# tgialoimtr/cnn_lstm_ctc_ocr

Hardware: AMD Instinct MI355X
Metric: line-crops/sec (train step) at 32x256 bs=256; CER vs ref (higher is better)
Workload: dtype bf16

## Files before the change

cnn_lstm_ctc_ocr_amd/_lib.py:

```python
import ctypes
import os

import torch

_HERE = os.path.dirname(os.path.abspath(__file__))
LIB_PATH = os.environ.get("OCRK_LIB") or os.path.join(_HERE, "libocrk.so")

OCRK_OK = 0
OCRK_ERR_INVALID_ARG = 1
OCRK_ERR_HIP = 2
OCRK_ERR_INFEASIBLE = 3

F32 = 0
BF16 = 1

_p = ctypes.c_void_p
_i32 = ctypes.c_int
_u32 = ctypes.c_uint
_i64 = ctypes.c_int64
_f32 = ctypes.c_float
_sz = ctypes.c_size_t

SIGNATURES = {
    "ocrk_version": [],
    "ocrk_last_error": [],
    "ocrk_set_option": [ctypes.c_char_p, _i64, _p],
    "ocrk_get_option": [ctypes.c_char_p, _p],
    "ocrk_preprocess": [_p, _i64, _p, _i32, _p],
    "ocrk_status_clear": [_p, ctypes.c_uint32, _p],
    "ocrk_set_f32_gemm_mode": [_i32],
    "ocrk_f32_gemm_exact": [],
    "ocrk_ctc_workspace_size": [_i32, _i32, _i32],
    "ocrk_ctc_loss": [_p, _p, _p, _p, _i32, _i32, _i32, _i32, _f32, _p, _p, _p, _p, _p, _sz, _p],
    "ocrk_ctc_align_workspace_size": [_i32, _i32, _i32],
    "ocrk_ctc_align": [_p, _p, _p, _p, _i32, _i32, _i32, _i32, _p, _p, _p, _p, _p, _p, _p, _sz, _p],
    "ocrk_ctc_lexicon_workspace_size": [_i32, _i32, _i32, _i32, _i32],
    "ocrk_ctc_lexicon_score": [_p, _p, _i32, _i32, _i32, _p, _p, _i32, _i32, _i32, _p, _p, _p, _p, _p, _p, _p, _sz,
                               _p],
    "ocrk_ctc_spot_workspace_size": [_i32, _i32, _i32, _i32, _i32],
    "ocrk_ctc_spot": [_p, _p, _i32, _i32, _i32, _p, _p, _p, _i32, _i32, _p, _p, _p, _p, _p, _sz, _p],
    "ocrk_ctc_greedy_decode": [_p, _p, _i32, _i32, _i32, _i32, _p, _p, _p, _p],
    "ocrk_ctc_beam_workspace_size": [_i32, _i32, _i32],
    "ocrk_gru_fwd_step": [_p, _p, _p, _p, _p, _p, _i32, _i32, _i32, _i32, _p, _p, _p, _p, _i32, _p],
    "ocrk_gru_fwd": [_p, _p, _p, _p, _p, _p, _i32, _i32, _i32, _p, _p, _p, _p, _i32, _p],
    "ocrk_gru_bwd": [_p, _p, _p, _p, _p, _p, _p, _i32, _i32, _i32, _p, _p, _p, _p, _i32, _p],
    "ocrk_ctc_beam_decode": [_p, _p, _i32, _i32, _i32, _i32, _i32, _i32, _p, _p, _p, _p, _sz, _p],
    "ocrk_crc32c": [_p, _sz, ctypes.c_uint32],
    "ocrk_edit_distance": [_p, _p, _i32, _p, _p, _i32, _i32, _p, _p, _p],
    "ocrk_conv1_fwd": [_p, _i32, _i32, _i32, _i32, _p, _p, _i32, _p, _i32, _p],
    "ocrk_conv1_wgrad_workspace_size": [_i32, _i32, _i32, _i32],
    "ocrk_conv1_bwd_weight": [_p, _i32, _p, _i32, _i32, _i32, _i32, _p, _p, _i32, _p, _sz, _i32, _p],
    "ocrk_conv2_bwd_data_conv1_wgrad_supported": [_i32, _i32, _i32, _i32, _i32, _i32],
    "ocrk_conv2_bwd_data_conv1_wgrad_workspace_size": [_i32, _i32, _i32],
    "ocrk_conv2_bwd_data_conv1_wgrad": [_p, _i32, _i32, _i32, _p, _p, _p, _p, _i32, _p, _p, _i32, _p, _sz, _i32,
                                        _p],
    "ocrk_conv12_bwd_supported": [_i32, _i32, _i32, _i32],
    "ocrk_conv12_bwd_workspace_size": [_i32, _i32, _i32],
    "ocrk_conv12_bwd": [_p, _i32, _i32, _i32, _p, _p, _p, _p, _i32, _p, _p, _p, _p, _p, _i32, _p, _sz, _i32, _p],
    "ocrk_conv12_fwd_supported": [_i32, _i32, _i32, _i32],
    "ocrk_conv12_fwd": [_p, _i32, _i32, _i32, _i32, _p, _p, _p, _p, _p, _p, _p, _p, _i32, _p],
    "ocrk_conv1_fwd_relu_bits": [_p, _i32, _i32, _i32, _i32, _p, _p, _i32, _p, _p, _i32, _p],
    "ocrk_conv_stats_tiles": [_i64],
    "ocrk_conv3x3_fwd": [_p, _i32, _i32, _i32, _i32, _p, _p, _i32, _p, _i32, _i32, _p, _i32, _p],
    "ocrk_conv3x3_bwd_data_workspace_size": [_i32, _i32, _i32, _i32],
    "ocrk_conv3x3_bwd_data": [_p, _i32, _i32, _i32, _i32, _p, _i32, _p, _p, _p, _i32, _p, _sz, _i32, _p],
    "ocrk_conv3x3_fwd_relu_bits_supported": [_i32, _i32, _i32, _i32, _i32, _i32],
    "ocrk_conv3x3_fwd_relu_bits": [_p, _i32, _i32, _i32, _i32, _p, _p, _i32, _p, _p, _i32, _p],
    "ocrk_conv3x3_bwd_data_bits_supported": [_i32, _i32, _i32, _i32, _i32, _i32],
    "ocrk_conv3x3_bwd_data_bits": [_p, _i32, _i32, _i32, _i32, _p, _i32, _p, _p, _p, _i32, _p, _sz, _i32, _p],
    "ocrk_conv3x3_bwd_data_bits_slab": [_p, _i32, _i32, _i32, _i32, _p, _i32, _p, _p, _p, _i32, _p],
    "ocrk_conv3x3_bwd_data_slab": [_p, _i32, _i32, _i32, _i32, _p, _i32, _p, _p, _p, _i32, _p],
    "ocrk_conv3x3_wgrad_workspace_size": [_i32, _i32, _i32, _i32, _i32],
    "ocrk_conv3x3_bwd_weight": [_p, _p, _i32, _i32, _i32, _i32, _i32, _p, _i32, _p, _sz, _i32, _p],
    "ocrk_bn_finalize_workspace_size": [_i32, _i32],
    "ocrk_bn_finalize": [_p, _i32, _i64, _i32, _f32, _f32, _p, _p, _p, _p, _p, _sz, _p],
    "ocrk_bn_finalize_tiles": [_p, _i32, _i32, _i64, _i32, _f32, _f32, _p, _p, _p, _p, _p, _sz, _p],
    "ocrk_conv3x3_fwd_rowstats_supported": [_i32, _i32, _i32, _i32, _i32],
    "ocrk_conv3x3_fwd_rowstats": [_p, _i32, _i32, _i32, _i32, _p, _p, _i32, _p, _i32, _p, _p],
    "ocrk_bn_infer_params": [_p, _p, _i32, _f32, _p, _p, _p],
    "ocrk_bn_relu_pool_fwd": [_p, _i32, _i32, _i32, _i32, _p, _p, _p, _p, _i32, _i32, _i32, _i32,
                              _p, _i32, _i32, _p],
    "ocrk_bn_bwd_workspace_size": [_i32, _i32, _i32, _i32],
    "ocrk_bn_relu_pool_bwd": [_p, _p, _i32, _i32, _i32, _i32, _p, _p, _p, _p, _i32, _i32, _i32, _i32,
                              _i32, _p, _p, _p, _p, _i32, _p, _sz, _i32, _p],
    "ocrk_bn_moments": [_p, _i32, _i32, _i64, _i32, _p, _p, _sz, _p],
    "ocrk_bn_finalize_moments": [_p, _i32, _f32, _f32, _p, _p, _p, _p, _p],
    "ocrk_bn_bwd_pooled_bias_slab_rows": [_i32, _i32, _i32, _i32, _i32, _i32, _i32, _i32],
    "ocrk_bn_relu_pool_bwd_pooled": [_p, _p, _p, _i32, _i32, _i32, _i32, _p, _p, _p, _p, _i32, _i32, _i32, _i32,
                                     _i32, _p, _p, _p, _p, _i32, _p, _p, _sz, _i32, _p],
    "ocrk_bn_relu_pool_bwd_reduce": [_p, _p, _i32, _i32, _i32, _i32, _p, _p, _p, _p, _i32, _i32, _i32, _i32,
                                     _i32, _p, _p, _i32, _p, _p, _sz, _i32, _p],
    "ocrk_bn_relu_pool_bwd_apply": [_p, _p, _i32, _i32, _i32, _i32, _p, _p, _p, _p, _i32, _i32, _i32, _i32,
                                    _i32, _p, _p, _p, _p, _i32, _p, _p, _sz, _i32, _p],
    "ocrk_bn_bwd_bias_slab_rows": [_i32, _i32, _i32, _i32, _i32, _i32, _i32, _i32],
    "ocrk_bn_relu_pool_bwd_slab": [_p, _p, _i32, _i32, _i32, _i32, _p, _p, _p, _p, _i32, _i32, _i32, _i32,
                                   _i32, _p, _p, _p, _i32, _p, _p, _sz, _i32, _p],
    "ocrk_lstm_fwd_step": [_p, _p, _p, _p, _p, _p, _i32, _i32, _i32, _i32, _p, _p, _p, _p, _i32, _p],
    "ocrk_lstm_bwd_step": [_p, _p, _p, _p, _p, _i32, _i32, _i32, _i32, _p, _p, _p, _p, _i32, _p],
    "ocrk_copy_batch": [_p, _i32, _i64, _p],
    "ocrk_gru_fwd_persistent_supported": [_i32, _i32],
    "ocrk_gru_fwd_persistent_workspace_size": [_i32, _i32],
    "ocrk_gru_fwd_persistent": [_p, _p, _p, _p, _i32, _i32, _i32, _p, _p, _p, _p, _p, _p, _p, _sz, _p],
    "ocrk_gru_bwd_persistent_supported": [_i32, _i32],
    "ocrk_gru_bwd_persistent_workspace_size": [_i32, _i32],
    "ocrk_gru_bwd_persistent": [_p, _p, _p, _i32, _i32, _i32, _p, _p, _p, _p, _p, _p, _p, _p, _sz, _p],
    "ocrk_persistent_flags_size": [_i32, _i32],
    "ocrk_lstm_fwd_persistent_supported": [_i32, _i32],
    "ocrk_lstm_fwd_persistent_workspace_size": [_i32, _i32],
    "ocrk_lstm_fwd_persistent": [_p, _p, _p, _i32, _i32, _i32, _p, _p, _p, _p, _p, _p, _p, _sz, _p],
    "ocrk_lstm_fwd_persistent_f32_supported": [_i32, _i32],
    "ocrk_lstm_fwd_persistent_f32_workspace_size": [_i32, _i32],
    "ocrk_lstm_fwd_persistent_f32_flags_size": [_i32, _i32],
    "ocrk_lstm_fwd_persistent_f32": [_p, _p, _p, _i32, _i32, _i32, _p, _p, _p, _p, _p, _p, _p, _sz, _p],
    "ocrk_lstm_bwd_persistent_f32_supported": [_i32, _i32],
    "ocrk_lstm_bwd_persistent_f32_workspace_size": [_i32, _i32],
    "ocrk_lstm_bwd_persistent_f32": [_p, _p, _i32, _i32, _i32, _p, _p, _p, _p, _p, _p, _p, _p, _sz, _p],
    "ocrk_lstm_bwd_persistent_supported": [_i32, _i32],
    "ocrk_lstm_bwd_persistent_workspace_size": [_i32, _i32],
    "ocrk_lstm_bwd_persistent_slices": [_i32, _i32],
    "ocrk_lstm_bwd_persistent": [_p, _p, _i32, _i32, _i32, _p, _p, _p, _p, _p, _p, _p, _p, _sz, _p],
    "ocrk_lstm_fwd": [_p, _p, _p, _p, _p, _i32, _i32, _i32, _p, _p, _p, _p, _i32, _p],
    "ocrk_lstm_bwd": [_p, _p, _p, _p, _i32, _i32, _i32, _p, _p, _p, _p, _i32, _p],
    "ocrk_gemm_workspace_size": [_i32, _i32, _i32, _i32],
    "ocrk_gemm": [_i32, _i32, _i32, _i32, _i32, _f32, _p, _i64, _i64, _p, _i64, _i64, _p, _i64, _i64,
                  _i32, _p, _i32, _i32, _i32, _i32, _i32, _p, _sz, _p],
    "ocrk_adam": [_p, _p, _p, _p, _i64, _f32, _f32, _f32, _f32, _f32, _p],
    "ocrk_adam_ex": [_p, _p, _p, _p, _i64, _f32, _f32, _f32, _f32, _f32, _u32, _p],
    "ocrk_cast": [_p, _i32, _p, _i32, _i64, _p],
    "ocrk_split_bf16": [_p, _i64, _p, _p, _p],
    "ocrk_permute3": [_p, _i32, _i32, _i32, _i32, _p, _i32, _p],
    "ocrk_strided_copy": [_p, _i64, _i64, _i64, _i64, _p, _i32, _i64, _i64, _p],
    "ocrk_colsum_workspace_size": [_i64, _i32],
    "ocrk_colsum": [_p, _i64, _i32, _i32, _p, _i32, _p, _sz, _p],
    "ocrk_slab_sum_workspace_size": [_i32],
    "ocrk_slab_sum": [_p, _i32, _i32, _i32, _p, _i32, _p, _sz, _p],
    "ocrk_relu_mask": [_p, _p, _i64, _f32, _p, _i32, _p],
    "ocrk_mul_scalar": [_p, _i64, _p, _p],
    "ocrk_mean": [_p, _i32, _p, _p],
    "ocrk_seq_len": [_p, _i32, _p, _p],
    "ocrk_timer_create": [_p],
    "ocrk_timer_record": [_p, _p],
    "ocrk_timer_elapsed": [_p, _p, _p],
    "ocrk_timer_destroy": [_p],
}
_RESTYPE = {"ocrk_last_error": ctypes.c_char_p}
_RESTYPE.update({n: ctypes.c_size_t for n in SIGNATURES if n.endswith("_workspace_size")})
_RESTYPE["ocrk_conv_stats_tiles"] = ctypes.c_size_t
_RESTYPE["ocrk_persistent_flags_size"] = ctypes.c_size_t
_RESTYPE["ocrk_bn_bwd_bias_slab_rows"] = ctypes.c_size_t
_RESTYPE["ocrk_bn_bwd_pooled_bias_slab_rows"] = ctypes.c_size_t
_RESTYPE["ocrk_crc32c"] = ctypes.c_uint32


class OcrkError(RuntimeError):

    def __init__(self, status, message):
        super().__init__(message)
        self.status = status


class InvalidArgumentError(OcrkError):
    """Mirrors tf.errors.InvalidArgumentError (e.g. infeasible CTC labels)."""


class DeviceError(OcrkError):
    """A device-side wait gave up (persistent recurrent kernels): its outputs are invalid."""


STATUS_CTC_INFEASIBLE = 1 << 1
STATUS_CTC_BAD_LENGTH = 1 << 2
STATUS_CTC_BAD_LABEL = 1 << 3
STATUS_LSTM_FWD_TIMEOUT = 1 << 4
STATUS_LSTM_BWD_TIMEOUT = 1 << 5
STATUS_LSTM_CENSUS = 1 << 6
STATUS_CTC = STATUS_CTC_INFEASIBLE | STATUS_CTC_BAD_LENGTH | STATUS_CTC_BAD_LABEL
STATUS_LSTM = STATUS_LSTM_FWD_TIMEOUT | STATUS_LSTM_BWD_TIMEOUT | STATUS_LSTM_CENSUS

_STATUS_TEXT = {
    STATUS_CTC_INFEASIBLE: "ctc_loss: not enough time for the target transition sequence "
                           "(label + repeats > sequence_length)",
    STATUS_CTC_BAD_LENGTH: "ctc_loss: a label length is negative or exceeds the labels' width",
    STATUS_CTC_BAD_LABEL: "ctc_loss: a label value is outside [0, num_classes - 1)",
    STATUS_LSTM_FWD_TIMEOUT: "persistent recurrent forward: a hand-off wait gave up (co-residency lost)",
    STATUS_LSTM_BWD_TIMEOUT: "persistent recurrent backward: a hand-off wait gave up (co-residency lost)",
    STATUS_LSTM_CENSUS: "persistent recurrent launch: the placement census gave up",
}


ON_DEVICE_ERROR = []


def raise_for_status(word):
    word = int(word)
    if not word:
        return
    text = "; ".join(t for b, t in _STATUS_TEXT.items() if word & b)
    if word & STATUS_LSTM:
        for fn in ON_DEVICE_ERROR:
            fn()
        raise DeviceError(OCRK_ERR_HIP, f"device status 0x{word:x}: {text}")
    raise InvalidArgumentError(OCRK_ERR_INFEASIBLE, f"device status 0x{word:x}: {text}")


DEBUG_SIGNATURES = {
    "ocrk_lstm_debug_stamps": [_p],
    "ocrk_conv2_bwd_weight_c1x_supported": [_i32, _i32, _i32, _i32],
    "ocrk_conv2_bwd_weight_c1x": [_p, _i32, _i32, _i32, _i32, _p, _p, _p, _p, _i32, _p, _sz, _i32, _p],
    "ocrk_stream_wait": [_p, _p, _i32],
    "ocrk_stream_create_cu_limited": [_i32, _p],
    "ocrk_stream_destroy": [_p],
    "ocrk_lstm_fwd_persistent_x_supported": [_i32, _i32, _i32],
    "ocrk_lstm_fwd_persistent_x": [_p, _i32, _p, _p, _p, _p, _i32, _i32, _i32, _p, _p, _p, _p, _p, _p, _p, _sz, _p],
}

_lib = None


def lib():
    global _lib
    if _lib is None:
        if not os.path.exists(LIB_PATH):
            raise ImportError(
                f"{LIB_PATH} is missing: build it with `make` in the repo root "
                "(or __graft_entry__.build()); there is no CPU fallback")
        handle = ctypes.CDLL(LIB_PATH)
        for name, argtypes in SIGNATURES.items():
            fn = getattr(handle, name)
            fn.argtypes = argtypes
            fn.restype = _RESTYPE.get(name, ctypes.c_int)
        for name, argtypes in DEBUG_SIGNATURES.items():
            if hasattr(handle, name):
                getattr(handle, name).argtypes = argtypes
        _lib = handle
    return _lib


class Timer:

    def __init__(self):
        h = ctypes.c_void_p()
        call("ocrk_timer_create", ctypes.byref(h))
        self.h = h

    def record(self):
        call("ocrk_timer_record", self.h, stream_ptr())

    def elapsed_ms(self, end):
        ms = ctypes.c_float()
        call("ocrk_timer_elapsed", self.h, end.h, ctypes.byref(ms))
        return ms.value

    def __del__(self):
        if _lib is not None and self.h:
            _lib.ocrk_timer_destroy(self.h)


PROBES = {}


def call(name, *args):
    probe = PROBES.get(name)
    if probe is not None and probe[0] is not None and probe[0](args) is None:
        probe = None
    if probe is not None:
        work_fn, records = probe
        ev0, ev1 = Timer(), Timer()
        ev0.record()
        status = getattr(lib(), name)(*args)
        ev1.record()
        records.append((ev0, ev1, work_fn(args) if work_fn else 0.0))
    else:
        status = getattr(lib(), name)(*args)
    if status != OCRK_OK:
        msg = lib().ocrk_last_error().decode(errors="replace")
        if status in (OCRK_ERR_INFEASIBLE, OCRK_ERR_INVALID_ARG):
            raise InvalidArgumentError(status, msg)
        raise OcrkError(status, msg)
    return status


def ptr(t):
    return None if t is None else ctypes.c_void_p(t.data_ptr())


def stream_ptr(device=None):
    return ctypes.c_void_p(torch.cuda.current_stream(device).cuda_stream)
```

cnn_lstm_ctc_ocr_amd/csrc/conv.hip:

```cpp
#include "common.h"
#include "gemm.h"
#include "reduce.h"
#include "mfma_util.h"

constexpr int C1_PX = 256;
constexpr int C1_WR = 8;

template <typename TIn>
__device__ __forceinline__ float conv1_in(TIn v) {
    if constexpr (sizeof(TIn) == 1) {
#pragma clang fp contract(off)
        return (float)v * (1.0f / 255.0f) - 0.5f;
    } else {
        return to_f32(v);
    }
}

template <typename TIn, int ROWS>
__device__ __forceinline__ void conv1_stage(const TIn* __restrict__ x, int H, int W, int b, int h0, int wo0,
                                            float (*sx)[C1_PX + 2]) {
    constexpr int N = ROWS * (C1_PX + 2), IT = (N + 255) / 256;
    TIn v[IT];
    bool ok[IT];
#pragma unroll
// ... 201 lines not shown
    OCRK_REQUIRE(relu_bits, "ocrk_conv1_fwd_relu_bits: null mask");
    return conv1_fwd_run(x, x_is_u8, B, H, W, w, bias, cout, y, (uint8_t*)relu_bits, dtype, stream);
}

static int64_t conv1_blocks(int B, int H, int W) {
    return std::max<int64_t>(1, (int64_t)B * ocrk::cdiv(H - 2, C1_GR) * ocrk::cdiv(W - 2, C1_PX));
}

extern "C" size_t ocrk_conv1_wgrad_workspace_size(int B, int H, int W, int cout) {
    return ((size_t)conv1_blocks(B, H, W) * 10 * cout * sizeof(float) + 15) / 16 * 16 +
           (size_t)ocrk::SLAB_P * 10 * cout * sizeof(double);
}

extern "C" int ocrk_conv1_bwd_weight(const void* x, int x_is_u8, const void* dz, int B, int H, int W,
                                     int cout, float* dw, float* db, int accumulate, void* ws,
                                     size_t ws_bytes, int dtype, void* stream) {
    OCRK_REQUIRE(cout == 32, "ocrk_conv1_bwd_weight: Cout=%d unsupported", cout);
    OCRK_REQUIRE(ws_bytes >= ocrk_conv1_wgrad_workspace_size(B, H, W, cout), "ocrk_conv1_bwd_weight: workspace too small");
    OCRK_REQUIRE(B >= 1 && H >= 3 && W >= 3, "ocrk_conv1_bwd_weight: bad shape B=%d H=%d W=%d", B, H, W);
    const int64_t nb = conv1_blocks(B, H, W);
    OCRK_REQUIRE(nb < (1ll << 31), "ocrk_conv1_bwd_weight: too many rows");
    hipStream_t s = ocrk::as_stream(stream);
    float* slab = (float*)ws;
    if (x_is_u8) {
        if (dtype == OCRK_BF16) conv1_wgrad_partial<uint8_t, bf16, 32><<<nb, 256, 0, s>>>((const uint8_t*)x, (const bf16*)dz, B, H, W, slab);
        else conv1_wgrad_partial<uint8_t, float, 32><<<nb, 256, 0, s>>>((const uint8_t*)x, (const float*)dz, B, H, W, slab);
    } else {
        if (dtype == OCRK_BF16) conv1_wgrad_partial<bf16, bf16, 32><<<nb, 256, 0, s>>>((const bf16*)x, (const bf16*)dz, B, H, W, slab);
        else conv1_wgrad_partial<float, float, 32><<<nb, 256, 0, s>>>((const float*)x, (const float*)dz, B, H, W, slab);
    }
    int st = ocrk::launch_status("ocrk_conv1_bwd_weight");
    if (st) return st;
    double* part = (double*)((char*)ws + ((size_t)nb * 10 * cout * sizeof(float) + 15) / 16 * 16);
    return ocrk::slab_sum(slab, (int)nb, 10 * cout, part, nullptr, dw, db, 9 * cout, accumulate, s);
}

extern "C" size_t ocrk_conv_stats_tiles(int64_t M) { return (size_t)ocrk::cdiv(M, 128); }

namespace ocrk {
int conv_direct_fwd(const void* x, int B, int H, int W, int cin, const void* w_nk, const float* bias, int cout,
                    void* y, int relu, float* stats, hipStream_t s);
int conv_direct_bwd_data(const void* dy, int B, int H, int W, int cout, const void* w_bwd, int cin, void* dx,
                         const void* relu_mask, float* stats, hipStream_t s);
size_t conv_direct_wgrad_ws_bytes(int B, int H, int W, int cin, int cout);
int conv_direct_wgrad(const void* x, const void* dy, int B, int H, int W, int cin, int cout, float* dw,
                      int accumulate, void* ws, size_t ws_bytes, hipStream_t s);
size_t conv_rows_wgrad_ws_bytes(int B, int cin, int cout);
bool conv_rows_fwd_covers(int B, int H, int W, int cin, int cout);
int conv_rows_fwd(const void* x, int B, int H, int W, int cin, const void* w_nk, const float* bias, int cout, void* y,
                  int relu, float* stats, hipStream_t s);
int conv_rows_dgrad(const void* dy, int B, int H, int W, int cout, const void* w_bwd, int cin, void* dx,
                    const void* relu_mask, float* stats, hipStream_t s);
int conv_rows_wgrad(const void* x, const void* dy, int B, int H, int W, int cin, int cout, float* dw, int accumulate,
                    void* ws, size_t ws_bytes, hipStream_t s);
bool conv_rows_dgrad_c1_covers(int B, int H, int W, int cin, int cout);
bool conv_rows_fwd_bits_covers(int B, int H, int W, int cin, int cout);
bool conv12_fwd_covers(int B, int H, int W);
int conv12_fwd(const void* img, int x_is_u8, int B, int H, int W, const float* w1, const float* b1,
               const void* w_nk2, const float* b2, void* y1, void* bits, void* z, float* stats, hipStream_t s);
int conv_rows_wgrad_c1x(const void* img, int x_is_u8, const float* w1, const float* b1, const void* dy, int B, int H,
                        int W, float* dw, int accumulate, void* ws, size_t ws_bytes, hipStream_t s);
int conv_rows_fwd_bits(const void* x, int B, int H, int W, int cin, const void* w_nk, const float* bias, int cout,
                       void* y, void* bits, hipStream_t s);
bool conv_rows_dgrad_bits_covers(int B, int H, int W, int cin, int cout);
int conv_rows_dgrad_bits(const void* dy, int B, int H, int W, int cout, const void* w_bwd, int cin, void* dx,
                         const void* bits, float* stats, hipStream_t s);
bool gemm_nt_enabled();
bool nt_staged_enabled();
int64_t conv_rows_dgrad_c1_parts(int B);
int conv_rows_dgrad_c1(const void* dy, int B, int H, int W, const void* w_bwd, const void* relu_mask,
                       const void* relu_bits, const void* x, int x_is_u8, float* part, hipStream_t s);
int64_t conv_rows_bwd_w2_parts(int B);
int conv_rows_bwd_w2(const void* dy, int B, int H, int W, const void* w_bwd, const void* relu_mask,
                     const void* relu_bits, const void* x, int x_is_u8, const float* w1, const float* b1,
                     float* c1part, float* w2part, float* dw2, int accumulate, hipStream_t s);
}

extern "C" int ocrk_conv12_fwd_supported(int B, int IH, int IW, int dtype) {
    return dtype == OCRK_BF16 && IH >= 3 && IW >= 3 && ocrk::conv12_fwd_covers(B, IH - 2, IW - 2) ? 1 : 0;
}

extern "C" int ocrk_conv12_fwd(const void* x, int x_is_u8, int B, int IH, int IW, const float* w1, const float* b1,
                               const void* w_nk2, const float* b2, void* y1, void* relu_bits, void* z, float* stats,
                               int dtype, void* stream) {
    OCRK_REQUIRE(ocrk_conv12_fwd_supported(B, IH, IW, dtype), "ocrk_conv12_fwd: B=%d IH=%d IW=%d dtype=%d not covered",
                 B, IH, IW, dtype);
    OCRK_REQUIRE(x && w1 && b1 && w_nk2 && relu_bits && z && stats, "ocrk_conv12_fwd: null pointer");
    return ocrk::conv12_fwd(x, x_is_u8, B, IH - 2, IW - 2, w1, b1, w_nk2, b2, y1, relu_bits, z, stats,
                            ocrk::as_stream(stream));
}

#ifdef OCRK_EXPERIMENTS
extern "C" int ocrk_conv2_bwd_weight_c1x_supported(int B, int IH, int IW, int dtype) {
    return ocrk_conv12_fwd_supported(B, IH, IW, dtype);
}

extern "C" int ocrk_conv2_bwd_weight_c1x(const void* x, int x_is_u8, int B, int IH, int IW, const float* w1,
                                         const float* b1, const void* dz, float* dw, int accumulate, void* ws,
                                         size_t ws_bytes, int dtype, void* stream) {
    OCRK_REQUIRE(ocrk_conv2_bwd_weight_c1x_supported(B, IH, IW, dtype),
                 "ocrk_conv2_bwd_weight_c1x: B=%d IH=%d IW=%d dtype=%d not covered", B, IH, IW, dtype);
    OCRK_REQUIRE(x && w1 && b1 && dz && dw && ws, "ocrk_conv2_bwd_weight_c1x: null pointer");
    int st = ocrk::conv_rows_wgrad_c1x(x, x_is_u8, w1, b1, dz, B, IH - 2, IW - 2, dw, accumulate, ws, ws_bytes,
                                       ocrk::as_stream(stream));
    OCRK_REQUIRE(st >= 0, "ocrk_conv2_bwd_weight_c1x: workspace too small or path disabled");
    return st;
}
#endif

extern "C" int ocrk_conv2_bwd_data_conv1_wgrad_supported(int B, int H, int W, int cin, int cout, int dtype) {
    return dtype == OCRK_BF16 && ocrk::conv_rows_dgrad_c1_covers(B, H, W, cin, cout) ? 1 : 0;
}

extern "C" size_t ocrk_conv2_bwd_data_conv1_wgrad_workspace_size(int B, int H, int W) {
    (void)H; (void)W;
    return ((size_t)ocrk::conv_rows_dgrad_c1_parts(std::max(B, 1)) * 10 * 32 * sizeof(float) + 15) / 16 * 16 +
           (size_t)ocrk::SLAB_P * 10 * 32 * sizeof(double);
}

extern "C" int ocrk_conv2_bwd_data_conv1_wgrad(const void* dz, int B, int H, int W, const void* w_bwd,
                                               const void* relu_mask, const void* relu_bits, const void* x,
                                               int x_is_u8, float* dw, float* db, int accumulate, void* ws,
                                               size_t ws_bytes, int dtype, void* stream) {
    OCRK_REQUIRE(ocrk_conv2_bwd_data_conv1_wgrad_supported(B, H, W, 32, 32, dtype),
                 "ocrk_conv2_bwd_data_conv1_wgrad: B=%d H=%d W=%d dtype=%d not covered", B, H, W, dtype);
    OCRK_REQUIRE(dz && w_bwd && x && dw && db && ws, "ocrk_conv2_bwd_data_conv1_wgrad: null pointer");
    OCRK_REQUIRE(!relu_mask != !relu_bits, "ocrk_conv2_bwd_data_conv1_wgrad: give exactly one of relu_mask / relu_bits");
    OCRK_REQUIRE(ws_bytes >= ocrk_conv2_bwd_data_conv1_wgrad_workspace_size(B, H, W) && (uintptr_t)ws % 16 == 0,
                 "ocrk_conv2_bwd_data_conv1_wgrad: workspace too small or misaligned");
    const int64_t nb = ocrk::conv_rows_dgrad_c1_parts(B);
    OCRK_REQUIRE(nb < (1ll << 31), "ocrk_conv2_bwd_data_conv1_wgrad: too many rows");
    hipStream_t s = ocrk::as_stream(stream);
    float* part = (float*)ws;
    int st = ocrk::conv_rows_dgrad_c1(dz, B, H, W, w_bwd, relu_mask, relu_bits, x, x_is_u8, part, s);
    if (st) return st;
    double* part2 = (double*)((char*)ws + ((size_t)nb * 10 * 32 * sizeof(float) + 15) / 16 * 16);
    return ocrk::slab_sum(part, (int)nb, 10 * 32, part2, nullptr, dw, db, 9 * 32, accumulate, s);
}

static size_t conv12_bwd_c1_bytes(int B) {
    return ((size_t)ocrk::conv_rows_bwd_w2_parts(std::max(B, 1)) * 10 * 32 * sizeof(float) + 15) / 16 * 16;
}

extern "C" int ocrk_conv12_bwd_supported(int B, int H, int W, int dtype) {
    return dtype == OCRK_BF16 && ocrk::conv_rows_dgrad_c1_covers(B, H, W, 32, 32) ? 1 : 0;
}

extern "C" size_t ocrk_conv12_bwd_workspace_size(int B, int H, int W) {
    (void)H; (void)W;
    return conv12_bwd_c1_bytes(B) + (size_t)ocrk::SLAB_P * 10 * 32 * sizeof(double) +
           (size_t)std::max<int64_t>(2, ocrk::conv_rows_bwd_w2_parts(std::max(B, 1))) * 9 * 32 * 32 * sizeof(float);
}

extern "C" int ocrk_conv12_bwd(const void* dz, int B, int H, int W, const void* w_bwd, const void* relu_mask,
                               const void* relu_bits, const void* x, int x_is_u8, const float* w1, const float* b1,
                               float* dw2, float* dw1, float* db1, int accumulate, void* ws, size_t ws_bytes,
                               int dtype, void* stream) {
    OCRK_REQUIRE(ocrk_conv12_bwd_supported(B, H, W, dtype), "ocrk_conv12_bwd: B=%d H=%d W=%d dtype=%d not covered",
                 B, H, W, dtype);
    OCRK_REQUIRE(dz && w_bwd && x && w1 && b1 && dw2 && dw1 && db1 && ws, "ocrk_conv12_bwd: null pointer");
    OCRK_REQUIRE(!relu_mask != !relu_bits, "ocrk_conv12_bwd: give exactly one of relu_mask / relu_bits");
    OCRK_REQUIRE(ws_bytes >= ocrk_conv12_bwd_workspace_size(B, H, W) && (uintptr_t)ws % 16 == 0,
                 "ocrk_conv12_bwd: workspace too small or misaligned");
    const int64_t nb = ocrk::conv_rows_bwd_w2_parts(B);
    OCRK_REQUIRE(nb < (1ll << 31), "ocrk_conv12_bwd: too many rows");
    hipStream_t s = ocrk::as_stream(stream);
    float* c1part = (float*)ws;
    double* c1sum = (double*)((char*)ws + conv12_bwd_c1_bytes(B));
    float* w2part = (float*)((char*)c1sum + (size_t)ocrk::SLAB_P * 10 * 32 * sizeof(double));
    int st = ocrk::conv_rows_bwd_w2(dz, B, H, W, w_bwd, relu_mask, relu_bits, x, x_is_u8, w1, b1, c1part, w2part, dw2,
                                    accumulate, s);
    if (st) return st;
    return ocrk::slab_sum(c1part, (int)nb, 10 * 32, c1sum, nullptr, dw1, db1, 9 * 32, accumulate, s);
}

extern "C" int ocrk_conv3x3_fwd(const void* x, int B, int H, int W, int cin, const void* w_nk,
                                const float* bias, int cout, void* y, int y_dtype, int relu,
                                float* stats, int dtype, void* stream) {
    ocrk::GemmParams p = {};
    p.M = B * H * W; p.N = cout; p.K = 9 * cin; p.batch = 1;
    p.A = x; p.B = w_nk; p.ldb = 9 * cin;
    p.C = y; p.ldc = cout; p.c_bf16 = y_dtype == OCRK_BF16;
    p.bias = bias; p.relu = relu; p.alpha = 1.f; p.stats = stats;
    p.splits = 1; p.k_chunk = (int)ocrk::cdiv(p.K, 32) * 32;
    p.convH = H; p.convW = W; p.convC = cin;
    if (dtype == OCRK_BF16 && y_dtype == OCRK_BF16) {
        int st = stats ? -1 : ocrk::conv_rows_fwd(x, B, H, W, cin, w_nk, bias, cout, y, relu, nullptr, ocrk::as_stream(stream));
        if (st >= 0) return st;
        st = ocrk::conv_direct_fwd(x, B, H, W, cin, w_nk, bias, cout, y, relu, stats, ocrk::as_stream(stream));
        if (st >= 0) return st;
    }
    return ocrk::gemm(p, ocrk::A_IM2COL, ocrk::B_NK, dtype, ocrk::as_stream(stream));
}

extern "C" int ocrk_conv3x3_fwd_rowstats_supported(int B, int H, int W, int cin, int cout) {
    return ocrk::conv_rows_fwd_covers(B, H, W, cin, cout) ? 1 : 0;
}

extern "C" int ocrk_conv3x3_fwd_rowstats(const void* x, int B, int H, int W, int cin, const void* w_nk,
                                         const float* bias, int cout, void* y, int relu, float* stats, void* stream) {
    OCRK_REQUIRE(stats && ocrk::conv_rows_fwd_covers(B, H, W, cin, cout),
                 "ocrk_conv3x3_fwd_rowstats: shape B=%d H=%d W=%d %d->%d not covered", B, H, W, cin, cout);
    return ocrk::conv_rows_fwd(x, B, H, W, cin, w_nk, bias, cout, y, relu, stats, ocrk::as_stream(stream));
}

static int64_t bwd_data_tiles(int B, int H, int W) { return ocrk::cdiv((int64_t)B * H * W, 128); }

static int bwd_data_run(const void* dy, int B, int H, int W, int cout, const void* w_bwd, int cin, void* dx,
                        const void* relu_mask, float* stats, int dtype, hipStream_t s, const void* relu_bits = nullptr) {
    ocrk::GemmParams p = {};
    p.M = B * H * W; p.N = cin; p.K = 9 * cout; p.batch = 1;
    p.A = dy; p.B = w_bwd; p.ldb = 9 * cout;
    p.C = dx; p.ldc = cin; p.c_bf16 = dtype == OCRK_BF16;
    p.mask = relu_mask; p.ldmask = cin; p.alpha = 1.f;
    p.splits = 1; p.k_chunk = (int)ocrk::cdiv(p.K, 32) * 32;
    p.convH = H; p.convW = W; p.convC = cout;
    p.stats = stats;
    if (relu_bits) {
        const int sb = ocrk::conv_rows_dgrad_bits(dy, B, H, W, cout, w_bwd, cin, dx, relu_bits, stats, s);
        if (sb >= 0) return sb;
        p.mask = nullptr;
        p.mask_bits = relu_bits;
        return ocrk::gemm(p, ocrk::A_IM2COL_FLIP, ocrk::B_NK, dtype, s);
    }
    int st = dtype == OCRK_BF16 ? ocrk::conv_rows_dgrad(dy, B, H, W, cout, w_bwd, cin, dx, relu_mask, stats, s) : -1;
    if (st < 0 && dtype == OCRK_BF16) st = ocrk::conv_direct_bwd_data(dy, B, H, W, cout, w_bwd, cin, dx, relu_mask, stats, s);
    if (st < 0) st = ocrk::gemm(p, ocrk::A_IM2COL_FLIP, ocrk::B_NK, dtype, s);
    return st;
}

static bool nt_bits_ok(int cin, int cout) {
    return ocrk::gemm_nt_enabled() && ocrk::nt_staged_enabled() && cin % 8 == 0 && cout % 8 == 0 &&
           (9 * cin >= 512 || cout <= 64);
}

extern "C" int ocrk_conv3x3_fwd_relu_bits_supported(int B, int H, int W, int cin, int cout, int dtype) {
    if (dtype != OCRK_BF16 || B < 1 || H < 1 || W < 1 || (int64_t)B * H * W >= (1ll << 31)) return 0;
    return ocrk::conv_rows_fwd_bits_covers(B, H, W, cin, cout) || nt_bits_ok(cin, cout) ? 1 : 0;
}

extern "C" int ocrk_conv3x3_fwd_relu_bits(const void* x, int B, int H, int W, int cin, const void* w_nk,
                                          const float* bias, int cout, void* y, void* relu_bits, int dtype,
                                          void* stream) {
    OCRK_REQUIRE(relu_bits && ocrk_conv3x3_fwd_relu_bits_supported(B, H, W, cin, cout, dtype),
                 "ocrk_conv3x3_fwd_relu_bits: B=%d H=%d W=%d %d->%d dtype=%d not covered", B, H, W, cin, cout, dtype);
    hipStream_t s = ocrk::as_stream(stream);
    const int st = ocrk::conv_rows_fwd_bits(x, B, H, W, cin, w_nk, bias, cout, y, relu_bits, s);
    if (st >= 0) return st;
    ocrk::GemmParams p = {};
    p.M = B * H * W; p.N = cout; p.K = 9 * cin; p.batch = 1;
    p.A = x; p.B = w_nk; p.ldb = 9 * cin;
    p.C = y; p.ldc = cout; p.c_bf16 = 1;
    p.bias = bias; p.relu = 1; p.alpha = 1.f;
    p.splits = 1; p.k_chunk = (int)ocrk::cdiv(p.K, 32) * 32;
    p.convH = H; p.convW = W; p.convC = cin;
    p.relu_bits = relu_bits;
    return ocrk::gemm(p, ocrk::A_IM2COL, ocrk::B_NK, dtype, s);
}

extern "C" int ocrk_conv3x3_bwd_data_bits_supported(int B, int H, int W, int cout, int cin, int dtype) {
    if (dtype != OCRK_BF16 || B < 1 || H < 1 || W < 1 || (int64_t)B * H * W >= (1ll << 31)) return 0;
    return ocrk::conv_rows_dgrad_bits_covers(B, H, W, cin, cout) || nt_bits_ok(cout, cin) ? 1 : 0;
}

extern "C" size_t ocrk_conv3x3_bwd_data_workspace_size(int B, int H, int W, int cin) {
    return ((size_t)bwd_data_tiles(B, H, W) * 2 * cin * sizeof(float) + 7) / 8 * 8 +
           (size_t)ocrk::SLAB_P * cin * sizeof(double);
}

extern "C" int ocrk_conv3x3_bwd_data_bits(const void* dy, int B, int H, int W, int cout, const void* w_bwd, int cin,
                                          void* dx, const void* relu_bits, float* dbias, int accumulate, void* ws,
                                          size_t ws_bytes, int dtype, void* stream) {
    OCRK_REQUIRE(relu_bits && ocrk_conv3x3_bwd_data_bits_supported(B, H, W, cout, cin, dtype),
                 "ocrk_conv3x3_bwd_data_bits: B=%d H=%d W=%d %d<-%d dtype=%d not covered", B, H, W, cin, cout, dtype);
    hipStream_t s = ocrk::as_stream(stream);
    if (!dbias) return bwd_data_run(dy, B, H, W, cout, w_bwd, cin, dx, nullptr, nullptr, dtype, s, relu_bits);
    OCRK_REQUIRE(ws && ws_bytes >= ocrk_conv3x3_bwd_data_workspace_size(B, H, W, cin),
                 "ocrk_conv3x3_bwd_data_bits: workspace too small for the bias gradient");
    int st = bwd_data_run(dy, B, H, W, cout, w_bwd, cin, dx, nullptr, (float*)ws, dtype, s, relu_bits);
    if (st) return st;
    const int tiles = (int)bwd_data_tiles(B, H, W);
    double* part = (double*)((char*)ws + ((size_t)tiles * 2 * cin * sizeof(float) + 7) / 8 * 8);
    return ocrk::slab_sum((const float*)ws, tiles, cin, part, nullptr, dbias, nullptr, cin, accumulate, s, 2 * cin);
}

extern "C" int ocrk_conv3x3_bwd_data(const void* dy, int B, int H, int W, int cout, const void* w_bwd,
                                     int cin, void* dx, const void* relu_mask, float* dbias, int accumulate,
                                     void* ws, size_t ws_bytes, int dtype, void* stream) {
    hipStream_t s = ocrk::as_stream(stream);
    if (!dbias) return bwd_data_run(dy, B, H, W, cout, w_bwd, cin, dx, relu_mask, nullptr, dtype, s);
    OCRK_REQUIRE(ws && ws_bytes >= ocrk_conv3x3_bwd_data_workspace_size(B, H, W, cin),
                 "ocrk_conv3x3_bwd_data: workspace too small for the bias gradient");
    int st = bwd_data_run(dy, B, H, W, cout, w_bwd, cin, dx, relu_mask, (float*)ws, dtype, s);
    if (st) return st;
    const int tiles = (int)bwd_data_tiles(B, H, W);
    double* part = (double*)((char*)ws + ((size_t)tiles * 2 * cin * sizeof(float) + 7) / 8 * 8);
    return ocrk::slab_sum((const float*)ws, tiles, cin, part, nullptr, dbias, nullptr, cin, accumulate, s, 2 * cin);
}

extern "C" int ocrk_conv3x3_bwd_data_bits_slab(const void* dy, int B, int H, int W, int cout, const void* w_bwd,
                                               int cin, void* dx, const void* relu_bits, float* slab, int dtype,
                                               void* stream) {
    OCRK_REQUIRE(slab && relu_bits && ocrk_conv3x3_bwd_data_bits_supported(B, H, W, cout, cin, dtype),
                 "ocrk_conv3x3_bwd_data_bits_slab: B=%d H=%d W=%d %d<-%d dtype=%d not covered (or no slab)", B, H, W,
                 cin, cout, dtype);
    return bwd_data_run(dy, B, H, W, cout, w_bwd, cin, dx, nullptr, slab, dtype, ocrk::as_stream(stream), relu_bits);
}

extern "C" int ocrk_conv3x3_bwd_data_slab(const void* dy, int B, int H, int W, int cout, const void* w_bwd,
                                          int cin, void* dx, const void* relu_mask, float* slab, int dtype,
                                          void* stream) {
    OCRK_REQUIRE(slab, "ocrk_conv3x3_bwd_data_slab: slab is required");
    return bwd_data_run(dy, B, H, W, cout, w_bwd, cin, dx, relu_mask, slab, dtype, ocrk::as_stream(stream));
}

static int conv_tn_items() {
    const int64_t v = ocrk::opt(ocrk::OPT_CONV_TN_ITEMS);
    return v >= 16 ? (int)v : 192;
}

static int wgrad_splits(int64_t M, int cin, int cout) {
    if (ocrk::gemm_pptn_covers(ocrk::A_IM2COL_T, 9 * cin, cout, cin)) {
        const int64_t tiles = ocrk::cdiv(9 * cin, 256) * ocrk::cdiv(cout, 256);
        return (int)std::max<int64_t>(1, std::min<int64_t>(conv_tn_items() / tiles, M / 2048));
    }
    int64_t tiles = ocrk::cdiv(9 * cin, 128) * ocrk::cdiv(cout, cout <= 32 ? 32 : (cout <= 64 ? 64 : 128));
// ... 41 lines not shown
```

cnn_lstm_ctc_ocr_amd/csrc/tensor_ops.hip:

```cpp
#include "common.h"
#include "reduce.h"
#include "mfma_util.h"

template <typename TI, typename TO>
__global__ void __launch_bounds__(256) cast_kernel(const TI* __restrict__ in, TO* __restrict__ out, int64_t n) {
    for (int64_t i = (int64_t)blockIdx.x * 256 + threadIdx.x; i < n; i += (int64_t)gridDim.x * 256)
        out[i] = from_f32<TO>(to_f32(in[i]));
}

template <typename TI, typename TO>
__global__ void __launch_bounds__(256) permute3_kernel(const TI* __restrict__ in, int d0, int d1, int d2,
                                                       TO* __restrict__ out) {
    const int64_t n = (int64_t)d0 * d1 * d2;
    for (int64_t o = (int64_t)blockIdx.x * 256 + threadIdx.x; o < n; o += (int64_t)gridDim.x * 256) {
        int i2 = (int)(o % d2);
        int64_t t = o / d2;
        int i0 = (int)(t % d0);
        int i1 = (int)(t / d0);
        out[o] = from_f32<TO>(to_f32(in[((int64_t)i0 * d1 + i1) * d2 + i2]));
    }
}

namespace ocrk {
namespace {

__global__ void __launch_bounds__(256)
slab_sum_fused(const float* __restrict__ slab, int nslab, int NC, int ld, float* __restrict__ res,
               float* __restrict__ dst_lo, float* __restrict__ dst_hi, int split, int accumulate) {
    constexpr int RG = 64, CQ = 4, U = 16;
    __shared__ double red[RG][4 * CQ + 1];
    const int cq = threadIdx.x % CQ, rg = threadIdx.x / CQ;
    const int c0 = blockIdx.x * 4 * CQ + 4 * cq;
    double s[4] = {0.0, 0.0, 0.0, 0.0};
    if (c0 < NC) {
        const float* col = slab + c0;
        int i = rg;
        for (; i + (U - 1) * RG < nslab; i += U * RG) {
            f32x4 v[U];
#pragma unroll
            for (int u = 0; u < U; ++u) v[u] = *reinterpret_cast<const f32x4*>(col + (int64_t)(i + u * RG) * ld);
#pragma unroll
            for (int u = 0; u < U; ++u)
#pragma unroll
                for (int e = 0; e < 4; ++e) s[e] += v[u][e];
        }
        for (; i < nslab; i += RG) {
            const f32x4 v = *reinterpret_cast<const f32x4*>(col + (int64_t)i * ld);
#pragma unroll
            for (int e = 0; e < 4; ++e) s[e] += v[e];
        }
    }
#pragma unroll
    for (int e = 0; e < 4; ++e) red[rg][4 * cq + e] = s[e];
    __syncthreads();
    if (threadIdx.x < 4 * CQ) {
        const int c = blockIdx.x * 4 * CQ + threadIdx.x;
        if (c >= NC) return;
        double t = 0.0;
        for (int y = 0; y < RG; ++y) t += red[y][threadIdx.x];
        const float v = (float)t;
        if (res) res[c] = v;
        float* d = c < split ? (dst_lo ? dst_lo + c : nullptr) : (dst_hi ? dst_hi + (c - split) : nullptr);
        if (d) *d = accumulate ? *d + v : v;
    }
}

__global__ void __launch_bounds__(256)
slab_sum_stage1(const float* __restrict__ slab, int nslab, int NC, int ld, double* __restrict__ part) {
    __shared__ double red[4][64];
    const int cl = threadIdx.x & 63, q = threadIdx.x >> 6;
    const int c = blockIdx.x * 64 + cl;
    const int rows = (nslab + SLAB_P - 1) / SLAB_P;
    const int r0 = blockIdx.y * rows, r1 = min(nslab, r0 + rows);
    double s = 0.0;
    if (c < NC)
        for (int i = r0 + q; i < r1; i += 4) s += slab[(int64_t)i * ld + c];
    red[q][cl] = s;
    __syncthreads();
    if (q == 0 && c < NC) part[(int64_t)blockIdx.y * NC + c] = red[0][cl] + red[1][cl] + red[2][cl] + red[3][cl];
}

__global__ void __launch_bounds__(64)
slab_sum_stage2(const double* __restrict__ part, int NC, float* __restrict__ res, float* __restrict__ dst_lo,
                float* __restrict__ dst_hi, int split, int accumulate) {
    const int c = blockIdx.x * 64 + threadIdx.x;
    if (c >= NC) return;
    double t = 0.0;
    for (int y = 0; y < SLAB_P; ++y) t += part[(int64_t)y * NC + c];
    const float v = (float)t;
    if (res) res[c] = v;
    float* d = c < split ? (dst_lo ? dst_lo + c : nullptr) : (dst_hi ? dst_hi + (c - split) : nullptr);
    if (d) *d = accumulate ? *d + v : v;
}

}

int slab_sum(const float* slab, int nslab, int NC, double* part, float* res, float* dst_lo, float* dst_hi,
             int split, int accumulate, hipStream_t s, int ld) {
    const int l = ld > 0 ? ld : NC;
    if (NC % 4 == 0 && l % 4 == 0 && ((uintptr_t)slab & 15) == 0) {
        slab_sum_fused<<<(NC + 15) / 16, 256, 0, s>>>(slab, nslab, NC, l, res, dst_lo, dst_hi, split, accumulate);
        return ocrk::launch_status("slab sum");
    }
    slab_sum_stage1<<<dim3((NC + 63) / 64, SLAB_P), 256, 0, s>>>(slab, nslab, NC, ld > 0 ? ld : NC, part);
    int st = ocrk::launch_status("slab sum 1");
    if (st) return st;
    slab_sum_stage2<<<(NC + 63) / 64, 64, 0, s>>>(part, NC, res, dst_lo, dst_hi, split, accumulate);
    return ocrk::launch_status("slab sum 2");
}

}

template <typename T>
__global__ void __launch_bounds__(256) colsum_partial_kernel(const T* __restrict__ in, int64_t M, int N,
                                                             int64_t rows_per_block, float* __restrict__ slab) {
    __shared__ float red[256 * 9];
    const int G = N / 8;
    const int TPR = G < 64 ? G : 64;
    const int RPP = 256 / TPR;
    const int tg = threadIdx.x % TPR, tr = threadIdx.x / TPR;
    const int g = blockIdx.x * TPR + tg;
    const int64_t r0 = (int64_t)blockIdx.y * rows_per_block;
    const int64_t r1 = min(M, r0 + rows_per_block);
    float acc[8] = {0.f, 0.f, 0.f, 0.f, 0.f, 0.f, 0.f, 0.f};
    if (tr < RPP && g < G) {
#pragma unroll 4
        for (int64_t r = r0 + tr; r < r1; r += RPP) {
            const F8 v = load8(in + r * N + g * 8);
#pragma unroll
            for (int i = 0; i < 8; ++i) acc[i] += v.v[i];
        }
    }
#pragma unroll
    for (int i = 0; i < 8; ++i) red[threadIdx.x * 9 + i] = acc[i];
    __syncthreads();
    for (int o = threadIdx.x; o < TPR * 8; o += 256) {
        int gg = o / 8, i = o % 8;
        float sum = 0.f;
        for (int q = 0; q < RPP; ++q) sum += red[(q * TPR + gg) * 9 + i];
        if (blockIdx.x * TPR + gg < G) slab[(int64_t)blockIdx.y * N + (blockIdx.x * TPR + gg) * 8 + i] = sum;
    }
}

template <typename TO>
__global__ void __launch_bounds__(256) relu_mask_kernel(const float* __restrict__ dy, const float* __restrict__ y,
                                                        int64_t n, float scale, TO* __restrict__ out) {
    for (int64_t i = (int64_t)blockIdx.x * 256 + threadIdx.x; i < n; i += (int64_t)gridDim.x * 256)
        out[i] = from_f32<TO>(y[i] > 0.f ? dy[i] * scale : 0.f);
}

static unsigned grid1d(int64_t n) { return (unsigned)std::max<int64_t>(1, std::min<int64_t>(ocrk::cdiv(n, 256), 16384)); }

extern "C" int ocrk_cast(const void* in, int in_dtype, void* out, int out_dtype, int64_t n, void* stream) {
    if (n == 0) return OCRK_OK;
    hipStream_t s = ocrk::as_stream(stream);
    if (in_dtype == OCRK_F32 && out_dtype == OCRK_BF16) cast_kernel<float, bf16><<<grid1d(n), 256, 0, s>>>((const float*)in, (bf16*)out, n);
    else if (in_dtype == OCRK_BF16 && out_dtype == OCRK_F32) cast_kernel<bf16, float><<<grid1d(n), 256, 0, s>>>((const bf16*)in, (float*)out, n);
    else if (in_dtype == OCRK_F32 && out_dtype == OCRK_F32) cast_kernel<float, float><<<grid1d(n), 256, 0, s>>>((const float*)in, (float*)out, n);
    else cast_kernel<bf16, bf16><<<grid1d(n), 256, 0, s>>>((const bf16*)in, (bf16*)out, n);
    return ocrk::launch_status("ocrk_cast");
}

__global__ void split_bf16_kernel(const float* __restrict__ x, unsigned* __restrict__ hi, unsigned* __restrict__ lo,
                                  int64_t n8) {
    for (int64_t i = blockIdx.x * (int64_t)blockDim.x + threadIdx.x; i < n8; i += (int64_t)gridDim.x * blockDim.x) {
        const float4 a = reinterpret_cast<const float4*>(x)[2 * i], b = reinterpret_cast<const float4*>(x)[2 * i + 1];
        unsigned h[4], l[4];
        ocrk::split2_bf16(a.x, a.y, h[0], l[0]);
        ocrk::split2_bf16(a.z, a.w, h[1], l[1]);
        ocrk::split2_bf16(b.x, b.y, h[2], l[2]);
        ocrk::split2_bf16(b.z, b.w, h[3], l[3]);
        reinterpret_cast<uint4*>(hi)[i] = make_uint4(h[0], h[1], h[2], h[3]);
        reinterpret_cast<uint4*>(lo)[i] = make_uint4(l[0], l[1], l[2], l[3]);
    }
}

extern "C" int ocrk_split_bf16(const float* x, int64_t n, void* hi, void* lo, void* stream) {
    OCRK_REQUIRE(n % 8 == 0 && ((uintptr_t)x | (uintptr_t)hi | (uintptr_t)lo) % 16 == 0,
                 "ocrk_split_bf16: n=%lld must be a multiple of 8 and the buffers 16-B aligned", (long long)n);
    if (n == 0) return OCRK_OK;
    split_bf16_kernel<<<grid1d(n / 8), 256, 0, ocrk::as_stream(stream)>>>(x, (unsigned*)hi, (unsigned*)lo, n / 8);
    return ocrk::launch_status("ocrk_split_bf16");
}

extern "C" int ocrk_permute3(const void* in, int in_dtype, int d0, int d1, int d2, void* out, int out_dtype,
                             void* stream) {
    int64_t n = (int64_t)d0 * d1 * d2;
    if (n == 0) return OCRK_OK;
    hipStream_t s = ocrk::as_stream(stream);
    OCRK_REQUIRE(in_dtype == OCRK_F32, "ocrk_permute3: f32 input only");
    if (out_dtype == OCRK_BF16) permute3_kernel<float, bf16><<<grid1d(n), 256, 0, s>>>((const float*)in, d0, d1, d2, (bf16*)out);
    else permute3_kernel<float, float><<<grid1d(n), 256, 0, s>>>((const float*)in, d0, d1, d2, (float*)out);
    return ocrk::launch_status("ocrk_permute3");
}

static int colsum_col_blocks(int N) { return (int)ocrk::cdiv(N / 8, 64); }
static int64_t colsum_blocks(int64_t M, int N) {
    const int64_t want = std::max<int64_t>(1, 2048 / colsum_col_blocks(std::max(N, 8)));
    return std::max<int64_t>(1, std::min<int64_t>(want, ocrk::cdiv(M, 64)));
}

extern "C" size_t ocrk_colsum_workspace_size(int64_t M, int N) {
    return ((size_t)colsum_blocks(M, N) * N * sizeof(float) + 7) / 8 * 8 + (size_t)ocrk::SLAB_P * N * sizeof(double);
}

extern "C" int ocrk_colsum(const void* in, int64_t M, int N, int dtype, float* out, int accumulate, void* ws,
                           size_t ws_bytes, void* stream) {
    OCRK_REQUIRE(ws_bytes >= ocrk_colsum_workspace_size(M, N), "ocrk_colsum: workspace too small");
    OCRK_REQUIRE(N % 8 == 0, "ocrk_colsum: N=%d must be a multiple of 8", N);
    if (N == 0) return OCRK_OK;
    int64_t nb = colsum_blocks(M, N);
    int64_t rpb = ocrk::cdiv(M, nb);
    nb = std::max<int64_t>(1, ocrk::cdiv(M, rpb));
    hipStream_t s = ocrk::as_stream(stream);
    dim3 grid(colsum_col_blocks(N), (unsigned)nb);
    if (dtype == OCRK_BF16) colsum_partial_kernel<bf16><<<grid, 256, 0, s>>>((const bf16*)in, M, N, rpb, (float*)ws);
    else colsum_partial_kernel<float><<<grid, 256, 0, s>>>((const float*)in, M, N, rpb, (float*)ws);
    int st = ocrk::launch_status("ocrk_colsum");
    if (st) return st;
    double* part = (double*)((char*)ws + ((size_t)nb * N * sizeof(float) + 7) / 8 * 8);
    return ocrk::slab_sum((const float*)ws, (int)nb, N, part, nullptr, out, nullptr, N, accumulate, s);
}

extern "C" size_t ocrk_slab_sum_workspace_size(int nc) { return (size_t)ocrk::SLAB_P * std::max(nc, 1) * sizeof(double); }

extern "C" int ocrk_slab_sum(const float* slab, int nslab, int nc, int ld, float* out, int accumulate, void* ws,
                             size_t ws_bytes, void* stream) {
    OCRK_REQUIRE(nslab >= 0 && nc >= 0 && ld >= nc, "ocrk_slab_sum: bad sizes");
    OCRK_REQUIRE(ws_bytes >= ocrk_slab_sum_workspace_size(nc), "ocrk_slab_sum: workspace too small");
    if (nc == 0) return OCRK_OK;
    return ocrk::slab_sum(slab, nslab, nc, (double*)ws, nullptr, out, nullptr, nc, accumulate, ocrk::as_stream(stream),
                          ld);
}

extern "C" int ocrk_relu_mask(const float* dy, const float* y, int64_t n, float scale, void* out, int out_dtype,
                              void* stream) {
    if (n == 0) return OCRK_OK;
    hipStream_t s = ocrk::as_stream(stream);
    if (out_dtype == OCRK_BF16) relu_mask_kernel<bf16><<<grid1d(n), 256, 0, s>>>(dy, y, n, scale, (bf16*)out);
    else relu_mask_kernel<float><<<grid1d(n), 256, 0, s>>>(dy, y, n, scale, (float*)out);
    return ocrk::launch_status("ocrk_relu_mask");
}

template <typename TO>
__global__ void __launch_bounds__(256) strided_copy_kernel(const float* __restrict__ in, int64_t rows, int64_t cols,
                                                           int64_t in_rs, int64_t in_cs, TO* __restrict__ out,
                                                           int64_t out_rs, int64_t out_cs) {
    const int64_t n = rows * cols;
    for (int64_t i = (int64_t)blockIdx.x * 256 + threadIdx.x; i < n; i += (int64_t)gridDim.x * 256) {
        int64_t r = i / cols, c = i - r * cols;
        out[r * out_rs + c * out_cs] = from_f32<TO>(in[r * in_rs + c * in_cs]);
    }
}

extern "C" int ocrk_strided_copy(const float* in, int64_t rows, int64_t cols, int64_t in_rs, int64_t in_cs,
                                 void* out, int out_dtype, int64_t out_rs, int64_t out_cs, void* stream) {
    int64_t n = rows * cols;
    if (n == 0) return OCRK_OK;
    hipStream_t s = ocrk::as_stream(stream);
    if (out_dtype == OCRK_BF16)
        strided_copy_kernel<bf16><<<grid1d(n), 256, 0, s>>>(in, rows, cols, in_rs, in_cs, (bf16*)out, out_rs, out_cs);
    else
        strided_copy_kernel<float><<<grid1d(n), 256, 0, s>>>(in, rows, cols, in_rs, in_cs, (float*)out, out_rs, out_cs);
    return ocrk::launch_status("ocrk_strided_copy");
}

struct CopyJob {
    const float* src;
    void* dst;
    int64_t rows, cols, in_rs, out_rs, tile0;
    int transpose, dtype;
};
static_assert(sizeof(CopyJob) == 8 * 8, "job layout (include/ocrk.h)");

constexpr int COPY_JOBS_LDS = 256;
__global__ void __launch_bounds__(256) copy_batch_kernel(const CopyJob* __restrict__ jobs, int njobs) {
    __shared__ float tile[32][33];
    __shared__ int64_t first[COPY_JOBS_LDS];
    const int64_t t = blockIdx.x;
    int lo = 0, hi = njobs - 1;
    if (njobs <= COPY_JOBS_LDS) {
        if ((int)threadIdx.x < njobs) first[threadIdx.x] = jobs[threadIdx.x].tile0;
        __syncthreads();
        while (lo < hi) {
            const int mid = (lo + hi + 1) >> 1;
            if (first[mid] <= t) lo = mid; else hi = mid - 1;
        }
    } else {
        while (lo < hi) {
            const int mid = (lo + hi + 1) >> 1;
            if (jobs[mid].tile0 <= t) lo = mid; else hi = mid - 1;
        }
    }
    const CopyJob j = jobs[lo];
    const int64_t lt = t - j.tile0, tc = (j.cols + 31) / 32;
    const int64_t r0 = (lt / tc) * 32, c0 = (lt % tc) * 32;
    const bool bf = j.dtype == OCRK_BF16;
    const bool vec = ((j.rows | j.cols | j.in_rs | j.out_rs) & 3) == 0 && ((uintptr_t)j.src & 15) == 0 &&
                     ((uintptr_t)j.dst & (bf ? 7 : 15)) == 0;
    if (vec) {
        const int q = threadIdx.x >> 3, c4 = (threadIdx.x & 7) * 4;
        if (r0 + q < j.rows && c0 + c4 < j.cols) {
            const float4 v = *reinterpret_cast<const float4*>(j.src + (r0 + q) * j.in_rs + c0 + c4);
            tile[q][c4] = v.x; tile[q][c4 + 1] = v.y; tile[q][c4 + 2] = v.z; tile[q][c4 + 3] = v.w;
        }
        __syncthreads();
        float o[4];
        int64_t orow, ocol;
        if (j.transpose) {
            orow = c0 + q; ocol = r0 + c4;
            if (orow >= j.cols || ocol >= j.rows) return;
#pragma unroll
            for (int e = 0; e < 4; ++e) o[e] = tile[c4 + e][q];
        } else {
            orow = r0 + q; ocol = c0 + c4;
            if (orow >= j.rows || ocol >= j.cols) return;
#pragma unroll
            for (int e = 0; e < 4; ++e) o[e] = tile[q][c4 + e];
        }
        const int64_t off = orow * j.out_rs + ocol;
        if (bf) {
            typedef unsigned int u32x2_t __attribute__((ext_vector_type(2)));
            u32x2_t w;
            w[0] = (unsigned)__builtin_bit_cast(unsigned short, (bf16)o[0]) |
                   ((unsigned)__builtin_bit_cast(unsigned short, (bf16)o[1]) << 16);
            w[1] = (unsigned)__builtin_bit_cast(unsigned short, (bf16)o[2]) |
                   ((unsigned)__builtin_bit_cast(unsigned short, (bf16)o[3]) << 16);
            *reinterpret_cast<u32x2_t*>(reinterpret_cast<bf16*>(j.dst) + off) = w;
        } else {
            *reinterpret_cast<float4*>(reinterpret_cast<float*>(j.dst) + off) = make_float4(o[0], o[1], o[2], o[3]);
        }
        return;
    }
    const int tx = threadIdx.x & 31, ty = threadIdx.x >> 5;
#pragma unroll
    for (int k = 0; k < 4; ++k) {
        const int64_t r = r0 + ty + 8 * k, c = c0 + tx;
        tile[ty + 8 * k][tx] = (r < j.rows && c < j.cols) ? j.src[r * j.in_rs + c] : 0.f;
    }
    __syncthreads();
#pragma unroll
    for (int k = 0; k < 4; ++k) {
        int64_t orow, ocol;
        float v;
        if (j.transpose) {
            orow = c0 + ty + 8 * k; ocol = r0 + tx;
            v = tile[tx][ty + 8 * k];
            if (orow >= j.cols || ocol >= j.rows) continue;
        } else {
            orow = r0 + ty + 8 * k; ocol = c0 + tx;
            v = tile[ty + 8 * k][tx];
            if (orow >= j.rows || ocol >= j.cols) continue;
        }
        const int64_t o = orow * j.out_rs + ocol;
        if (bf) reinterpret_cast<bf16*>(j.dst)[o] = (bf16)v;
        else reinterpret_cast<float*>(j.dst)[o] = v;
    }
}

extern "C" int ocrk_copy_batch(const void* jobs, int njobs, int64_t total_tiles, void* stream) {
    OCRK_REQUIRE(njobs >= 1 && total_tiles >= 1 && total_tiles < (1ll << 31), "ocrk_copy_batch: njobs=%d tiles=%lld",
                 njobs, (long long)total_tiles);
    copy_batch_kernel<<<(unsigned)total_tiles, 256, 0, ocrk::as_stream(stream)>>>((const CopyJob*)jobs, njobs);
    return ocrk::launch_status("ocrk_copy_batch");
}

__global__ void __launch_bounds__(256) mul_scalar_kernel(float* __restrict__ x, int64_t n, const float* __restrict__ s) {
    const float v = s[0];
    for (int64_t i = (int64_t)blockIdx.x * 256 + threadIdx.x; i < n; i += (int64_t)gridDim.x * 256) x[i] *= v;
}

extern "C" int ocrk_mul_scalar(float* x, int64_t n, const float* s, void* stream) {
    if (n == 0) return OCRK_OK;
    mul_scalar_kernel<<<grid1d(n), 256, 0, ocrk::as_stream(stream)>>>(x, n, s);
    return ocrk::launch_status("ocrk_mul_scalar");
}

__global__ void __launch_bounds__(256) mean_kernel(const float* __restrict__ x, int n, float* __restrict__ out) {
    __shared__ double s[256];
    double acc = 0.0;
    for (int i = threadIdx.x; i < n; i += 256) acc += x[i];
    s[threadIdx.x] = acc;
    __syncthreads();
    for (int k = 128; k > 0; k >>= 1) {
        if (threadIdx.x < k) s[threadIdx.x] += s[threadIdx.x + k];
        __syncthreads();
    }
// ... 34 lines not shown
```

cnn_lstm_ctc_ocr_amd/kernels.py:

```python
import ctypes

import torch

from . import _lib, options
from ._lib import ptr, call

F32, BF16 = _lib.F32, _lib.BF16
_DT = {torch.float32: F32, torch.bfloat16: BF16}


def dtype_code(dt):
    try:
        return _DT[dt]
    except KeyError:
        raise TypeError(f"unsupported dtype {dt}; libocrk computes in float32 or bfloat16")


def _stream(t):
    return _lib.stream_ptr(t.device)


def _chk(*ts):
    for t in ts:
        if t is None:
            continue
        if not t.is_cuda:
            raise ValueError("libocrk ops take device tensors (got a CPU tensor)")
        if not t.is_contiguous():
            raise ValueError("libocrk ops take contiguous tensors")


def _ws(nbytes, device):
    return torch.empty(max(int(nbytes), 16), dtype=torch.uint8, device=device)


def preprocess(img_u8, dtype=torch.float32):
    if img_u8.dtype != torch.uint8:
        raise TypeError("preprocess expects uint8 pixels")
    _chk(img_u8)
    out = torch.empty(img_u8.shape, dtype=dtype, device=img_u8.device)
    call("ocrk_preprocess", ptr(img_u8), img_u8.numel(), ptr(out), dtype_code(dtype), _stream(img_u8))
    return out


def seq_len(widths):
    _chk(widths)
    w = widths if widths.dtype == torch.int32 else widths.to(torch.int32)
    out = torch.empty_like(w)
    call("ocrk_seq_len", ptr(w), w.numel(), ptr(out), _stream(w))
    return out


def conv1_fwd(x, w, b, dtype, relu_bits=False):
    _chk(x, w, b)
    B, H, W = x.shape[0], x.shape[1], x.shape[2]
    C = w.shape[-1]
    y = torch.empty(B, H - 2, W - 2, C, dtype=dtype, device=x.device)
    is_u8 = x.dtype == torch.uint8
    if not is_u8 and x.dtype != dtype:
        raise TypeError("conv1 float input must have the compute dtype")
    if relu_bits:
        bits = torch.empty(B, H - 2, W - 2, C // 8, dtype=torch.uint8, device=x.device)
        call("ocrk_conv1_fwd_relu_bits", ptr(x), int(is_u8), B, H, W, ptr(w), ptr(b), C, ptr(y), ptr(bits),
             dtype_code(dtype), _stream(x))
        return y, bits
    call("ocrk_conv1_fwd", ptr(x), int(is_u8), B, H, W, ptr(w), ptr(b), C, ptr(y), dtype_code(dtype), _stream(x))
    return y


def conv12_fwd_ok(x, dtype):
    B, IH, IW = x.shape[:3]
    return (x.dtype in (torch.uint8, torch.bfloat16) and (x.dtype == torch.uint8 or x.dtype == dtype)
            and bool(_lib.lib().ocrk_conv12_fwd_supported(B, IH, IW, dtype_code(dtype))))


def conv12_fwd(x, w1, b1, w_nk2, b2, want_y1=True):
    _chk(x, w1, b1, w_nk2, b2)
    B, IH, IW = x.shape[:3]
    H, W = IH - 2, IW - 2
    dev = x.device
    y1 = torch.empty(B, H, W, 32, dtype=torch.bfloat16, device=dev) if want_y1 else None
    bits = torch.empty(B, H, W, 4, dtype=torch.uint8, device=dev)
    z = torch.empty(B, H, W, 32, dtype=torch.bfloat16, device=dev)
    stats = torch.empty(B * H, 2, 32, dtype=torch.float32, device=dev)
    call("ocrk_conv12_fwd", ptr(x), int(x.dtype == torch.uint8), B, IH, IW, ptr(w1), ptr(b1), ptr(w_nk2), ptr(b2),
         ptr(y1), ptr(bits), ptr(z), ptr(stats), BF16, _stream(x))
    return y1, bits, z, stats


def conv2_bwd_weight_c1x(x, w1, b1, dz, dw, accumulate=True):
    _chk(x, w1, b1, dz, dw)
    B, IH, IW = x.shape[:3]
    nb = _lib.lib().ocrk_conv3x3_wgrad_workspace_size(B, IH - 2, IW - 2, 32, 32)
    ws = _ws(nb, x.device)
    call("ocrk_conv2_bwd_weight_c1x", ptr(x), int(x.dtype == torch.uint8), B, IH, IW, ptr(w1), ptr(b1), ptr(dz),
         ptr(dw), int(accumulate), ptr(ws), nb, BF16, _stream(x))


def conv1_bwd_weight(x, dz, dw, db, accumulate=True):
    _chk(x, dz, dw, db)
    B, H, W = x.shape[0], x.shape[1], x.shape[2]
    C = dz.shape[-1]
    nb = _lib.lib().ocrk_conv1_wgrad_workspace_size(B, H, W, C)
    ws = _ws(nb, x.device)
    call("ocrk_conv1_bwd_weight", ptr(x), int(x.dtype == torch.uint8), ptr(dz), B, H, W, C, ptr(dw), ptr(db),
         int(accumulate), ptr(ws), nb, dtype_code(dz.dtype), _stream(x))


def conv2_bwd_data_conv1_wgrad_ok(dz, x):
    B, H, W, C = dz.shape
    return (x.dtype in (torch.uint8, torch.bfloat16) and tuple(x.shape) == (B, H + 2, W + 2)
            and bool(_lib.lib().ocrk_conv2_bwd_data_conv1_wgrad_supported(B, H, W, C, C, dtype_code(dz.dtype))))


def conv2_bwd_data_conv1_wgrad(dz, w_bwd, relu_mask, x, dw, db, accumulate=True, relu_bits=None):
    _chk(dz, w_bwd, relu_mask, relu_bits, x, dw, db)
    if (relu_mask is None) == (relu_bits is None):
        raise ValueError("give exactly one of relu_mask / relu_bits")
    B, H, W, _ = dz.shape
    if relu_bits is not None and (relu_bits.dtype != torch.uint8 or tuple(relu_bits.shape) != (B, H, W, 4)):
        raise ValueError("relu_bits must be uint8 [B, H, W, 4]")
    nb = _lib.lib().ocrk_conv2_bwd_data_conv1_wgrad_workspace_size(B, H, W)
    ws = _ws(nb, dz.device)
    call("ocrk_conv2_bwd_data_conv1_wgrad", ptr(dz), B, H, W, ptr(w_bwd), ptr(relu_mask), ptr(relu_bits), ptr(x),
         int(x.dtype == torch.uint8), ptr(dw), ptr(db), int(accumulate), ptr(ws), nb, dtype_code(dz.dtype),
         _stream(dz))


def conv12_bwd_ok(x, dtype):
    B, IH, IW = x.shape[:3]
    return (x.dim() == 3 and dtype == torch.bfloat16 and x.dtype in (torch.uint8, torch.bfloat16)
            and IH >= 3 and IW >= 3 and bool(_lib.lib().ocrk_conv12_bwd_supported(B, IH - 2, IW - 2, BF16)))


def conv12_bwd(dz, w_bwd, x, w1, b1, dw2, dw1, db1, relu_mask=None, relu_bits=None, accumulate=True):
    _chk(dz, w_bwd, relu_mask, relu_bits, x, w1, b1, dw2, dw1, db1)
    if (relu_mask is None) == (relu_bits is None):
        raise ValueError("give exactly one of relu_mask / relu_bits")
    B, H, W, _ = dz.shape
    if relu_bits is not None and (relu_bits.dtype != torch.uint8 or tuple(relu_bits.shape) != (B, H, W, 4)):
        raise ValueError("relu_bits must be uint8 [B, H, W, 4]")
    nb = _lib.lib().ocrk_conv12_bwd_workspace_size(B, H, W)
    ws = _ws(nb, dz.device)
    call("ocrk_conv12_bwd", ptr(dz), B, H, W, ptr(w_bwd), ptr(relu_mask), ptr(relu_bits), ptr(x),
         int(x.dtype == torch.uint8), ptr(w1), ptr(b1), ptr(dw2), ptr(dw1), ptr(db1), int(accumulate), ptr(ws), nb,
         BF16, _stream(dz))


def conv_stats_tiles(M):
    return _lib.lib().ocrk_conv_stats_tiles(M)


def relu_bits_ok(x_shape, cin, cout, cout_next, dtype):
    B, H, W = x_shape[:3]
    lib = _lib.lib()
    code = dtype_code(dtype)
    return (bool(lib.ocrk_conv3x3_fwd_relu_bits_supported(B, H, W, cin, cout, code))
            and bool(lib.ocrk_conv3x3_bwd_data_bits_supported(B, H, W, cout_next, cout, code)))


def conv3x3_fwd_relu_bits(x, w_nk, bias):
    _chk(x, w_nk, bias)
    B, H, W, Cin = x.shape
    Cout = w_nk.shape[0]
    y = torch.empty(B, H, W, Cout, dtype=x.dtype, device=x.device)
    bits = torch.empty(B, H, W, Cout // 8, dtype=torch.uint8, device=x.device)
    call("ocrk_conv3x3_fwd_relu_bits", ptr(x), B, H, W, Cin, ptr(w_nk), ptr(bias), Cout, ptr(y), ptr(bits),
         dtype_code(x.dtype), _stream(x))
    return y, bits


def conv3x3_fwd(x, w_nk, bias, relu, stats=None, y_dtype=None):
    _chk(x, w_nk, bias, stats)
    B, H, W, Cin = x.shape
    Cout = w_nk.shape[0]
    y_dtype = y_dtype or x.dtype
    y = torch.empty(B, H, W, Cout, dtype=y_dtype, device=x.device)
    call("ocrk_conv3x3_fwd", ptr(x), B, H, W, Cin, ptr(w_nk), ptr(bias), Cout, ptr(y), dtype_code(y_dtype),
         int(relu), ptr(stats), dtype_code(x.dtype), _stream(x))
    return y


def conv3x3_bwd_data(dy, w_bwd, relu_mask=None, dbias=None, accumulate=True, defer=None, relu_bits=None):
    _chk(dy, w_bwd, relu_mask, dbias, relu_bits)
    B, H, W, Cout = dy.shape
    Cin = w_bwd.shape[0]
    dx = torch.empty(B, H, W, Cin, dtype=dy.dtype, device=dy.device)
    if relu_bits is not None:
        if relu_mask is not None:
            raise ValueError("relu_bits replaces relu_mask")
        if dbias is not None and defer is not None:
            tiles = conv_stats_tiles(B * H * W)
            slab = torch.empty(tiles, 2 * Cin, dtype=torch.float32, device=dy.device)
            call("ocrk_conv3x3_bwd_data_bits_slab", ptr(dy), B, H, W, Cout, ptr(w_bwd), Cin, ptr(dx), ptr(relu_bits),
                 ptr(slab), dtype_code(dy.dtype), _stream(dy))
            defer.append((lambda: slab_sum(slab, tiles, Cin, 2 * Cin, dbias, accumulate), (slab,)))
            return dx
        nb, ws = 0, None
        if dbias is not None:
            nb = _lib.lib().ocrk_conv3x3_bwd_data_workspace_size(B, H, W, Cin)
            ws = _ws(nb, dy.device)
        call("ocrk_conv3x3_bwd_data_bits", ptr(dy), B, H, W, Cout, ptr(w_bwd), Cin, ptr(dx), ptr(relu_bits),
             ptr(dbias), int(accumulate), ptr(ws), nb, dtype_code(dy.dtype), _stream(dy))
        return dx
    if dbias is not None and defer is not None:
        tiles = conv_stats_tiles(B * H * W)
        slab = torch.empty(tiles, 2 * Cin, dtype=torch.float32, device=dy.device)
        call("ocrk_conv3x3_bwd_data_slab", ptr(dy), B, H, W, Cout, ptr(w_bwd), Cin, ptr(dx), ptr(relu_mask),
             ptr(slab), dtype_code(dy.dtype), _stream(dy))
        defer.append((lambda: slab_sum(slab, tiles, Cin, 2 * Cin, dbias, accumulate), (slab,)))
        return dx
    nb, ws = 0, None
    if dbias is not None:
        nb = _lib.lib().ocrk_conv3x3_bwd_data_workspace_size(B, H, W, Cin)
        ws = _ws(nb, dy.device)
    call("ocrk_conv3x3_bwd_data", ptr(dy), B, H, W, Cout, ptr(w_bwd), Cin, ptr(dx), ptr(relu_mask), ptr(dbias),
         int(accumulate), ptr(ws), nb, dtype_code(dy.dtype), _stream(dy))
    return dx


def conv3x3_bwd_weight(x, dy, dw, accumulate=True):
    _chk(x, dy, dw)
    B, H, W, Cin = x.shape
    Cout = dy.shape[-1]
    nb = _lib.lib().ocrk_conv3x3_wgrad_workspace_size(B, H, W, Cin, Cout)
    ws = _ws(nb, x.device)
    call("ocrk_conv3x3_bwd_weight", ptr(x), ptr(dy), B, H, W, Cin, Cout, ptr(dw), int(accumulate), ptr(ws), nb,
         dtype_code(x.dtype), _stream(x))


def bn_finalize(stats, M, C, eps, momentum, moving_mean=None, moving_var=None, tile_rows=128):
    _chk(stats, moving_mean, moving_var)
    tiles = stats.shape[0]
    mean = torch.empty(C, dtype=torch.float32, device=stats.device)
    invstd = torch.empty_like(mean)
    nb = _lib.lib().ocrk_bn_finalize_workspace_size(tiles, C)
    ws = _ws(nb, stats.device)
    call("ocrk_bn_finalize_tiles", ptr(stats), tiles, int(tile_rows), M, C, float(eps), float(momentum), ptr(mean),
         ptr(invstd), ptr(moving_mean), ptr(moving_var), ptr(ws), nb, _stream(stats))
    return mean, invstd


def bn_finalize_sync(stats, M, C, eps, momentum, moving_mean, moving_var, tile_rows, group):
    import torch.distributed as dist
    _chk(stats, moving_mean, moving_var)
    tiles = stats.shape[0]
    moments = torch.empty(3 * C + 1, dtype=torch.float64, device=stats.device)
    nb = _lib.lib().ocrk_bn_finalize_workspace_size(tiles, C)
    ws = _ws(nb, stats.device)
    call("ocrk_bn_moments", ptr(stats), tiles, int(tile_rows), M, C, ptr(moments), ptr(ws), nb, _stream(stats))
    dist.all_reduce(moments, op=dist.ReduceOp.SUM, group=group)
    mean = torch.empty(C, dtype=torch.float32, device=stats.device)
    invstd = torch.empty_like(mean)
    call("ocrk_bn_finalize_moments", ptr(moments), C, float(eps), float(momentum), ptr(mean), ptr(invstd),
         ptr(moving_mean), ptr(moving_var), _stream(stats))
    return mean, invstd, moments[3 * C:]


def conv3x3_fwd_rowstats_ok(x, cout):
    if x.dtype != torch.bfloat16 or not x.is_cuda:
        return False
    B, H, W, cin = x.shape
    return bool(_lib.lib().ocrk_conv3x3_fwd_rowstats_supported(B, H, W, cin, cout))


def conv3x3_fwd_rowstats(x, w_nk, bias, relu=False):
    _chk(x, w_nk, bias)
    B, H, W, cin = x.shape
    cout = w_nk.shape[0]
    y = torch.empty(B, H, W, cout, dtype=x.dtype, device=x.device)
    stats = torch.empty(B * H, 2, cout, dtype=torch.float32, device=x.device)
    call("ocrk_conv3x3_fwd_rowstats", ptr(x), B, H, W, cin, ptr(w_nk), ptr(bias), cout, ptr(y), int(relu),
         ptr(stats), _stream(x))
    return y, stats


def bn_infer_params(moving_mean, moving_var, eps):
    _chk(moving_mean, moving_var)
    C = moving_mean.numel()
    mean = torch.empty(C, dtype=torch.float32, device=moving_mean.device)
    invstd = torch.empty_like(mean)
    call("ocrk_bn_infer_params", ptr(moving_mean), ptr(moving_var), C, float(eps), ptr(mean), ptr(invstd),
         _stream(moving_mean))
    return mean, invstd


def bn_relu_pool_fwd(z, mean, invstd, gamma, beta, pool, time_major=False):
    _chk(z, mean, invstd, gamma, beta)
    B, H, W, C = z.shape
    kh, kw, sh, sw = pool
    Ho, Wo = (H - kh) // sh + 1, (W - kw) // sw + 1
    shape = (Wo, B, C) if time_major else (B, Ho, Wo, C)
    out = torch.empty(shape, dtype=z.dtype, device=z.device)
    call("ocrk_bn_relu_pool_fwd", ptr(z), B, H, W, C, ptr(mean), ptr(invstd), ptr(gamma), ptr(beta), kh, kw, sh, sw,
         ptr(out), int(time_major), dtype_code(z.dtype), _stream(z))
    return out


def bn_relu_pool_bwd(z, dp, mean, invstd, gamma, beta, pool, dp_time_major, dgamma, dbeta, accumulate=True,
                     dbias=None, defer=None, sync=None, pooled=None):
    _chk(z, dp, mean, invstd, gamma, beta, dgamma, dbeta, dbias, pooled)
    B, H, W, C = z.shape
    kh, kw, sh, sw = pool
    nb = _lib.lib().ocrk_bn_bwd_workspace_size(B, H, W, C)
    ws = _ws(nb, z.device)
    dz = torch.empty_like(z)
    if sync is not None:
        return _bn_bwd_sync(z, dp, mean, invstd, gamma, beta, pool, dp_time_major, dgamma, dbeta, accumulate, dbias,
                            defer, sync, dz, ws, nb)
    if pooled is not None:
        if pooled.shape != dp.shape or pooled.dtype != dp.dtype:
            raise ValueError("pooled must have dp's shape and dtype")
        rows = _lib.lib().ocrk_bn_bwd_pooled_bias_slab_rows(B, H, W, C, kh, kw, sh, sw)
        if rows == 0:
            pooled = None
    if pooled is not None:
        slab = None
        if dbias is not None and defer is not None:
            slab = torch.empty(rows, 2 * C, dtype=torch.float32, device=z.device)
        call("ocrk_bn_relu_pool_bwd_pooled", ptr(z), ptr(pooled), ptr(dp), B, H, W, C, ptr(mean), ptr(invstd),
             ptr(gamma), ptr(beta), kh, kw, sh, sw, int(dp_time_major), ptr(dz), ptr(dgamma), ptr(dbeta),
             ptr(dbias), int(accumulate), ptr(slab), ptr(ws), nb, dtype_code(z.dtype), _stream(z))
        if slab is not None:
            def _late():
                slab_sum(slab, rows, C, 2 * C, dbias, accumulate)
                slab_sum(slab.view(-1)[C:], rows, C, 2 * C, dgamma, accumulate)
            defer.append((_late, (slab,)))
        return dz
    if dbias is not None and defer is not None:
        rows = _lib.lib().ocrk_bn_bwd_bias_slab_rows(B, H, W, C, kh, kw, sh, sw)
        slab = torch.empty(rows, C, dtype=torch.float32, device=z.device)
        call("ocrk_bn_relu_pool_bwd_slab", ptr(z), ptr(dp), B, H, W, C, ptr(mean), ptr(invstd), ptr(gamma),
             ptr(beta), kh, kw, sh, sw, int(dp_time_major), ptr(dz), ptr(dgamma), ptr(dbeta), int(accumulate),
             ptr(slab), ptr(ws), nb, dtype_code(z.dtype), _stream(z))
        defer.append((lambda: slab_sum(slab, rows, C, C, dbias, accumulate), (slab,)))
        return dz
    call("ocrk_bn_relu_pool_bwd", ptr(z), ptr(dp), B, H, W, C, ptr(mean), ptr(invstd), ptr(gamma), ptr(beta),
         kh, kw, sh, sw, int(dp_time_major), ptr(dz), ptr(dgamma), ptr(dbeta), ptr(dbias), int(accumulate),
         ptr(ws), nb,
         dtype_code(z.dtype), _stream(z))
    return dz


def _bn_bwd_sync(z, dp, mean, invstd, gamma, beta, pool, dp_time_major, dgamma, dbeta, accumulate, dbias, defer,
                 sync, dz, ws, nb):
    import torch.distributed as dist
    group, count = sync
    B, H, W, C = z.shape
    kh, kw, sh, sw = pool
    dsum = torch.empty(2 * C, dtype=torch.float32, device=z.device)
    args = (ptr(z), ptr(dp), B, H, W, C, ptr(mean), ptr(invstd), ptr(gamma), ptr(beta), kh, kw, sh, sw,
            int(dp_time_major))
    call("ocrk_bn_relu_pool_bwd_reduce", *args, ptr(dgamma), ptr(dbeta), int(accumulate), ptr(dsum), ptr(ws), nb,
         dtype_code(z.dtype), _stream(z))
    dist.all_reduce(dsum, op=dist.ReduceOp.SUM, group=group)
    slab = None
    if dbias is not None and defer is not None:
        rows = _lib.lib().ocrk_bn_bwd_bias_slab_rows(B, H, W, C, kh, kw, sh, sw)
        slab = torch.empty(rows, C, dtype=torch.float32, device=z.device)
    call("ocrk_bn_relu_pool_bwd_apply", *args, ptr(dsum), ptr(count), ptr(dz),
         ptr(dbias if slab is None else None), int(accumulate), ptr(slab), ptr(ws), nb, dtype_code(z.dtype), _stream(z))
    if slab is not None:
        defer.append((lambda: slab_sum(slab, rows, C, C, dbias, accumulate), (slab,)))
    return dz


def gemm(a, b, trans_a=False, trans_b=False, bias=None, relu=False, out=None, out_dtype=torch.float32,
         accumulate=False, alpha=1.0, M=None, N=None, K=None, lda=None, ldb=None, ldc=None,
         batch=1, stride_a=0, stride_b=0, stride_c=0, splits=1):
    for t in (a, b, bias, out):
        if t is not None and not t.is_cuda:
            raise ValueError("libocrk ops take device tensors (got a CPU tensor)")
    if M is None:
        _chk(a, b)
        M, K = (a.shape[1], a.shape[0]) if trans_a else (a.shape[0], a.shape[1])
        N = b.shape[0] if trans_b else b.shape[1]
        lda, ldb = a.shape[1], b.shape[1]
    if out is None:
        out = torch.empty(M, N, dtype=out_dtype, device=a.device)
        ldc = N
    ldc = ldc if ldc is not None else N
    if a.dtype != b.dtype:
        raise TypeError("gemm operands must share a dtype")
    kc = -(-(-(-K // splits)) // 32) * 32 if splits > 1 else K
    splits = -(-K // kc) if splits > 1 else 1
    nb = _lib.lib().ocrk_gemm_workspace_size(M, N, batch, splits) if splits > 1 else 0
    ws = _ws(nb, a.device) if nb else None
    call("ocrk_gemm", int(trans_a), int(trans_b), M, N, K, float(alpha), ptr(a), lda, stride_a, ptr(b), ldb,
         stride_b, ptr(out), ldc, stride_c, dtype_code(out.dtype), ptr(bias), int(relu), int(accumulate),
         batch, dtype_code(a.dtype), splits, ptr(ws), nb, _stream(a))
    return out


_PERSISTENT = {}


def lstm_persistent_ok(B, H, dtype):
    if dtype != torch.bfloat16 or not options.get("LSTM_PERSISTENT"):
        return False
    key = (B, H)
    if key not in _PERSISTENT:
        lib = _lib.lib()
        _PERSISTENT[key] = bool(lib.ocrk_lstm_fwd_persistent_supported(B, H)) and \
            bool(lib.ocrk_lstm_bwd_persistent_supported(B, H))
    return _PERSISTENT[key]


_STATUS = {}
_FLAGS = {}


def persistent_flags(kind, B, H, device, size_fn="ocrk_persistent_flags_size"):
    device = torch.device(device)
    key = (kind, B, H, device, torch.cuda.current_stream(device).cuda_stream)
    t = _FLAGS.get(key)
    if t is None:
        nb = getattr(_lib.lib(), size_fn)(B, H)
        t = _FLAGS[key] = torch.zeros(max(int(nb), 16) // 4, dtype=torch.int32, device=device)
    return t


def reset_persistent_flags():
    for t in _FLAGS.values():
        t.zero_()
    for d in {t.device for t in _FLAGS.values()}:
        torch.cuda.synchronize(d)


_lib.ON_DEVICE_ERROR.append(reset_persistent_flags)


def status_word(device):
    device = torch.device(device)
    if device not in _STATUS:
        _STATUS[device] = torch.zeros(1, dtype=torch.int32, device=device)
    return _STATUS[device]


lstm_error_word = status_word


def clear_status(device, bits):
    w = status_word(device)
    if bits:
        call("ocrk_status_clear", ptr(w), int(bits) & 0xFFFFFFFF, _stream(w))


def read_status(device, reset=True):
    w = status_word(device)
    v = int(w.item())
    if v and reset:
        clear_status(device, v)
    return v


def check_status(device, reset=True):
    _lib.raise_for_status(read_status(device, reset))


class f32_exact:

    def __init__(self, on=True):
        self.on = on
        self.prev = None

    def __enter__(self):
        self.prev = _lib.lib().ocrk_set_f32_gemm_mode(1 if self.on else 0)
        return self

    def __exit__(self, *exc):
        _lib.lib().ocrk_set_f32_gemm_mode(self.prev)
        return False


def f32_mode_exact():
    return bool(_lib.lib().ocrk_f32_gemm_exact())


def lstm_f32_persistent_ok(B, H):
    if not options.get("LSTM_PERSISTENT") or f32_mode_exact():
        return False
    key = ("f32", B, H)
    if key not in _PERSISTENT:
        _PERSISTENT[key] = bool(_lib.lib().ocrk_lstm_fwd_persistent_f32_supported(B, H))
    return _PERSISTENT[key]


def lstm_f32_bwd_persistent_ok(B, H):
    if not options.get("LSTM_PERSISTENT") or f32_mode_exact():
        return False
    key = ("f32bwd", B, H)
    if key not in _PERSISTENT:
        _PERSISTENT[key] = bool(_lib.lib().ocrk_lstm_bwd_persistent_f32_supported(B, H))
    return _PERSISTENT[key]


def lstm_fwd(gx, whT, seq_len, T, B, H, dtype, save=True):
    _chk(gx, whT, seq_len)
    if gx.dtype != dtype or whT.dtype != dtype:
        raise TypeError(f"lstm_fwd: gx and whT must be {dtype} (got {gx.dtype}, {whT.dtype})")
    dev = gx.device
    if dtype == torch.float32 and lstm_f32_persistent_ok(B, H):
        out = torch.empty(T, B, 2 * H, dtype=dtype, device=dev)
        hprev = cprev = acts = None
        if save:
            hprev = torch.empty(T, B, 2, H, dtype=dtype, device=dev)
            cprev = torch.empty(T, B, 2, H, dtype=torch.float32, device=dev)
            acts = torch.empty(T, B, 2, 4 * H, dtype=dtype, device=dev)
        nb = _lib.lib().ocrk_lstm_fwd_persistent_f32_workspace_size(B, H)
        ws = _ws(nb, dev)
        call("ocrk_lstm_fwd_persistent_f32", ptr(gx), ptr(whT), ptr(seq_len), T, B, H, ptr(out), ptr(hprev),
             ptr(cprev), ptr(acts), ptr(lstm_error_word(dev)),
             ptr(persistent_flags("lstm_fwd_f32", B, H, dev, "ocrk_lstm_fwd_persistent_f32_flags_size")),
             ptr(ws), nb, _stream(gx))
        return out, hprev, cprev, acts
    if lstm_persistent_ok(B, H, dtype):
# ... 70 lines not shown
    dc_state = torch.zeros(2, B, H, dtype=torch.float32, device=dev)
    call("ocrk_lstm_bwd", ptr(wh), ptr(dg_state), ptr(dc_state), ptr(seq_len), T, B, H, ptr(dout), ptr(cprev),
         ptr(acts), ptr(dG), dtype_code(dtype), _stream(dout))
    if dbias is not None:
        colsum(dG, T * B, 2 * 4 * H, dbias)
    return dG


_GRU_PERSISTENT = {}


def gru_persistent_ok(B, H, dtype):
    if dtype != torch.bfloat16 or not options.get("LSTM_PERSISTENT"):
        return False
    key = (B, H)
    if key not in _GRU_PERSISTENT:
        lib = _lib.lib()
        _GRU_PERSISTENT[key] = bool(lib.ocrk_gru_fwd_persistent_supported(B, H)) and \
            bool(lib.ocrk_gru_bwd_persistent_supported(B, H))
    return _GRU_PERSISTENT[key]


def gru_fwd(gx, whgT, whcT, seq_len, T, B, H, dtype):
    _chk(gx, whgT, whcT, seq_len)
    if gx.dtype != dtype or whgT.dtype != dtype:
        raise TypeError(f"gru_fwd: gx and weights must be {dtype} (got {gx.dtype}, {whgT.dtype})")
    dev = gx.device
    if gru_persistent_ok(B, H, dtype):
        out = torch.empty(T, B, 2 * H, dtype=dtype, device=dev)
        hprev = torch.empty(T, B, 2, H, dtype=dtype, device=dev)
        rh_t = torch.empty(T, B, 2, H, dtype=dtype, device=dev)
        acts = torch.empty(T, B, 2, 3 * H, dtype=dtype, device=dev)
        nb = _lib.lib().ocrk_gru_fwd_persistent_workspace_size(B, H)
        ws = _ws(nb, dev)
        call("ocrk_gru_fwd_persistent", ptr(gx), ptr(whgT), ptr(whcT), ptr(seq_len), T, B, H, ptr(out), ptr(hprev),
             ptr(rh_t), ptr(acts), ptr(status_word(dev)), ptr(persistent_flags("gru_fwd", B, H, dev)), ptr(ws), nb,
             _stream(gx))
        return out, hprev, rh_t, acts
    h = torch.zeros(2, B, H, dtype=dtype, device=dev)
    rh = torch.empty(2, B, H, dtype=dtype, device=dev)
    out = torch.zeros(T, B, 2 * H, dtype=dtype, device=dev)
    hprev = torch.empty(T, B, 2, H, dtype=dtype, device=dev)
    rh_t = torch.empty(T, B, 2, H, dtype=dtype, device=dev)
    acts = torch.empty(T, B, 2, 3 * H, dtype=dtype, device=dev)
    call("ocrk_gru_fwd", ptr(gx), ptr(whgT), ptr(whcT), ptr(h), ptr(rh), ptr(seq_len), T, B, H, ptr(out),
         ptr(hprev), ptr(rh_t), ptr(acts), dtype_code(dtype), _stream(gx))
    return out, hprev, rh_t, acts


def gru_bwd(whg, whc, seq_len, dout, hprev, acts, T, B, H, dbias=None, defer=None):
    _chk(whg, whc, seq_len, dout, hprev, acts, dbias)
    dtype = dout.dtype
    dev = dout.device
    if gru_persistent_ok(B, H, dtype):
        dG = torch.empty(T, B, 2, 3 * H, dtype=dtype, device=dev)
        nb = _lib.lib().ocrk_gru_bwd_persistent_workspace_size(B, H)
        ws = _ws(nb, dev)
        part = torch.empty(B // 32, 2 * 3 * H, dtype=torch.float32, device=dev) if dbias is not None else None
        call("ocrk_gru_bwd_persistent", ptr(whg), ptr(whc), ptr(seq_len), T, B, H, ptr(dout), ptr(hprev), ptr(acts),
             ptr(dG), ptr(status_word(dev)), ptr(persistent_flags("gru_bwd", B, H, dev)), ptr(part), ptr(ws), nb,
             _stream(dout))
        if dbias is not None:
            _bias_parts(part, B // 32, 2 * 3 * H, dbias, defer)
        return dG
    dzg = torch.empty(2, B, 2 * H, dtype=dtype, device=dev)
    dzc = torch.empty(2, B, H, dtype=dtype, device=dev)
    dh_tot = torch.empty(2, B, H, dtype=torch.float32, device=dev)
    direct = torch.empty(2, B, H, dtype=torch.float32, device=dev)
    dG = torch.empty(T, B, 2, 3 * H, dtype=dtype, device=dev)
    call("ocrk_gru_bwd", ptr(whg), ptr(whc), ptr(dzg), ptr(dzc), ptr(dh_tot), ptr(direct), ptr(seq_len), T, B, H,
         ptr(dout), ptr(hprev), ptr(acts), ptr(dG), dtype_code(dtype), _stream(dout))
    if dbias is not None:
        colsum(dG, T * B, 2 * 3 * H, dbias)
    return dG


def split_bf16(x):
    _chk(x)
    if x.dtype != torch.float32 or not x.is_contiguous():
        raise TypeError("split_bf16 takes a contiguous float32 tensor")
    hi = torch.empty(x.shape, dtype=torch.bfloat16, device=x.device)
    lo = torch.empty_like(hi)
    call("ocrk_split_bf16", ptr(x), x.numel(), ptr(hi), ptr(lo), _stream(x))
    return hi, lo


def split_products(*tensors):
    a, b = (split_bf16(t) for t in tensors)
    return [(a[0], b[0]), (a[0], b[1]), (a[1], b[0])]


def cast(x, dtype, out=None):
    _chk(x)
    out = out if out is not None else torch.empty(x.shape, dtype=dtype, device=x.device)
    call("ocrk_cast", ptr(x), dtype_code(x.dtype), ptr(out), dtype_code(out.dtype), x.numel(), _stream(x))
    return out


def permute3(x, d0, d1, d2, dtype, out=None):
    _chk(x)
    out = out if out is not None else torch.empty(d1, d0, d2, dtype=dtype, device=x.device)
    call("ocrk_permute3", ptr(x), dtype_code(x.dtype), d0, d1, d2, ptr(out), dtype_code(out.dtype), _stream(x))
    return out


def stream_wait(waiter, signaller, mode=1):
    call("ocrk_stream_wait", ctypes.c_void_p(waiter.cuda_stream), ctypes.c_void_p(signaller.cuda_stream), int(mode))


_CU_STREAMS = []


def cu_limited_stream(device, n_cus):
    with torch.cuda.device(device):
        h = ctypes.c_void_p()
        call("ocrk_stream_create_cu_limited", int(n_cus), ctypes.byref(h))
        st = torch.cuda.ExternalStream(h.value, device=device)
    _CU_STREAMS.append((h, st))
    return st


def fork(waiter, signaller):
    waiter.wait_stream(signaller)


def wait_mark(waiter, mark):
    waiter.wait_event(mark)


def copy_batch(table, njobs, total_tiles, stream_of):
    _chk(table, stream_of)
    call("ocrk_copy_batch", ptr(table), int(njobs), int(total_tiles), _stream(stream_of))


def strided_copy(src, rows, cols, in_rs, in_cs, out, out_rs, out_cs, out_offset=0, in_offset=0):
    _chk(src, out)
    sp = ctypes_offset(src, in_offset)
    op = ctypes_offset(out, out_offset)
    call("ocrk_strided_copy", sp, rows, cols, in_rs, in_cs, op, dtype_code(out.dtype), out_rs, out_cs, _stream(src))


def ctypes_offset(t, elems):
    return ctypes.c_void_p(t.data_ptr() + elems * t.element_size())


def slab_sum(slab, nslab, nc, ld, out, accumulate=True):
    _chk(slab, out)
    nb = _lib.lib().ocrk_slab_sum_workspace_size(nc)
    ws = _ws(nb, slab.device)
    call("ocrk_slab_sum", ptr(slab), int(nslab), int(nc), int(ld), ptr(out), int(accumulate), ptr(ws), nb,
         _stream(slab))


def _bias_parts(part, rows, nc, dbias, defer):
    if defer is None:
        slab_sum(part, rows, nc, nc, dbias)
    else:
        defer.append((lambda: slab_sum(part, rows, nc, nc, dbias), (part,)))


def colsum(x, M, N, out, accumulate=True):
    _chk(x, out)
    nb = _lib.lib().ocrk_colsum_workspace_size(M, N)
    ws = _ws(nb, x.device)
    call("ocrk_colsum", ptr(x), M, N, dtype_code(x.dtype), ptr(out), int(accumulate), ptr(ws), nb, _stream(x))


def relu_mask(dy, y, out_dtype, scale=1.0):
    _chk(dy, y)
    out = torch.empty(dy.shape, dtype=out_dtype, device=dy.device)
    call("ocrk_relu_mask", ptr(dy), ptr(y), dy.numel(), float(scale), ptr(out), dtype_code(out_dtype), _stream(dy))
    return out


def mul_scalar_(x, s):
    _chk(x, s)
    call("ocrk_mul_scalar", ptr(x), x.numel(), ptr(s), _stream(x))
    return x


def mean(x):
    _chk(x)
    out = torch.empty((), dtype=torch.float32, device=x.device)
    call("ocrk_mean", ptr(x), x.numel(), ptr(out), _stream(x))
    return out


def adam_(p, g, m, v, lr_t, beta1=0.9, beta2=0.999, eps=1e-8, grad_scale=1.0, zero_grad=False):
    _chk(p, g, m, v)
    call("ocrk_adam_ex", ptr(p), ptr(g), ptr(m), ptr(v), p.numel(), float(lr_t), float(beta1), float(beta2),
         float(eps), float(grad_scale), 1 if zero_grad else 0, _stream(p))


def ctc_loss(logits, labels, label_len, seq_len, grad_scale=1.0, need_grad=True, status=None):
    if logits.dtype != torch.float32:
        raise TypeError("ctc_loss takes float32 logits")
    _chk(logits, labels, label_len, seq_len)
    T, B, C = logits.shape
    Lmax = labels.shape[1] if labels.dim() == 2 else 0
    labels = labels.reshape(B, Lmax)
    if labels.numel() == 0:
        labels = torch.zeros(B, 1, dtype=torch.int32, device=logits.device)
        Lmax = 1
    nb = _lib.lib().ocrk_ctc_workspace_size(T, B, Lmax)
    ws = _ws(nb, logits.device)
    loss = torch.empty(B, dtype=torch.float32, device=logits.device)
    grad = torch.empty_like(logits) if need_grad else None
    if status is None:
        status = torch.empty(B, dtype=torch.int32, device=logits.device)
    call("ocrk_ctc_loss", ptr(logits), ptr(labels), ptr(label_len), ptr(seq_len), T, B, C, Lmax,
         float(grad_scale), ptr(loss), ptr(grad), ptr(status), ptr(status_word(logits.device)), ptr(ws), nb,
         _stream(logits))
    return loss, grad, status


def ctc_align(logits, labels, label_len, seq_len, status=None):
    if logits.dtype != torch.float32:
        raise TypeError("ctc_align takes float32 logits")
    _chk(logits, labels, label_len, seq_len)
    T, B, C = logits.shape
    Lmax = Lout = labels.shape[1] if labels.dim() == 2 else 0
    labels = labels.reshape(B, Lmax)
    if labels.numel() == 0:
        labels = torch.zeros(B, 1, dtype=torch.int32, device=logits.device)
        Lmax = 1
    nb = _lib.lib().ocrk_ctc_align_workspace_size(T, B, Lmax)
    ws = _ws(nb, logits.device)
    dev = logits.device
    frame_state = torch.empty(B, T, dtype=torch.int32, device=dev)
    span = torch.empty(B, Lmax, 2, dtype=torch.int32, device=dev)
    char_conf = torch.empty(B, Lmax, dtype=torch.float32, device=dev)
    path_logp = torch.empty(B, dtype=torch.float32, device=dev)
    if status is None:
        status = torch.empty(B, dtype=torch.int32, device=dev)
    call("ocrk_ctc_align", ptr(logits), ptr(labels), ptr(label_len), ptr(seq_len), T, B, C, Lmax,
         ptr(frame_state), ptr(span), ptr(char_conf), ptr(path_logp), ptr(status), ptr(status_word(dev)),
         ptr(ws), nb, _stream(logits))
    return frame_state, span[:, :Lout], char_conf[:, :Lout], path_logp, status


def ctc_lexicon_score(logits, seq_len, words, word_len, top_k=1, need_scores=True):
    if logits.dtype != torch.float32:
        raise TypeError("ctc_lexicon_score takes float32 logits")
    if words.dim() != 2 or word_len.dim() != 1 or words.shape[0] != word_len.shape[0]:
        raise ValueError("ctc_lexicon_score takes words [K, Wmax] and word_len [K]")
    if words.dtype != torch.int32 or word_len.dtype != torch.int32 or seq_len.dtype != torch.int32:
        raise TypeError("ctc_lexicon_score takes int32 words, word_len and seq_len")
    _chk(logits, seq_len, words, word_len)
    T, B, C = logits.shape
    n_words, Wmax = words.shape
    top_k = int(top_k)
    dev = logits.device
    nb = _lib.lib().ocrk_ctc_lexicon_workspace_size(T, B, C, n_words, Wmax)
    ws = _ws(nb, dev)
    logp = torch.empty(B, n_words, dtype=torch.float32, device=dev) if need_scores else None
    top_idx = torch.empty(B, max(top_k, 0), dtype=torch.int32, device=dev)
    top_logp = torch.empty(B, max(top_k, 0), dtype=torch.float32, device=dev)
    log_norm = torch.empty(B, dtype=torch.float32, device=dev)
    word_status = torch.empty(n_words, dtype=torch.int32, device=dev)
    call("ocrk_ctc_lexicon_score", ptr(logits), ptr(seq_len), T, B, C, ptr(words), ptr(word_len), n_words, Wmax,
         top_k, ptr(logp), ptr(top_idx), ptr(top_logp), ptr(log_norm), ptr(word_status), ptr(status_word(dev)),
         ptr(ws), nb, _stream(logits))
    return logp, top_idx, top_logp, log_norm, word_status


def ctc_spot(logits, seq_len, kw, kw_alt, kw_len):
    if logits.dtype != torch.float32:
        raise TypeError("ctc_spot takes float32 logits")
    if kw.dim() != 2 or kw_len.dim() != 1 or kw.shape[0] != kw_len.shape[0]:
        raise ValueError("ctc_spot takes kw [K, Wmax] and kw_len [K]")
    if kw_alt is not None and kw_alt.shape != kw.shape:
        raise ValueError("ctc_spot takes kw_alt of kw's shape")
    if any(t.dtype != torch.int32 for t in (kw, kw_len, seq_len) + (() if kw_alt is None else (kw_alt,))):
        raise TypeError("ctc_spot takes int32 kw, kw_alt, kw_len and seq_len")
    _chk(logits, seq_len, kw, kw_alt, kw_len)
    T, B, C = logits.shape
    n_kw, Wmax = kw.shape
    dev = logits.device
    nb = _lib.lib().ocrk_ctc_spot_workspace_size(T, B, C, n_kw, Wmax)
    ws = _ws(nb, dev)
    score = torch.empty(B, n_kw, dtype=torch.float32, device=dev)
    span = torch.empty(B, n_kw, 2, dtype=torch.int32, device=dev)
    kw_status = torch.empty(n_kw, dtype=torch.int32, device=dev)
    call("ocrk_ctc_spot", ptr(logits), ptr(seq_len), T, B, C, ptr(kw), ptr(kw_alt), ptr(kw_len), n_kw, Wmax,
         ptr(score), ptr(span), ptr(kw_status), ptr(status_word(dev)), ptr(ws), nb, _stream(logits))
    return score, span, kw_status


def ctc_greedy_decode(logits, seq_len, merge_repeated=True):
    if logits.dtype != torch.float32:
        raise TypeError("ctc_greedy_decode takes float32 logits")
    _chk(logits, seq_len)
    T, B, C = logits.shape
    out = torch.empty(B, T, dtype=torch.int64, device=logits.device)
    out_len = torch.empty(B, dtype=torch.int32, device=logits.device)
    neg = torch.empty(B, dtype=torch.float32, device=logits.device)
    call("ocrk_ctc_greedy_decode", ptr(logits), ptr(seq_len), T, B, C, int(bool(merge_repeated)),
         ptr(out), ptr(out_len), ptr(neg), _stream(logits))
    return out, out_len, neg


def ctc_beam_decode(logits, seq_len, beam_width=100, top_paths=1, merge_repeated=True):
    if logits.dtype != torch.float32:
        raise TypeError("ctc_beam_decode takes float32 logits")
    _chk(logits, seq_len)
    T, B, C = logits.shape
    dev = logits.device
    out = torch.empty(top_paths, B, T, dtype=torch.int64, device=dev)
    out_len = torch.empty(top_paths, B, dtype=torch.int32, device=dev)
    logp = torch.empty(B, top_paths, dtype=torch.float32, device=dev)
    nb = _lib.lib().ocrk_ctc_beam_workspace_size(T, B, int(beam_width))
# ... 20 lines not shown
```

cnn_lstm_ctc_ocr_amd/model.py:

```python
import contextlib

import numpy as np
import torch
import torch.distributed as dist

from . import kernels as K
from . import options
from .config import BN_EPS, BN_MOMENTUM, INFER, LAYER_PARAMS, POOLS, TRAIN, ModelConfig, rnn_size
from .params import ParamStore

layer_params = LAYER_PARAMS

_DEFAULT = []


@contextlib.contextmanager
def use_store(store):
    _DEFAULT.append(store)
    try:
        yield store
    finally:
        _DEFAULT.pop()


def default_store():
    if not _DEFAULT:
        raise RuntimeError("no ParamStore: pass store= or wrap the calls in model.use_store(store)")
    return _DEFAULT[-1]


def _grad_enabled(*ts):
    return torch.is_grad_enabled() and any(t is not None and t.requires_grad for t in ts)


def _conv_precision(exact):
    return K.f32_exact() if exact else contextlib.nullcontext()


def _conv_wgrad(split, x, dy, dw):
    if split:
        for xa, da in K.split_products(x, dy):
            K.conv3x3_bwd_weight(xa, da, dw)
    else:
        K.conv3x3_bwd_weight(x, dy, dw)


class _ConvBlock(torch.autograd.Function):

    @staticmethod
    def forward(ctx, x, store, k, training, *variables):
        ctx.exact = store.cfg.dtype == torch.float32 and store.f32_conv_exact
        with _conv_precision(ctx.exact):
            return _ConvBlock._forward(ctx, x, store, k, training)

    @staticmethod
    def _forward(ctx, x, store, k, training):
        dt = store.cfg.dtype
        odd, even = f"conv{2 * k - 1}", f"conv{2 * k}"
        P = store.params
        pe = f"convnet/{even}"
        ctx.bn_sync = None
        ctx.relu_bits = None
        ctx.c1_fused = bool(k == 1 and not ctx.exact and options.get("CONV1_FUSED"))
        ctx.pooled_bn = bool(options.get("POOLED_BN"))
        ctx.conv12_bwd = False
        zs = None
        if (k == 1 and training and dt == torch.bfloat16 and not ctx.exact and options.get("CONV1_FUSED")
                and options.get("CONV12_FUSED") and K.conv12_fwd_ok(x, dt)):
            ctx.conv12_bwd = bool(options.get("CONV12_BWD") and K.conv12_bwd_ok(x, dt))
            w_nk2, _ = store.conv_images(even, dt)
            y_odd, bits, z12, st12 = K.conv12_fwd(x, P["convnet/conv1/kernel"], P["convnet/conv1/bias"], w_nk2,
                                                  P[pe + "/bias"], want_y1=not ctx.conv12_bwd)
            ctx.relu_bits = bits if ctx.conv12_bwd or K.conv2_bwd_data_conv1_wgrad_ok(z12, x) else None
            zs = (z12, st12)
        elif k == 1 and training and dt == torch.bfloat16 and not ctx.exact and options.get("CONV1_FUSED"):
            y_odd, bits = K.conv1_fwd(x, P["convnet/conv1/kernel"], P["convnet/conv1/bias"], dt, relu_bits=True)
            ctx.relu_bits = bits if K.conv2_bwd_data_conv1_wgrad_ok(y_odd, x) else None
        elif k == 1:
            y_odd = K.conv1_fwd(x, P["convnet/conv1/kernel"], P["convnet/conv1/bias"], dt)
        else:
            w_nk, _ = store.conv_images(odd, dt)
            if (training and dt == torch.bfloat16 and not ctx.exact and options.get("RELU_BITS")
                    and K.relu_bits_ok(x.shape, x.shape[3], w_nk.shape[0], store.conv_images(even, dt)[0].shape[0],
                                       dt)):
                y_odd, ctx.relu_bits = K.conv3x3_fwd_relu_bits(x, w_nk, P[f"convnet/{odd}/bias"])
            else:
                y_odd = K.conv3x3_fwd(x, w_nk, P[f"convnet/{odd}/bias"], relu=True)
        B, H, W, _ = (y_odd if zs is None else zs[0]).shape
        M = B * H * W
        w_nk, _ = store.conv_images(even, dt)
        C = w_nk.shape[0]
        if training:
            if zs is not None:
                z, stats = zs
                trows = W
            elif K.conv3x3_fwd_rowstats_ok(y_odd, C):
                z, stats = K.conv3x3_fwd_rowstats(y_odd, w_nk, P[pe + "/bias"])
                trows = W
            else:
                stats = torch.empty(K.conv_stats_tiles(M), 2, C, dtype=torch.float32, device=x.device)
                z = K.conv3x3_fwd(y_odd, w_nk, P[pe + "/bias"], relu=False, stats=stats)
                trows = 128
            group = _bn_group(store)
            if group is not None:
                mean, invstd, count = K.bn_finalize_sync(stats, M, C, BN_EPS, BN_MOMENTUM,
                                                         store.stats[pe + "/batch_norm/moving_mean"],
                                                         store.stats[pe + "/batch_norm/moving_variance"], trows,
                                                         group)
                ctx.bn_sync = (group, count)
            else:
                mean, invstd = K.bn_finalize(stats, M, C, BN_EPS, BN_MOMENTUM,
                                             store.stats[pe + "/batch_norm/moving_mean"],
                                             store.stats[pe + "/batch_norm/moving_variance"], tile_rows=trows)
        else:
            z = K.conv3x3_fwd(y_odd, w_nk, P[pe + "/bias"], relu=False)
            mean, invstd = K.bn_infer_params(store.stats[pe + "/batch_norm/moving_mean"],
                                             store.stats[pe + "/batch_norm/moving_variance"], BN_EPS)
        p = K.bn_relu_pool_fwd(z, mean, invstd, P[pe + "/batch_norm/gamma"], P[pe + "/batch_norm/beta"],
                               POOLS[even], time_major=(k == 4))
        ctx.store, ctx.k = store, k
        ctx.save_for_backward(x, y_odd, z, mean, invstd, p)
        return p

    @staticmethod
    def backward(ctx, dp):
        with _conv_precision(ctx.exact):
            return _ConvBlock._backward(ctx, dp)

    @staticmethod
    def _backward(ctx, dp):
        store, k = ctx.store, ctx.k
        x, y_odd, z, mean, invstd, pooled = ctx.saved_tensors
        dt = store.cfg.dtype
        P, G = store.params, store.grads
        odd, even = f"conv{2 * k - 1}", f"conv{2 * k}"
        pe, po = f"convnet/{even}", f"convnet/{odd}"
        dp = dp.contiguous()
        if dp.dtype != dt:
            dp = K.cast(dp, dt)
        dz = K.bn_relu_pool_bwd(z, dp, mean, invstd, P[pe + "/batch_norm/gamma"], P[pe + "/batch_norm/beta"],
                                POOLS[even], dp_time_major=(k == 4),
                                dgamma=G[pe + "/batch_norm/gamma"], dbeta=G[pe + "/batch_norm/beta"],
                                dbias=G[pe + "/bias"],
                                sync=ctx.bn_sync,
                                pooled=pooled if ctx.bn_sync is None and ctx.pooled_bn else None)
        B, H, W, C = dz.shape
        if k > 1:
            with _conv_side(store, y_odd, dz, *_conv_late_tensors(store)):
                _conv_late_run(store)
                _conv_wgrad(ctx.exact, y_odd, dz, G[pe + "/kernel"])
        _, w_bwd = store.conv_images(even, dt)
        if ctx.conv12_bwd:
            if store.conv_late:
                with _conv_side(store, *_conv_late_tensors(store)):
                    _conv_late_run(store)
            K.conv12_bwd(dz, w_bwd, x, P["convnet/conv1/kernel"], P["convnet/conv1/bias"], G[pe + "/kernel"],
                         G[po + "/kernel"], G[po + "/bias"], relu_bits=ctx.relu_bits)
            store.join()
            return (None, None, None, None) + (None,) * (len(ctx.needs_input_grad) - 4)
        if ctx.c1_fused and K.conv2_bwd_data_conv1_wgrad_ok(dz, x):
            with _conv_side(store, y_odd, dz, *_conv_late_tensors(store)):
                _conv_late_run(store)
                _conv_wgrad(ctx.exact, y_odd, dz, G[pe + "/kernel"])
            bits = ctx.relu_bits
            K.conv2_bwd_data_conv1_wgrad(dz, w_bwd, None if bits is not None else y_odd, x, G[po + "/kernel"],
                                         G[po + "/bias"], relu_bits=bits)
            store.join()
            return (None, None, None, None) + (None,) * (len(ctx.needs_input_grad) - 4)
        if k > 1 and ctx.relu_bits is not None:
            dy_odd = K.conv3x3_bwd_data(dz, w_bwd, dbias=G[po + "/bias"], relu_bits=ctx.relu_bits)
        else:
            dy_odd = K.conv3x3_bwd_data(dz, w_bwd, relu_mask=y_odd, dbias=G[po + "/bias"] if k > 1 else None)
        dx = None
        if k == 1:
            with _conv_side(store, x, dy_odd, *_conv_late_tensors(store)):
                _conv_late_run(store)
                K.conv1_bwd_weight(x, dy_odd, G[po + "/kernel"], G[po + "/bias"])
            _conv_wgrad(ctx.exact, y_odd, dz, G[pe + "/kernel"])
            store.join()
        else:
            if k > 2 and options.get("CONV_SIDE") and options.get("SIDE_STREAM"):
                store.conv_late.append((lambda x=x, d=dy_odd, dw=G[po + "/kernel"], ex=ctx.exact:
                                        _conv_wgrad(ex, x, d, dw), (x, dy_odd)))
            else:
                with _conv_side(store, x, dy_odd):
                    _conv_wgrad(ctx.exact, x, dy_odd, G[po + "/kernel"])
            if ctx.needs_input_grad[0]:
                _, w_bwd_odd = store.conv_images(odd, dt)
                dx = K.conv3x3_bwd_data(dy_odd, w_bwd_odd)
        return (dx, None, None, None) + (None,) * (len(ctx.needs_input_grad) - 4)


def _bn_group(store):
    g = store.bn_group
    if g is None or not (dist.is_available() and dist.is_initialized()):
        return None
    return g if dist.get_world_size(g) > 1 else None


def _block_variables(store, k):
    names = [f"convnet/conv{2 * k - 1}/kernel", f"convnet/conv{2 * k - 1}/bias",
             f"convnet/conv{2 * k}/kernel", f"convnet/conv{2 * k}/bias",
             f"convnet/conv{2 * k}/batch_norm/gamma", f"convnet/conv{2 * k}/batch_norm/beta"]
    return [store.params[n] for n in names]


def convnet_layers(inputs, widths, mode, store=None):
    store = store or default_store()
    training = mode == TRAIN
    x = inputs
    if x.dim() == 4:
        if x.shape[-1] != 1:
            raise ValueError("inputs must be [batch, 32, width, 1]")
        x = x[..., 0]
    x = x.contiguous()
    if x.dtype not in (torch.uint8, store.cfg.dtype):
        x = K.cast(x, store.cfg.dtype)
    track = torch.is_grad_enabled() and training
    h = x
    for k in (1, 2, 3, 4):
        variables = _block_variables(store, k) if track else []
        if track:
            for v in variables:
                v.requires_grad_(True)
        h = _ConvBlock.apply(h, store, k, training, *variables)
    if not isinstance(widths, torch.Tensor):
        widths = torch.as_tensor(np.asarray(widths), dtype=torch.int32)
    widths = widths.to(device=h.device, dtype=torch.int32)
    sequence_length = K.seq_len(widths)
    return h.transpose(0, 1), sequence_length


_SIDE_STREAMS = {}


def _new_side_stream(dev, lane):
    return torch.cuda.Stream(device=dev)


class side_work:

    def __init__(self, store, *tensors, lane="side"):
        self.store, self.tensors, self.lane = store, tensors, lane

    def __enter__(self):
        dev = self.store.device
        if not options.get("SIDE_STREAM"):
            self.side = None
            return self
        side = _SIDE_STREAMS.get((dev, self.lane))
        if side is None:
            side = _SIDE_STREAMS[(dev, self.lane)] = _new_side_stream(dev, self.lane)
        self.side = side
        K.fork(side, torch.cuda.current_stream(dev))
        self.ctx = torch.cuda.stream(side)
        self.ctx.__enter__()
        return self

    def __exit__(self, *exc):
        if self.side is None:
            return False
        done = torch.cuda.Event()
        done.record(self.side)
        self.ctx.__exit__(*exc)
        for t in self.tensors:
            t.record_stream(self.side)
        self.store.pending.append(done)
        return False


def _conv_late_tensors(store):
    return tuple(t for _, ts in store.conv_late for t in ts)


def _conv_late_run(store):
    late, store.conv_late = store.conv_late, []
    for fn, _ in late:
        fn()


def _conv_side(store, *tensors):
    if not options.get("CONV_SIDE"):
        return contextlib.nullcontext()
    return side_work(store, *tensors)


class _BiLSTM(torch.autograd.Function):

    @staticmethod
    def forward(ctx, x, seq_len, store, layer, *variables):
        dt = store.cfg.dtype
        T, B, n_in = x.shape
        H = store.cfg.rnn_sizes[layer - 1]
        wxT, _wx, whT, _wh, bias = store.lstm_images(layer, dt)
        gx = K.gemm(x.view(T * B, n_in), wxT, trans_b=True, bias=bias, out_dtype=dt)
        out, hprev, cprev, acts = K.lstm_fwd(gx, whT, seq_len, T, B, H, dt, save=any(ctx.needs_input_grad))
        ctx.store, ctx.layer, ctx.H = store, layer, H
        ctx.save_for_backward(x, seq_len, hprev, cprev, acts)
        return out

    @staticmethod
    def backward(ctx, dout):
        store, layer, H = ctx.store, ctx.layer, ctx.H
        x, seq_len, hprev, cprev, acts = ctx.saved_tensors
        dt = store.cfg.dtype
        T, B, n_in = x.shape
        G4 = 4 * H
        dout = dout.contiguous()
        if dout.dtype != dt:
            dout = K.cast(dout, dt)
        _wxT, wx, _whT, wh, _bias = store.lstm_images(layer, dt)
        dG = K.lstm_bwd(wh, seq_len, dout, cprev, acts, T, B, H, dbias=store.flat_bias_pair_grad(layer))
        R = T * B
        dx = None
        pre = f"rnn/bdrnn{layer}"
        with side_work(store, x, hprev, dG):
            gf, gb = store.grads[f"{pre}/fw/lstm_cell/kernel"], store.grads[f"{pre}/bw/lstm_cell/kernel"]
            sk = gf.numel()
            if dt == torch.float32 and not K.f32_mode_exact():
                (xh, xl), (hh, hl), (gh, gl) = K.split_bf16(x), K.split_bf16(hprev), K.split_bf16(dG)
                passes = [(xh, hh, gh), (xh, hh, gl), (xl, hl, gh)]
            else:
                passes = [(x, hprev, dG)]
            if gb.data_ptr() == gf.data_ptr() + 4 * sk:
                for _xa, ha, ga in passes:
                    K.gemm(ha.view(R, 2 * H), ga.view(R, 2 * G4), trans_a=True, out=gf[n_in:], accumulate=True,
                           M=H, N=G4, K=R, lda=2 * H, ldb=2 * G4, ldc=G4, batch=2, stride_a=H, stride_b=G4,
                           stride_c=sk, splits=_splits(H, G4, R, batch=2, items=_tn_items(layer)))
                for xa, _ha, ga in passes:
                    K.gemm(xa, ga.view(R, 2 * G4), trans_a=True, out=gf, accumulate=True, M=n_in, N=G4, K=R,
                           lda=n_in, ldb=2 * G4, ldc=G4, batch=2, stride_a=0, stride_b=G4, stride_c=sk,
                           splits=_splits(n_in, G4, R, batch=2, items=_tn_items(layer)))
            else:
                for xa, ha, ga in passes:
                    dg = ga.view(R, 2 * G4)
                    for d, gk in enumerate((gf, gb)):
                        dgd = dg[:, d * G4:]
                        K.gemm(xa, dgd, trans_a=True, out=gk, accumulate=True, M=n_in, N=G4, K=R, lda=n_in,
                               ldb=2 * G4, ldc=G4, splits=_splits(n_in, G4, R, items=_tn_items(layer)))
                        K.gemm(ha.view(R, 2 * H)[:, d * H:], dgd, trans_a=True, out=gk[n_in:], accumulate=True,
                               M=H, N=G4, K=R, lda=2 * H, ldb=2 * G4, ldc=G4,
                               splits=_splits(H, G4, R, items=_tn_items(layer)))
        if ctx.needs_input_grad[0]:
            dx = K.gemm(dG.view(R, 2 * G4), wx, trans_b=True, out_dtype=dt).view(T, B, n_in)
        return (dx,) + (None,) * (len(ctx.needs_input_grad) - 1)


class _BiGRU(torch.autograd.Function):

    @staticmethod
    def forward(ctx, x, seq_len, store, layer, *variables):
        dt = store.cfg.dtype
        T, B, n_in = x.shape
        H = store.cfg.rnn_sizes[layer - 1]
        wxT, _wx, whgT, whcT, _whg, _whc, bias = store.gru_images(layer, dt)
        gx = K.gemm(x.view(T * B, n_in), wxT, trans_b=True, bias=bias, out_dtype=dt)
        out, hprev, rh, acts = K.gru_fwd(gx, whgT, whcT, seq_len, T, B, H, dt)
        ctx.store, ctx.layer, ctx.H = store, layer, H
        ctx.save_for_backward(x, seq_len, hprev, rh, acts)
        return out

    @staticmethod
    def backward(ctx, dout):
        store, layer, H = ctx.store, ctx.layer, ctx.H
        x, seq_len, hprev, rh, acts = ctx.saved_tensors
        dt = store.cfg.dtype
        T, B, n_in = x.shape
        G2, G3 = 2 * H, 3 * H
        dout = dout.contiguous()
        if dout.dtype != dt:
            dout = K.cast(dout, dt)
        _wxT, wx, _whgT, _whcT, whg, whc, _bias = store.gru_images(layer, dt)
        dG = K.gru_bwd(whg, whc, seq_len, dout, hprev, acts, T, B, H, dbias=store.gru_bias_cat_grad(layer))
        pre = f"rnn/bdrnn{layer}"
        R = T * B
        side = side_work(store, x, hprev, rh, dG)
        side.__enter__()
        gf, gb = store.grads[f"{pre}/fw/gru_cell/gates/kernel"], store.grads[f"{pre}/bw/gru_cell/gates/kernel"]
        cf, cb = store.grads[f"{pre}/fw/gru_cell/candidate/kernel"], store.grads[f"{pre}/bw/gru_cell/candidate/kernel"]
        sk = (gb.data_ptr() - gf.data_ptr()) // 4
        batched = sk > 0 and cb.data_ptr() - cf.data_ptr() == 4 * sk
        if batched:
            dg = dG.view(R, 2 * G3)
            hp, rhv = hprev.view(R, 2 * H), rh.view(R, 2 * H)
            K.gemm(x, dg, trans_a=True, out=gf, accumulate=True, M=n_in, N=G2, K=R, lda=n_in, ldb=2 * G3,
                   ldc=G2, batch=2, stride_a=0, stride_b=G3, stride_c=sk, splits=_splits(n_in, G2, R, batch=2, items=_tn_items(layer)))
            K.gemm(hp, dg, trans_a=True, out=gf[n_in:], accumulate=True, M=H, N=G2, K=R, lda=2 * H, ldb=2 * G3,
                   ldc=G2, batch=2, stride_a=H, stride_b=G3, stride_c=sk, splits=_splits(H, G2, R, batch=2, items=_tn_items(layer)))
            K.gemm(x, dg[:, G2:], trans_a=True, out=cf, accumulate=True, M=n_in, N=H, K=R, lda=n_in,
                   ldb=2 * G3, ldc=H, batch=2, stride_a=0, stride_b=G3, stride_c=sk,
                   splits=_splits(n_in, H, R, batch=2, items=_tn_items(layer)))
            K.gemm(rhv, dg[:, G2:], trans_a=True, out=cf[n_in:], accumulate=True, M=H, N=H, K=R, lda=2 * H,
                   ldb=2 * G3, ldc=H, batch=2, stride_a=H, stride_b=G3, stride_c=sk, splits=_splits(H, H, R, batch=2, items=_tn_items(layer)))
        for d, dn in enumerate(() if batched else ("fw", "bw")):
            gk = store.grads[f"{pre}/{dn}/gru_cell/gates/kernel"]
            ck = store.grads[f"{pre}/{dn}/gru_cell/candidate/kernel"]
            dgg = dG.view(R, 2 * G3)[:, d * G3:]
            dgc = dG.view(R, 2 * G3)[:, d * G3 + G2:]
            hp = hprev.view(R, 2 * H)[:, d * H:]
            rhd = rh.view(R, 2 * H)[:, d * H:]
            K.gemm(x, dgg, trans_a=True, out=gk, accumulate=True, M=n_in, N=G2, K=R, lda=n_in,
                   ldb=2 * G3, ldc=G2, splits=_splits(n_in, G2, R, items=_tn_items(layer)))
            K.gemm(hp, dgg, trans_a=True, out=gk[n_in:], accumulate=True, M=H, N=G2, K=R, lda=2 * H,
                   ldb=2 * G3, ldc=G2, splits=_splits(H, G2, R, items=_tn_items(layer)))
            K.gemm(x, dgc, trans_a=True, out=ck, accumulate=True, M=n_in, N=H, K=R, lda=n_in,
                   ldb=2 * G3, ldc=H, splits=_splits(n_in, H, R, items=_tn_items(layer)))
            K.gemm(rhd, dgc, trans_a=True, out=ck[n_in:], accumulate=True, M=H, N=H, K=R, lda=2 * H,
                   ldb=2 * G3, ldc=H, splits=_splits(H, H, R, items=_tn_items(layer)))
        side.__exit__(None, None, None)
        dx = None
        if ctx.needs_input_grad[0]:
            dx = K.gemm(dG.view(R, 2 * G3), wx, trans_b=True, out_dtype=dt).view(T, B, n_in)
        return (dx,) + (None,) * (len(ctx.needs_input_grad) - 1)




def _tn_items(layer):
    if layer == 1:
        return options.get("TN_ITEMS_L1")
    return options.get("TN_ITEMS")


def _splits(M, N, Kdim, batch=1, items=None):
    if M >= 256 and N >= 256:
        tiles = -(-M // 256) * -(-N // 256) * batch
        return int(max(1, min((items or options.get("TN_ITEMS")) // tiles, Kdim // 1024)))
    tiles = -(-M // 128) * -(-N // 128) * batch
    return int(max(1, min(-(-512 // tiles), Kdim // 2048)))


class _Logits(torch.autograd.Function):

    @staticmethod
    def forward(ctx, x, store, *variables):
        dt = store.cfg.dtype
        T, B, D = x.shape
        wT = store.logits_image_t(dt)
        logits = K.gemm(x.view(T * B, D), wT, trans_b=True, bias=store.params["rnn/logits/bias"], relu=True)
        logits = logits.view(T, B, -1)
        ctx.store = store
        ctx.save_for_backward(x, logits)
        return logits

    @staticmethod
    def backward(ctx, dlogits):
        store = ctx.store
        x, logits = ctx.saved_tensors
        dt = store.cfg.dtype
        T, B, D = x.shape
        C = logits.shape[-1]
        R = T * B
        dpre = K.relu_mask(dlogits.contiguous(), logits, dt)
        with side_work(store, x, dpre):
            split = dt == torch.float32 and not K.f32_mode_exact() and x.numel() % 8 == 0 and dpre.numel() % 8 == 0
            for xa, pa in (K.split_products(x, dpre) if split else [(x, dpre)]):
                K.gemm(xa, pa, trans_a=True, out=store.grads["rnn/logits/kernel"], accumulate=True,
                       M=D, N=C, K=R, lda=D, ldb=C, ldc=C, splits=_splits(D, C, R))
            K.colsum(dpre, R, C, store.grads["rnn/logits/bias"])
        dx = None
        if ctx.needs_input_grad[0]:
            dx = K.gemm(dpre.view(R, C), store.logits_image(dt), trans_b=True, out_dtype=dt).view(T, B, D)
        return (dx,) + (None,) * (len(ctx.needs_input_grad) - 1)


def rnn_layers(features, sequence_length, num_classes, store=None):
    store = store or default_store()
    cfg = store.cfg
    if num_classes != cfg.num_classes:
        raise ValueError(f"store was built for {cfg.num_classes} classes, got {num_classes}")
    x = features.transpose(0, 1)
    if not x.is_contiguous():
        x = x.contiguous()
    if x.dtype != cfg.dtype:
        x = K.cast(x, cfg.dtype)
    sequence_length = sequence_length.to(device=x.device, dtype=torch.int32).contiguous()
    B = x.shape[1]
    mult = 64 if cfg.dtype == torch.bfloat16 else 32
    Bp = -(-B // mult) * mult
    if Bp != B:
        x = torch.cat([x, x.new_zeros(x.shape[0], Bp - B, x.shape[2])], dim=1)
        sequence_length = torch.cat([sequence_length, sequence_length.new_zeros(Bp - B)])
    track = torch.is_grad_enabled() and x.requires_grad
    for layer in range(1, len(cfg.rnn_sizes) + 1):
        variables = []
        if track:
            pre = f"rnn/bdrnn{layer}"
            leaves = ("lstm_cell/kernel", "lstm_cell/bias") if cfg.cell == "lstm" else \
                ("gru_cell/gates/kernel", "gru_cell/gates/bias", "gru_cell/candidate/kernel", "gru_cell/candidate/bias")
            variables = [store.params[f"{pre}/{d}/{v}"] for d in ("fw", "bw") for v in leaves]
        op = _BiLSTM if cfg.cell == "lstm" else _BiGRU
        x = op.apply(x, sequence_length, store, layer, *variables)
    variables = [store.params["rnn/logits/kernel"], store.params["rnn/logits/bias"]] if track else []
    logits = _Logits.apply(x, store, *variables)
    return logits if Bp == B else logits[:, :B]


class _CTCLoss(torch.autograd.Function):
    @staticmethod
    def forward(ctx, logits, labels, label_len, seq_len):
        B = logits.shape[1]
        loss_b, grad, status = K.ctc_loss(logits.contiguous(), labels, label_len, seq_len,
                                          grad_scale=1.0 / max(B, 1), need_grad=logits.requires_grad)
        ctx.save_for_backward(grad if grad is not None else loss_b)
        ctx.status = status
        return K.mean(loss_b)

    @staticmethod
    def backward(ctx, g):
        (grad,) = ctx.saved_tensors
        if _UNIT_ARMED[0] and g.data_ptr() in _UNIT_SEEDS and g.dtype == torch.float32:
            return grad, None, None, None
        return K.mul_scalar_(grad, g.to(torch.float32).contiguous()), None, None, None


_UNIT_SEEDS = {}
_UNIT_BY_DEVICE = {}
_UNIT_ARMED = [False]


def _unit_seed(device):
    t = _UNIT_BY_DEVICE.get(device)
    if t is None:
        t = _UNIT_BY_DEVICE[device] = torch.ones((), dtype=torch.float32, device=device)
        _UNIT_SEEDS[t.data_ptr()] = t
    return t
# ... 87 lines not shown
```

cnn_lstm_ctc_ocr_amd/options.py:

```python
import contextlib
import os

_HOST_DEFAULTS = {
    "LSTM_PERSISTENT": 1,
    "F32_TRAIN_EXACT": 0,
    "SIDE_STREAM": 1,
    "CONV_SIDE": 1,
    "CONV12_FUSED": 1,
    "RELU_BITS": 1,
    "POOLED_BN": 1,
    "CONV1_FUSED": 1,
    "CONV12_BWD": 1,
    "TN_ITEMS": 256,
    "TN_ITEMS_L1": 160,
}
KERNEL_OPTIONS = ("CONV_DIRECT", "CONV_ROWS", "CONV_ROWS_WIDE", "CONV_WGRAD_BLOCKS", "LSTM_SPIN_LIMIT",
                  "PERSIST_LATE", "LSTM_BWD_R16", "CTC_LDS",
                  "PP_PERSIST_NK", "NT_F32_EXACT", "NT_F32_MASK",
                  "NT_F32_X6", "BEAM_WAVE", "BN_BWD_BLOCKS", "BN_ROUTE", "BN_ROUTE_SEG", "BN_ROUTE_NCH", "CONV_TN_ITEMS", "CONV_TN4_ITEMS",
                  "CONV_WGRAD_CUS", "F32_MFMA", "GEMM_NT", "GEMM_NT_STAGED", "GEMM_PP", "GEMM_PPTN", "PP_MIN_N", "GEMM_TN",
                  "LSTM_DMA", "LSTM_BWD_DMA", "LSTM_FWD_R16", "NT_TAP_UNIFORM")


def _env_int(name, default):
    v = os.environ.get("OCRK_" + name)
    if v is None or v == "":
        return default
    try:
        return int(v)
    except ValueError:
        raise ValueError(f"OCRK_{name}={v!r}: an integer is expected") from None


_HOST = {k: _env_int(k, d) for k, d in _HOST_DEFAULTS.items()}


def get(name):
    if name in _HOST:
        return _HOST[name]
    if name in KERNEL_OPTIONS:
        import ctypes

        from . import _lib
        v = ctypes.c_int64()
        _lib.call("ocrk_get_option", name.encode(), ctypes.byref(v))
        return v.value
    raise KeyError(f"unknown option {name!r}")


def set(name, value):
    value = int(value)
    if name in _HOST:
        prev, _HOST[name] = _HOST[name], value
        return prev
    if name in KERNEL_OPTIONS:
        import ctypes

        from . import _lib
        prev = ctypes.c_int64()
        _lib.call("ocrk_set_option", name.encode(), value, ctypes.byref(prev))
        return prev.value
    raise KeyError(f"unknown option {name!r}")


@contextlib.contextmanager
def override(**values):
    prev = []
    try:
        for k, v in values.items():
            prev.append((k, set(k, v)))
        yield
    finally:
        for k, v in reversed(prev):
            set(k, v)
```

cnn_lstm_ctc_ocr_amd/params.py:

```python

import numpy as np
import torch

from . import kernels as K
from .config import LAYER_PARAMS, ModelConfig

_ALIGN = 64


def param_shapes(cfg):
    out = []
    cin = 1
    for filters, k, _pad, name, bn in LAYER_PARAMS:
        out.append((f"convnet/{name}/kernel", (k, k, cin, filters), True))
        out.append((f"convnet/{name}/bias", (filters,), True))
        if bn:
            out.append((f"convnet/{name}/batch_norm/gamma", (filters,), True))
            out.append((f"convnet/{name}/batch_norm/beta", (filters,), True))
            out.append((f"convnet/{name}/batch_norm/moving_mean", (filters,), False))
            out.append((f"convnet/{name}/batch_norm/moving_variance", (filters,), False))
        cin = filters
    n_in = cin
    for li, H in enumerate(cfg.rnn_sizes, start=1):
        pre = f"rnn/bdrnn{li}"
        if cfg.cell == "lstm":
            for d in ("fw", "bw"):
                out.append((f"{pre}/{d}/lstm_cell/kernel", (n_in + H, 4 * H), True))
            for d in ("fw", "bw"):
                out.append((f"{pre}/{d}/lstm_cell/bias", (4 * H,), True))
        else:
            for d in ("fw", "bw"):
                out.append((f"{pre}/{d}/gru_cell/gates/kernel", (n_in + H, 2 * H), True))
                out.append((f"{pre}/{d}/gru_cell/candidate/kernel", (n_in + H, H), True))
            for d in ("fw", "bw"):
                out.append((f"{pre}/{d}/gru_cell/gates/bias", (2 * H,), True))
                out.append((f"{pre}/{d}/gru_cell/candidate/bias", (H,), True))
        n_in = 2 * H
    out.append(("rnn/logits/kernel", (n_in, cfg.num_classes + 1), True))
    out.append(("rnn/logits/bias", (cfg.num_classes + 1,), True))
    return out


def creation_order(cfg):
    names = [n for n, _s, _t in param_shapes(cfg)]
    out = [n for n in names if not n.startswith("rnn/bdrnn")]
    rnn = []
    for li in range(1, len(cfg.rnn_sizes) + 1):
        pre = f"rnn/bdrnn{li}"
        for d in ("fw", "bw"):
            if cfg.cell == "lstm":
                rnn += [f"{pre}/{d}/lstm_cell/kernel", f"{pre}/{d}/lstm_cell/bias"]
            else:
                rnn += [f"{pre}/{d}/gru_cell/{v}" for v in
                        ("gates/kernel", "gates/bias", "candidate/kernel", "candidate/bias")]
    i = out.index("rnn/logits/kernel")
    return out[:i] + rnn + out[i:]


def _trunc_normal(rng, shape, std):
    x = rng.standard_normal(shape)
    bad = np.abs(x) > 2
    while bad.any():
        x[bad] = rng.standard_normal(int(bad.sum()))
        bad = np.abs(x) > 2
    return x * std


def reference_init(cfg, seed=0):
    rng = np.random.default_rng(seed)
    vals = {}
    shapes = {n: sh for n, sh, _t in param_shapes(cfg)}
    for name in creation_order(cfg):
        shape = shapes[name]
        leaf = name.rsplit("/", 1)[1]
        if name.startswith("convnet") and leaf == "kernel":
            v = _trunc_normal(rng, shape, np.sqrt(2.6 / (shape[0] * shape[1] * shape[2])))
        elif name == "rnn/logits/kernel":
            v = _trunc_normal(rng, shape, np.sqrt(2.6 / shape[0]))
        elif "gru_cell" in name or ("lstm_cell" in name and leaf == "kernel"):
            v = _trunc_normal(rng, shape, 0.01)
        elif leaf in ("gamma", "moving_variance"):
            v = np.ones(shape)
        else:
            v = np.zeros(shape)
        vals[name] = v.astype(np.float32)
    return vals


class ParamStore:
    def __init__(self, cfg=None, device="cuda", seed=0, values=None):
        self.cfg = cfg or ModelConfig()
        self.device = torch.device(device)
        self.spec = param_shapes(self.cfg)
        self.offsets = {}
        sizes = {True: 0, False: 0}
        for name, shape, tr in self.spec:
            n = int(np.prod(shape))
            self.offsets[name] = (tr, sizes[tr], shape)
            sizes[tr] += (n + _ALIGN - 1) // _ALIGN * _ALIGN
        self.n_trainable = sum(int(np.prod(s)) for _, s, tr in self.spec if tr)
        self.flat = torch.zeros(sizes[True], dtype=torch.float32, device=self.device)
        self.flat_grad = torch.zeros_like(self.flat)
        self.flat_stats = torch.zeros(max(sizes[False], _ALIGN), dtype=torch.float32, device=self.device)
        self.params, self.grads, self.stats = {}, {}, {}
        for name, shape, tr in self.spec:
            _, off, _ = self.offsets[name]
            n = int(np.prod(shape))
            if tr:
                self.params[name] = self.flat[off:off + n].view(shape)
                self.grads[name] = self.flat_grad[off:off + n].view(shape)
            else:
                self.stats[name] = self.flat_stats[off:off + n].view(shape)
        self.version = 0
        self._images = {}
        self.pending = []
        self.conv_late = []
        self.bn_group = None
        self.f32_conv_exact = False
        self.load_state_dict(values if values is not None else reference_init(self.cfg, seed))

    def state_dict(self):
        out = {k: v.detach().cpu().numpy().copy() for k, v in self.params.items()}
        out.update({k: v.detach().cpu().numpy().copy() for k, v in self.stats.items()})
        return out

    def load_state_dict(self, values):
        for name, _shape, _tr in self.spec:
            if name not in values:
                raise KeyError(f"missing variable {name}")
            dst = self.params.get(name, self.stats.get(name))
            src = torch.as_tensor(np.asarray(values[name], dtype=np.float32))
            if tuple(src.shape) != tuple(dst.shape):
                raise ValueError(f"{name}: shape {tuple(src.shape)} != {tuple(dst.shape)}")
            dst.copy_(src.to(self.device))
        self.bump()

    def save(self, path):
        np.savez(path, **{k.replace("/", "__"): v for k, v in self.state_dict().items()})

    def load(self, path):
        with np.load(path, allow_pickle=False) as z:
            self.load_state_dict({k.replace("__", "/"): z[k] for k in z.files})

    def zero_grad(self):
        self.join()
        self.flat_grad.zero_()

    def join(self):
        while self.conv_late:
            fn, _tensors = self.conv_late.pop(0)
            fn()
        if self.pending:
            cur = torch.cuda.current_stream(self.device)
            for ev in self.pending:
                K.wait_mark(cur, ev)
            self.pending.clear()

    def bump(self):
        self.version += 1
        self._images.clear()
        self._plan_fresh = False

    def images(self, key, builder):
        plan = self._plan_for(key)
        if plan is not None:
            if not self._plan_fresh:
                K.copy_batch(plan["table"], plan["njobs"], plan["tiles"], self.flat)
                self._plan_fresh = True
            return plan["images"][key]
        img = self._images.get(key)
        if img is None:
            img = builder()
            self._images[key] = img
        return img

    def _plan_for(self, key):
        if self.device.type != "cuda":
            return None
        dtype = key[-1]
        if dtype != self.cfg.dtype:
            return None
        plan = getattr(self, "_plan", None)
        if plan is None:
            plan = self._plan = self._build_plan(dtype)
            self._plan_fresh = False
        return plan if key in plan["images"] else None

    def _build_plan(self, dtype):
        dev = self.device
        esz = torch.empty(0, dtype=dtype).element_size()
        code = K.dtype_code(dtype)
        jobs, images = [], {}

        def job(src, s_off, rows, cols, in_rs, dst, d_off, out_rs, transpose):
            jobs.append([src.data_ptr() + 4 * s_off, dst.data_ptr() + esz * d_off, rows, cols, in_rs, out_rs, 0,
                         int(transpose) | (code << 32)])

        for li in range(2, 9):
            w = self.params[f"convnet/conv{li}/kernel"]
            kh, kw, cin, cout = w.shape
            w_nk = torch.empty(cout, kh * kw * cin, dtype=dtype, device=dev)
            w_bwd = torch.empty(cin, kh * kw * cout, dtype=dtype, device=dev)
            job(w, 0, kh * kw * cin, cout, cout, w_nk, 0, kh * kw * cin, True)
            for t in range(kh * kw):
                job(w, t * cin * cout, cin, cout, cout, w_bwd, t * cout, kh * kw * cout, False)
            images[("conv", f"conv{li}", dtype)] = (w_nk, w_bwd)
        for layer in range(1, len(self.cfg.rnn_sizes) + 1):
            pre = f"rnn/bdrnn{layer}"
            if self.cfg.cell == "lstm":
                kf = self.params[f"{pre}/fw/lstm_cell/kernel"]
                rows, G = kf.shape
                H = G // 4
                n_in = rows - H
                wxT = torch.empty(2 * G, n_in, dtype=dtype, device=dev)
                wx = torch.empty(n_in, 2 * G, dtype=dtype, device=dev)
                whT = torch.empty(2, G, H, dtype=dtype, device=dev)
                wh = torch.empty(2, H, G, dtype=dtype, device=dev)
                for d, dn in enumerate(("fw", "bw")):
                    k = self.params[f"{pre}/{dn}/lstm_cell/kernel"]
                    job(k, 0, n_in, G, G, wxT, d * G * n_in, n_in, True)
                    job(k, 0, n_in, G, G, wx, d * G, 2 * G, False)
                    job(k, n_in * G, H, G, G, whT, d * G * H, H, True)
                    job(k, n_in * G, H, G, G, wh, d * H * G, G, False)
                images[("lstm", layer, dtype)] = (wxT, wx, whT, wh, self.flat_bias_pair(layer))
            else:
                gk = self.params[f"{pre}/fw/gru_cell/gates/kernel"]
                rows, G2 = gk.shape
                H = G2 // 2
                n_in = rows - H
                G3 = 3 * H
                wxT = torch.empty(2 * G3, n_in, dtype=dtype, device=dev)
                wx = torch.empty(n_in, 2 * G3, dtype=dtype, device=dev)
                whgT = torch.empty(2, G2, H, dtype=dtype, device=dev)
                whcT = torch.empty(2, H, H, dtype=dtype, device=dev)
                whg = torch.empty(2, H, G2, dtype=dtype, device=dev)
                whc = torch.empty(2, H, H, dtype=dtype, device=dev)
                for d, dn in enumerate(("fw", "bw")):
                    g = self.params[f"{pre}/{dn}/gru_cell/gates/kernel"]
                    c = self.params[f"{pre}/{dn}/gru_cell/candidate/kernel"]
                    job(g, 0, n_in, G2, G2, wxT, d * G3 * n_in, n_in, True)
                    job(c, 0, n_in, H, H, wxT, (d * G3 + G2) * n_in, n_in, True)
                    job(g, 0, n_in, G2, G2, wx, d * G3, 2 * G3, False)
                    job(c, 0, n_in, H, H, wx, d * G3 + G2, 2 * G3, False)
                    job(g, n_in * G2, H, G2, G2, whgT, d * G2 * H, H, True)
                    job(c, n_in * H, H, H, H, whcT, d * H * H, H, True)
                    job(g, n_in * G2, H, G2, G2, whg, d * H * G2, G2, False)
                    job(c, n_in * H, H, H, H, whc, d * H * H, H, False)
                images[("gru", layer, dtype)] = (wxT, wx, whgT, whcT, whg, whc, self.gru_bias_cat(layer))
        lk = self.params["rnn/logits/kernel"]
        limg = torch.empty(lk.shape, dtype=dtype, device=dev)
        limgT = torch.empty(lk.shape[1], lk.shape[0], dtype=dtype, device=dev)
        job(lk, 0, lk.shape[0], lk.shape[1], lk.shape[1], limg, 0, lk.shape[1], False)
        job(lk, 0, lk.shape[0], lk.shape[1], lk.shape[1], limgT, 0, lk.shape[0], True)
        images[("logits", dtype)] = limg
        images[("logitsT", dtype)] = limgT
        tiles = 0
        for j in jobs:
            j[6] = tiles
            tiles += -(-j[2] // 32) * -(-j[3] // 32)
        table = torch.tensor(jobs, dtype=torch.int64).to(dev)
        return {"table": table, "njobs": len(jobs), "tiles": tiles, "images": images}

    def conv_images(self, name, dtype):
        def build():
            w = self.params[f"convnet/{name}/kernel"]
            kh, kw, cin, cout = w.shape
            w_nk = K.permute3(w, kh * kw * cin, cout, 1, dtype).view(cout, kh * kw * cin)
            w_bwd = K.permute3(w, kh * kw, cin, cout, dtype).view(cin, kh * kw * cout)
            return w_nk, w_bwd
        return self.images(("conv", name, dtype), build)

    def lstm_images(self, layer, dtype):
        def build():
            pre = f"rnn/bdrnn{layer}"
            kf = self.params[f"{pre}/fw/lstm_cell/kernel"]
            rows, G = kf.shape
            H = G // 4
            n_in = rows - H
            dev = kf.device
            wxT = torch.empty(2 * G, n_in, dtype=dtype, device=dev)
            wx = torch.empty(n_in, 2 * G, dtype=dtype, device=dev)
            whT = torch.empty(2, G, H, dtype=dtype, device=dev)
            wh = torch.empty(2, H, G, dtype=dtype, device=dev)
            for d, dn in enumerate(("fw", "bw")):
                k = self.params[f"{pre}/{dn}/lstm_cell/kernel"]
                K.strided_copy(k, n_in, G, G, 1, wxT, 1, n_in, out_offset=d * G * n_in)
                K.strided_copy(k, n_in, G, G, 1, wx, 2 * G, 1, out_offset=d * G)
                K.strided_copy(k, H, G, G, 1, whT, 1, H, out_offset=d * G * H, in_offset=n_in * G)
                K.strided_copy(k, H, G, G, 1, wh, G, 1, out_offset=d * H * G, in_offset=n_in * G)
            bias = self.flat_bias_pair(layer)
            return wxT, wx, whT, wh, bias
        return self.images(("lstm", layer, dtype), build)

    def flat_bias_pair(self, layer):
        pre = f"rnn/bdrnn{layer}"
        bf = self.params[f"{pre}/fw/lstm_cell/bias"]
        _, off, _ = self.offsets[f"{pre}/fw/lstm_cell/bias"]
        _, off2, _ = self.offsets[f"{pre}/bw/lstm_cell/bias"]
        n = bf.numel()
        if off2 != off + n:
            raise RuntimeError("LSTM biases must be adjacent in the flat buffer")
# ... 66 lines not shown
```

cnn_lstm_ctc_ocr_amd/train.py:

```python
import collections
import math
import time

import torch
import torch.distributed as dist

from . import _lib
from . import kernels as K
from . import options
from . import model as _model
from .config import TRAIN
from .model import check_feasible_host, convnet_layers, ctc_loss_layer, dense_labels, host_labels, rnn_layers




class GradBuckets:

    def __init__(self, store, group=None, comm=None, force=False):
        self.store, self.group, self.comm, self.force = store, group, comm, bool(force)
        rnn = [off for name, (tr, off, _s) in store.offsets.items() if tr and name.startswith("rnn/")]
        self.split = min(rnn) if rnn else store.flat_grad.numel()
        self.work = None
        self._stream = None
        self._comm_world = comm.info()[0] if comm is not None else None

    def world(self):
        if self.comm is not None:
            return self._comm_world
        if not (dist.is_available() and dist.is_initialized()):
            return 1
        return dist.get_world_size(self.group)

    def active(self):
        return self.world() > 1 or (self.force and (self.comm is not None or
                                                    (dist.is_available() and dist.is_initialized())))

    def _sum_(self, t, async_op=False):
        if self.comm is not None:
            self.comm.allreduce_(t)
            return None
        return dist.all_reduce(t, op=dist.ReduceOp.SUM, group=self.group, async_op=async_op)

    def rnn_ready(self, *_):
        if not self.active() or self.work is not None:
            return
        g = self.store.flat_grad
        if g.is_cuda:
            if self._stream is None:
                self._stream = torch.cuda.Stream(g.device)
            K.fork(self._stream, torch.cuda.current_stream(g.device))
            for ev in self.store.pending:
                K.wait_mark(self._stream, ev)
            with torch.cuda.stream(self._stream):
                self.work = self._sum_(g[self.split:], async_op=True)
                if self.work is None:
                    self.work = "stream"
                g.record_stream(self._stream)
        else:
            self.work = self._sum_(g[self.split:], async_op=True)

    def finish(self):
        if not self.active():
            return 1.0
        world = self.world()
        g = self.store.flat_grad
        if self.work is None:
            self._sum_(g)
        else:
            self._sum_(g[:self.split])
            if self.work == "stream":
                torch.cuda.current_stream(g.device).wait_stream(self._stream)
            else:
                self.work.wait()
            self.work = None
        if g.is_cuda:
            or_allreduce_status(K.status_word(g.device), self.group, comm=self.comm)
        return 1.0 / world


_STATUS_BITS = {}


def or_allreduce_status(word, group=None, comm=None):
    key = word.device
    if key not in _STATUS_BITS:
        _STATUS_BITS[key] = torch.arange(31, dtype=torch.int32, device=word.device)
    bits = _STATUS_BITS[key]
    vec = torch.bitwise_and(torch.bitwise_right_shift(word, bits), 1)
    if comm is not None:
        comm.allreduce_(vec)
        vec = (vec > 0).to(torch.int32)
    else:
        dist.all_reduce(vec, op=dist.ReduceOp.MAX, group=group)
    word.bitwise_or_(torch.bitwise_left_shift(vec, bits).sum(dtype=torch.int32).view(1))
    return word


def allreduce_mean_scale(flat_grad, group=None):
    if not (dist.is_available() and dist.is_initialized()):
        return 1.0
    world = dist.get_world_size(group)
    if world > 1:
        dist.all_reduce(flat_grad, op=dist.ReduceOp.SUM, group=group)
    return 1.0 / world


class Trainer:

    def __init__(self, store, learning_rate=1e-4, momentum=0.9, decay_rate=0.9, decay_steps=2 ** 16,
                 decay_staircase=False, beta2=0.999, epsilon=1e-8, process_group=None, global_step=0,
                 summary=None, summary_every=100, sync_bn=False, comm=None, force_exchange=False):
        self.store = store
        self.sync_bn = bool(sync_bn)
        self.summary = summary
        self.summary_every = max(1, int(summary_every))
        self._summary_mark = None
        self.base_lr = learning_rate
        self.beta1 = momentum
        self.beta2 = beta2
        self.eps = epsilon
        self.decay_rate = decay_rate
        self.decay_steps = decay_steps
        self.staircase = decay_staircase
        self.group = process_group
        self.global_step = global_step
        self.m = torch.zeros_like(store.flat)
        self.v = torch.zeros_like(store.flat)
        self._grads_zeroed = False
        self._status_host = None
        self._status_ev = None
        self._status_stream = None
        self._status_ring = collections.deque()
        self.status_lag = 2
        self.buckets = GradBuckets(store, process_group, comm=comm, force=force_exchange)
        self.overlap_allreduce = True

    def learning_rate(self, step=None):
        step = self.global_step if step is None else step
        e = step / self.decay_steps
        if self.staircase:
            e = math.floor(e)
        return self.base_lr * self.decay_rate ** e

    def _bn_group(self):
        if not self.sync_bn or not (dist.is_available() and dist.is_initialized()):
            return None
        return self.group if self.group is not None else dist.group.WORLD

    def world_size(self):
        if self.buckets.comm is not None:
            return self.buckets.world()
        if dist.is_available() and dist.is_initialized():
            return dist.get_world_size(self.group)
        return 1

    def loss_and_grads(self, image, width, label):
        store = self.store
        if store.cfg.dtype != torch.float32:
            return self._loss_and_grads(image, width, label)
        if options.get("F32_TRAIN_EXACT"):
            with K.f32_exact():
                return self._loss_and_grads(image, width, label)
        prev, store.f32_conv_exact = store.f32_conv_exact, True
        try:
            return self._loss_and_grads(image, width, label)
        finally:
            store.f32_conv_exact = prev

    def _loss_and_grads(self, image, width, label):
        store = self.store
        prev_group, store.bn_group = store.bn_group, self._bn_group()
        try:
            return self._forward_backward(image, width, label)
        finally:
            store.bn_group = prev_group

    def _forward_backward(self, image, width, label):
        store = self.store
        if host_labels(label) and not (isinstance(width, torch.Tensor) and width.is_cuda):
            check_feasible_host(label, width)
        if self._grads_zeroed and not (store.device.type == "cuda" and torch.cuda.is_current_stream_capturing()):
            store.join()
        else:
            store.zero_grad()
        self._grads_zeroed = False
        features, seq_len = convnet_layers(image, width, TRAIN, store)
        if self.overlap_allreduce and features.requires_grad and self.buckets.active() and \
                not (features.is_cuda and torch.cuda.is_current_stream_capturing()):
            features.register_hook(self.buckets.rnn_ready)
        logits = rnn_layers(features, seq_len, store.cfg.num_classes, store)
        loss = ctc_loss_layer(logits, label, seq_len)
        if loss.dtype == torch.float32:
            _model.unit_backward(loss)
        else:
            loss.backward()
        return loss

    def reduce_gradients(self):
        self.store.join()
        return self.buckets.finish()

    def apply_gradients(self):
        store = self.store
        grad_scale = self.reduce_gradients()
        t = self.global_step + 1
        lr = self.learning_rate()
        lr_t = lr * math.sqrt(1 - self.beta2 ** t) / (1 - self.beta1 ** t)
        zero = store.device.type == "cuda"
        K.adam_(store.flat, store.flat_grad, self.m, self.v, lr_t, self.beta1, self.beta2, self.eps,
                grad_scale=grad_scale, zero_grad=zero)
        self._grads_zeroed = zero
        store.bump()
        self.global_step += 1

    def step(self, image, width, label):
        self.poll_status()
        lr = self.learning_rate()
        loss = self.loss_and_grads(image, width, label)
        self.apply_gradients()
        self.post_status()
        self.summarize(loss, lr, int(image.shape[0]))
        return loss

    def summarize(self, loss, lr, batch):
        if self.summary is None:
            return
        if self._summary_mark is not None and self.global_step % self.summary_every:
            return
        dev = self.store.device
        if dev.type == "cuda":
            now = torch.cuda.Event(enable_timing=True)
            now.record(torch.cuda.current_stream(dev))
        else:
            now = time.perf_counter()
        if self._summary_mark is None:
            self._summary_mark = (self.global_step, now)
        if self.global_step % self.summary_every:
            return
        s0, t0 = self._summary_mark
        crops = (self.global_step - s0) * batch * self.world_size()
        vals = {"learning_rate": lr, "loss": loss}
        if self.global_step > s0:
            if dev.type == "cuda":
                vals["crops_per_sec"] = lambda: round(crops / max(t0.elapsed_time(now) / 1e3, 1e-9), 2)
            elif now > t0:
                vals["crops_per_sec"] = round(crops / (now - t0), 2)
        self.summary.scalars(self.global_step, **vals)
        self._summary_mark = (self.global_step, now)

    def post_status(self):
        dev = self.store.device
        if dev.type == "cuda" and self.buckets.active():
            buf = torch.zeros(1, dtype=torch.int32, pin_memory=True)
            buf.copy_(K.status_word(dev), non_blocking=True)
            ev = torch.cuda.Event()
            ev.record(torch.cuda.current_stream(dev))
            self._status_ring.append((ev, buf))
            return
        if dev.type != "cuda" or self._status_ev is not None:
            return
        if self._status_host is None:
            self._status_host = torch.zeros(1, dtype=torch.int32, pin_memory=True)
            self._status_stream = torch.cuda.Stream(dev)
        cur = torch.cuda.current_stream(dev)
        K.fork(self._status_stream, cur)
        with torch.cuda.stream(self._status_stream):
            self._status_host.copy_(K.status_word(dev), non_blocking=True)
            self._status_ev = torch.cuda.Event()
            self._status_ev.record(self._status_stream)

    def poll_status(self):
        while len(self._status_ring) > self.status_lag:
            ev, buf = self._status_ring.popleft()
            ev.synchronize()
            v = int(buf[0])
            if v:
                self._status_ring.clear()
                K.clear_status(self.store.device, v)
                _lib.raise_for_status(v)
        if self._status_ev is None or not self._status_ev.query():
            return
        v = int(self._status_host[0])
        self._status_ev = None
        if v:
            K.clear_status(self.store.device, v)
            _lib.raise_for_status(v)

    def check_status(self):
        self._status_ev = None
        self._status_ring.clear()
        if self.store.device.type == "cuda":
            K.check_status(self.store.device)

    def graphed(self, image, width, label, max_label_len=None, before_capture=None):
        return GraphedStep(self, image, width, label, max_label_len, before_capture)


class GraphedStep:

    def __init__(self, trainer, image, width, label, max_label_len=None, before_capture=None):
        store = trainer.store
        dev = store.device
        if trainer._bn_group() is not None and trainer.world_size() > 1:
            raise NotImplementedError("GraphedStep with Trainer(sync_bn=True): run eager steps")
        self.trainer = trainer
        self.B = int(image.shape[0])
        self.image = image.detach().to(dev).clone()
        self.width = torch.as_tensor(width).to(device=dev, dtype=torch.int32).clone()
        lab, ln = dense_labels(label, self.B, dev)
        lmax = int(max_label_len or lab.shape[1])
        if lab.shape[1] > lmax:
            raise ValueError(f"labels of {lab.shape[1]} > max_label_len={lmax}")
        self.labels = torch.zeros(self.B, lmax, dtype=torch.int32, device=dev)
        self.labels[:, :lab.shape[1]].copy_(lab)
        self.label_len = ln.clone()
        self.stream = torch.cuda.Stream(dev)
        self.stream.wait_stream(torch.cuda.current_stream(dev))
        moving = store.flat_stats.clone()
        overlap, trainer.overlap_allreduce = trainer.overlap_allreduce, False
        with torch.cuda.stream(self.stream):
            trainer.loss_and_grads(self.image, self.width, (self.labels, self.label_len))
            store.flat_stats.copy_(moving)
            store.join()
        trainer.overlap_allreduce = overlap
        self.stream.synchronize()
        store.bump()
        if before_capture is not None:
            before_capture()
        self.graph = torch.cuda.CUDAGraph()
        with torch.cuda.graph(self.graph, stream=self.stream):
            self.loss = trainer.loss_and_grads(self.image, self.width, (self.labels, self.label_len))
        torch.cuda.current_stream(dev).wait_stream(self.stream)

    def load(self, image=None, width=None, label=None):
# ... 27 lines not shown
```

include/ocrk.h:

```cpp
#ifndef OCRK_H_
#define OCRK_H_

#include <stddef.h>
#include <stdint.h>

#ifdef __cplusplus
extern "C" {
#endif

#define OCRK_ABI_VERSION 7

enum ocrk_status {
    OCRK_OK = 0,
    OCRK_ERR_INVALID_ARG = 1,
    OCRK_ERR_HIP = 2,
    OCRK_ERR_INFEASIBLE = 3
};

enum ocrk_dtype { OCRK_F32 = 0, OCRK_BF16 = 1 };

int ocrk_set_f32_gemm_mode(int mode);
int ocrk_f32_gemm_exact(void);

enum ocrk_device_status {
    OCRK_STATUS_CTC_INFEASIBLE = 1 << 1,
    OCRK_STATUS_CTC_BAD_LENGTH = 1 << 2,
    OCRK_STATUS_CTC_BAD_LABEL = 1 << 3,
    OCRK_STATUS_LSTM_FWD_TIMEOUT = 1 << 4,
    OCRK_STATUS_LSTM_BWD_TIMEOUT = 1 << 5,
    OCRK_STATUS_LSTM_CENSUS = 1 << 6
};

int ocrk_status_clear(unsigned* status_word, uint32_t bits, void* stream);

int ocrk_version(void);
const char* ocrk_last_error(void);

int ocrk_set_option(const char* name, int64_t value, int64_t* prev);

int ocrk_split_bf16(const float* x, int64_t n, void* hi, void* lo, void* stream);
int ocrk_get_option(const char* name, int64_t* value);

int ocrk_preprocess(const uint8_t* in, int64_t n, void* out, int dtype, void* stream);

size_t ocrk_ctc_workspace_size(int T, int B, int max_label_len);
int ocrk_ctc_loss(const float* logits, const int* labels, const int* label_len, const int* seq_len,
                  int T, int B, int C, int max_label_len, float grad_scale, float* loss, float* grad,
                  int* status, unsigned* status_word, void* ws, size_t ws_bytes, void* stream);

size_t ocrk_ctc_align_workspace_size(int T, int B, int max_label_len);
int ocrk_ctc_align(const float* logits, const int* labels, const int* label_len, const int* seq_len,
                   int T, int B, int C, int max_label_len, int* frame_state, int* span, float* char_conf,
                   float* path_logp, int* status, uint32_t* status_word, void* ws, size_t ws_bytes,
                   void* stream);

size_t ocrk_ctc_lexicon_workspace_size(int T, int B, int C, int n_words, int max_word_len);
int ocrk_ctc_lexicon_score(const float* logits, const int* seq_len, int T, int B, int C,
                           const int* words, const int* word_len, int n_words, int max_word_len,
                           int top_k, float* logp, int* top_idx, float* top_logp, float* log_norm,
                           int* word_status, uint32_t* status_word, void* ws, size_t ws_bytes, void* stream);

size_t ocrk_ctc_spot_workspace_size(int T, int B, int C, int n_kw, int max_kw_len);
int ocrk_ctc_spot(const float* logits, const int* seq_len, int T, int B, int C, const int* kw,
                  const int* kw_alt, const int* kw_len, int n_kw, int max_kw_len, float* score,
                  int* span, int* kw_status, uint32_t* status_word, void* ws, size_t ws_bytes,
                  void* stream);

int ocrk_ctc_greedy_decode(const float* logits, const int* seq_len, int T, int B, int C,
                           int merge_repeated, int64_t* out, int* out_len, float* neg_sum_logits,
                           void* stream);


size_t ocrk_ctc_beam_workspace_size(int T, int B, int beam_width);
int ocrk_ctc_beam_decode(const float* logits, const int* seq_len, int T, int B, int C, int beam_width,
                         int top_paths, int merge_repeated, int64_t* out, int* out_len, float* log_probs,
                         void* ws, size_t ws_bytes, void* stream);

int ocrk_edit_distance(const int64_t* hyp, const int* hyp_len, int hyp_stride, const int* label,
                       const int* label_len, int label_stride, int B, float* dist, int* totals,
                       void* stream);

int ocrk_conv1_fwd(const void* x, int x_is_u8, int B, int H, int W, const float* w, const float* bias,
                   int cout, void* y, int dtype, void* stream);
int ocrk_conv1_fwd_relu_bits(const void* x, int x_is_u8, int B, int H, int W, const float* w, const float* bias,
                             int cout, void* y, void* relu_bits, int dtype, void* stream);
int ocrk_conv12_fwd_supported(int B, int IH, int IW, int dtype);
int ocrk_conv12_fwd(const void* x, int x_is_u8, int B, int IH, int IW, const float* w1, const float* b1,
                    const void* w_nk2, const float* b2, void* y1, void* relu_bits, void* z, float* stats, int dtype,
                    void* stream);
size_t ocrk_conv1_wgrad_workspace_size(int B, int H, int W, int cout);
int ocrk_conv1_bwd_weight(const void* x, int x_is_u8, const void* dz, int B, int H, int W, int cout,
                          float* dw, float* db, int accumulate, void* ws, size_t ws_bytes, int dtype,
                          void* stream);
int ocrk_conv2_bwd_data_conv1_wgrad_supported(int B, int H, int W, int cin, int cout, int dtype);
size_t ocrk_conv2_bwd_data_conv1_wgrad_workspace_size(int B, int H, int W);
int ocrk_conv2_bwd_data_conv1_wgrad(const void* dz, int B, int H, int W, const void* w_bwd, const void* relu_mask,
                                    const void* relu_bits, const void* x, int x_is_u8, float* dw, float* db,
                                    int accumulate, void* ws, size_t ws_bytes, int dtype, void* stream);

int ocrk_conv12_bwd_supported(int B, int H, int W, int dtype);
size_t ocrk_conv12_bwd_workspace_size(int B, int H, int W);
int ocrk_conv12_bwd(const void* dz, int B, int H, int W, const void* w_bwd, const void* relu_mask,
                    const void* relu_bits, const void* x, int x_is_u8, const float* w1, const float* b1, float* dw2,
                    float* dw1, float* db1, int accumulate, void* ws, size_t ws_bytes, int dtype, void* stream);

size_t ocrk_conv_stats_tiles(int64_t M);
int ocrk_conv3x3_fwd_rowstats_supported(int B, int H, int W, int cin, int cout);
int ocrk_conv3x3_fwd_rowstats(const void* x, int B, int H, int W, int cin, const void* w_nk, const float* bias,
                              int cout, void* y, int relu, float* stats, void* stream);
int ocrk_conv3x3_fwd(const void* x, int B, int H, int W, int cin, const void* w_nk, const float* bias,
                     int cout, void* y, int y_dtype, int relu, float* stats, int dtype, void* stream);
size_t ocrk_conv3x3_bwd_data_workspace_size(int B, int H, int W, int cin);
int ocrk_conv3x3_bwd_data(const void* dy, int B, int H, int W, int cout, const void* w_bwd, int cin,
                          void* dx, const void* relu_mask, float* dbias, int accumulate, void* ws,
                          size_t ws_bytes, int dtype, void* stream);
int ocrk_conv3x3_fwd_relu_bits_supported(int B, int H, int W, int cin, int cout, int dtype);
int ocrk_conv3x3_fwd_relu_bits(const void* x, int B, int H, int W, int cin, const void* w_nk, const float* bias,
                               int cout, void* y, void* relu_bits, int dtype, void* stream);
int ocrk_conv3x3_bwd_data_bits_supported(int B, int H, int W, int cout, int cin, int dtype);
int ocrk_conv3x3_bwd_data_bits(const void* dy, int B, int H, int W, int cout, const void* w_bwd, int cin,
                               void* dx, const void* relu_bits, float* dbias, int accumulate, void* ws,
                               size_t ws_bytes, int dtype, void* stream);
int ocrk_conv3x3_bwd_data_bits_slab(const void* dy, int B, int H, int W, int cout, const void* w_bwd, int cin,
                                    void* dx, const void* relu_bits, float* slab, int dtype, void* stream);
int ocrk_conv3x3_bwd_data_slab(const void* dy, int B, int H, int W, int cout, const void* w_bwd, int cin,
                               void* dx, const void* relu_mask, float* slab, int dtype, void* stream);
size_t ocrk_conv3x3_wgrad_workspace_size(int B, int H, int W, int cin, int cout);
int ocrk_conv3x3_bwd_weight(const void* x, const void* dy, int B, int H, int W, int cin, int cout,
                            float* dw, int accumulate, void* ws, size_t ws_bytes, int dtype, void* stream);

size_t ocrk_bn_finalize_workspace_size(int tiles, int C);
int ocrk_bn_finalize_tiles(const float* stats, int tiles, int tile_rows, int64_t M, int C, float eps,
                           float momentum, float* mean, float* invstd, float* moving_mean, float* moving_var,
                           void* ws, size_t ws_bytes, void* stream);
int ocrk_bn_finalize(const float* stats, int tiles, int64_t M, int C, float eps, float momentum,
                     float* mean, float* invstd, float* moving_mean, float* moving_var, void* ws, size_t ws_bytes,
                     void* stream);
int ocrk_bn_moments(const float* stats, int tiles, int tile_rows, int64_t M, int C, double* moments, void* ws,
                    size_t ws_bytes, void* stream);
int ocrk_bn_finalize_moments(const double* moments, int C, float eps, float momentum, float* mean, float* invstd,
                             float* moving_mean, float* moving_var, void* stream);
int ocrk_bn_infer_params(const float* moving_mean, const float* moving_var, int C, float eps,
                         float* mean, float* invstd, void* stream);
int ocrk_bn_relu_pool_fwd(const void* z, int B, int H, int W, int C, const float* mean,
                          const float* invstd, const float* gamma, const float* beta, int kh, int kw,
                          int sh, int sw, void* out, int time_major, int dtype, void* stream);
size_t ocrk_bn_bwd_workspace_size(int B, int H, int W, int C);
int ocrk_bn_relu_pool_bwd(const void* z, const void* dp, int B, int H, int W, int C, const float* mean,
                          const float* invstd, const float* gamma, const float* beta, int kh, int kw,
                          int sh, int sw, int dp_time_major, void* dz, float* dgamma, float* dbeta,
                          float* dbias, int accumulate, void* ws, size_t ws_bytes, int dtype, void* stream);
size_t ocrk_bn_bwd_bias_slab_rows(int B, int H, int W, int C, int kh, int kw, int sh, int sw);
int ocrk_bn_relu_pool_bwd_slab(const void* z, const void* dp, int B, int H, int W, int C, const float* mean,
                               const float* invstd, const float* gamma, const float* beta, int kh, int kw,
                               int sh, int sw, int dp_time_major, void* dz, float* dgamma, float* dbeta,
                               int accumulate, float* bias_slab, void* ws, size_t ws_bytes, int dtype,
                               void* stream);
size_t ocrk_bn_bwd_pooled_bias_slab_rows(int B, int H, int W, int C, int kh, int kw, int sh, int sw);
int ocrk_bn_relu_pool_bwd_pooled(const void* z, const void* pooled, const void* dp, int B, int H, int W, int C,
                                 const float* mean, const float* invstd, const float* gamma, const float* beta,
                                 int kh, int kw, int sh, int sw, int dp_time_major, void* dz, float* dgamma,
                                 float* dbeta, float* dbias, int accumulate, float* bias_slab, void* ws,
                                 size_t ws_bytes, int dtype, void* stream);
int ocrk_bn_relu_pool_bwd_reduce(const void* z, const void* dp, int B, int H, int W, int C, const float* mean,
                                 const float* invstd, const float* gamma, const float* beta, int kh, int kw,
                                 int sh, int sw, int dp_time_major, float* dgamma, float* dbeta, int accumulate,
                                 float* dsum, void* ws, size_t ws_bytes, int dtype, void* stream);
int ocrk_bn_relu_pool_bwd_apply(const void* z, const void* dp, int B, int H, int W, int C, const float* mean,
                                const float* invstd, const float* gamma, const float* beta, int kh, int kw,
                                int sh, int sw, int dp_time_major, const float* dsum, const double* count,
                                void* dz, float* dbias, int accumulate, float* bias_slab, void* ws,
                                size_t ws_bytes, int dtype, void* stream);

int ocrk_lstm_fwd_step(const void* gx, const void* whT, const void* h_in, void* h_out, float* c_state,
                       const int* seq_len, int s, int T, int B, int H, void* out, void* hprev_t,
                       float* cprev_t, void* acts_t, int dtype, void* stream);
int ocrk_lstm_bwd_step(const void* wh, const void* dg_in, void* dg_out, float* dc_state, const int* seq_len,
                       int s, int T, int B, int H, const void* dout, const float* cprev_t,
                       const void* acts_t, void* dG_t, int dtype, void* stream);
int ocrk_lstm_fwd_persistent_supported(int B, int H);
size_t ocrk_lstm_fwd_persistent_workspace_size(int B, int H);
int ocrk_lstm_fwd_persistent(const void* gx, const void* whT, const int* seq_len, int T, int B, int H,
                             void* out, void* hprev_t, float* cprev_t, void* acts_t, unsigned* err,
                             unsigned* flags, void* ws, size_t ws_bytes, void* stream);
int ocrk_lstm_fwd_persistent_f32_supported(int B, int H);
size_t ocrk_lstm_fwd_persistent_f32_workspace_size(int B, int H);
size_t ocrk_lstm_fwd_persistent_f32_flags_size(int B, int H);
int ocrk_lstm_fwd_persistent_f32(const float* gx, const float* whT, const int* seq_len, int T, int B, int H,
                                 float* out, float* hprev_t, float* cprev_t, float* acts_t, unsigned* err,
                                 unsigned* flags, void* ws, size_t ws_bytes, void* stream);
int ocrk_lstm_bwd_persistent_f32_supported(int B, int H);
size_t ocrk_lstm_bwd_persistent_f32_workspace_size(int B, int H);
int ocrk_lstm_bwd_persistent_f32(const float* wh, const int* seq_len, int T, int B, int H, const float* dout,
                                 const float* cprev_t, const float* acts_t, float* dG_t, unsigned* err,
                                 unsigned* flags, float* dbias_part, void* ws, size_t ws_bytes, void* stream);
int ocrk_lstm_bwd_persistent_supported(int B, int H);
int ocrk_lstm_bwd_persistent_slices(int B, int H);
size_t ocrk_lstm_bwd_persistent_workspace_size(int B, int H);
int ocrk_lstm_bwd_persistent(const void* wh, const int* seq_len, int T, int B, int H, const void* dout,
                             const float* cprev_t, const void* acts_t, void* dG_t, unsigned* err,
                             unsigned* flags, float* dbias_part, void* ws, size_t ws_bytes, void* stream);
int ocrk_gru_fwd_step(const void* gx, const void* whgT, const void* whcT, void* h, void* rh,
                      const int* seq_len, int s, int T, int B, int H, void* out, void* hprev_t, void* rh_t,
                      void* acts_t, int dtype, void* stream);
int ocrk_gru_fwd(const void* gx, const void* whgT, const void* whcT, void* h, void* rh, const int* seq_len,
                 int T, int B, int H, void* out, void* hprev_t, void* rh_t, void* acts_t, int dtype,
                 void* stream);
int ocrk_gru_bwd(const void* whg, const void* whc, void* dzg, void* dzc, float* dh_tot, float* direct,
                 const int* seq_len, int T, int B, int H, const void* dout, const void* hprev_t,
                 const void* acts_t, void* dG_t, int dtype, void* stream);
int ocrk_gru_fwd_persistent_supported(int B, int H);
size_t ocrk_gru_fwd_persistent_workspace_size(int B, int H);
int ocrk_gru_fwd_persistent(const void* gx, const void* whgT, const void* whcT, const int* seq_len, int T, int B,
                            int H, void* out, void* hprev_t, void* rh_t, void* acts_t, unsigned* err,
                            unsigned* flags, void* ws, size_t ws_bytes, void* stream);
int ocrk_gru_bwd_persistent_supported(int B, int H);
size_t ocrk_gru_bwd_persistent_workspace_size(int B, int H);
int ocrk_gru_bwd_persistent(const void* whg, const void* whc, const int* seq_len, int T, int B, int H,
                            const void* dout, const void* hprev_t, const void* acts_t, void* dG_t, unsigned* err,
                            unsigned* flags, float* dbias_part, void* ws, size_t ws_bytes, void* stream);
size_t ocrk_persistent_flags_size(int B, int H);
int ocrk_lstm_fwd(const void* gx, const void* whT, void* h_state, float* c_state, const int* seq_len,
                  int T, int B, int H, void* out, void* hprev_t, float* cprev_t, void* acts_t, int dtype,
                  void* stream);
int ocrk_lstm_bwd(const void* wh, void* dg_state, float* dc_state, const int* seq_len, int T, int B, int H,
                  const void* dout, const float* cprev_t, const void* acts_t, void* dG_t, int dtype,
                  void* stream);

size_t ocrk_gemm_workspace_size(int M, int N, int batch, int splits);
int ocrk_gemm(int trans_a, int trans_b, int M, int N, int K, float alpha, const void* A, int64_t lda,
              int64_t stride_a, const void* B, int64_t ldb, int64_t stride_b, void* C, int64_t ldc,
              int64_t stride_c, int c_dtype, const float* bias, int relu, int accumulate, int batch,
              int dtype, int splits, void* ws, size_t ws_bytes, void* stream);

int ocrk_adam(float* p, const float* g, float* m, float* v, int64_t n, float lr_t, float beta1,
              float beta2, float eps, float grad_scale, void* stream);
#define OCRK_ADAM_ZERO_GRAD 1u
int ocrk_adam_ex(float* p, float* g, float* m, float* v, int64_t n, float lr_t, float beta1,
                 float beta2, float eps, float grad_scale, unsigned flags, void* stream);

int ocrk_copy_batch(const void* jobs, int njobs, int64_t total_tiles, void* stream);
int ocrk_cast(const void* in, int in_dtype, void* out, int out_dtype, int64_t n, void* stream);
int ocrk_permute3(const void* in, int in_dtype, int d0, int d1, int d2, void* out, int out_dtype,
                  void* stream);
int ocrk_strided_copy(const float* in, int64_t rows, int64_t cols, int64_t in_rs, int64_t in_cs, void* out,
                      int out_dtype, int64_t out_rs, int64_t out_cs, void* stream);
size_t ocrk_colsum_workspace_size(int64_t M, int N);
int ocrk_colsum(const void* in, int64_t M, int N, int dtype, float* out, int accumulate, void* ws,
                size_t ws_bytes, void* stream);
size_t ocrk_slab_sum_workspace_size(int nc);
int ocrk_slab_sum(const float* slab, int nslab, int nc, int ld, float* out, int accumulate, void* ws,
                  size_t ws_bytes, void* stream);
int ocrk_relu_mask(const float* dy, const float* y, int64_t n, float scale, void* out, int out_dtype,
                   void* stream);
int ocrk_mul_scalar(float* x, int64_t n, const float* s, void* stream);
int ocrk_mean(const float* x, int n, float* out, void* stream);
int ocrk_seq_len(const int* widths, int n, int* out, void* stream);

int ocrk_timer_create(void** ev);
int ocrk_timer_record(void* ev, void* stream);
int ocrk_timer_elapsed(void* ev0, void* ev1, float* ms);
int ocrk_timer_destroy(void* ev);

uint32_t ocrk_crc32c(const void* data, size_t n, uint32_t crc);

#ifdef __cplusplus
}
#endif
#endif
```

Measured before the change: 54290.

## Batch deferred bias/gamma slab reductions into one multi-job kernel launch

Adds a batched slab-sum kernel that reads a table of up to 32 reduction jobs and assigns each block to one job. Conv, BN and RNN backward passes now queue their per-layer bias and gamma partial sums in a LateSums collector, which is flushed at join or all-reduce time. The conv1 gradient reduction is also split out so it can be deferred. This removes many small kernel launches and Python callbacks per train step, at the cost of more host bookkeeping, overlap checks on destinations, and a longer lifetime for the slab buffers.

```diff
diff --git a/cnn_lstm_ctc_ocr_amd/_lib.py b/cnn_lstm_ctc_ocr_amd/_lib.py
--- a/cnn_lstm_ctc_ocr_amd/_lib.py
+++ b/cnn_lstm_ctc_ocr_amd/_lib.py
@@ -57,6 +57,7 @@
     "ocrk_conv12_bwd_supported": [_i32, _i32, _i32, _i32],
     "ocrk_conv12_bwd_workspace_size": [_i32, _i32, _i32],
     "ocrk_conv12_bwd": [_p, _i32, _i32, _i32, _p, _p, _p, _p, _i32, _p, _p, _p, _p, _p, _i32, _p, _sz, _i32, _p],
+    "ocrk_conv12_bwd_parts": [_p, _i32, _i32, _i32, _p, _p, _p, _p, _i32, _p, _p, _p, _p, _i32, _p, _sz, _i32, _p],
     "ocrk_conv12_fwd_supported": [_i32, _i32, _i32, _i32],
     "ocrk_conv12_fwd": [_p, _i32, _i32, _i32, _i32, _p, _p, _p, _p, _p, _p, _p, _p, _i32, _p],
     "ocrk_conv1_fwd_relu_bits": [_p, _i32, _i32, _i32, _i32, _p, _p, _i32, _p, _p, _i32, _p],
@@ -134,6 +135,8 @@
     "ocrk_colsum": [_p, _i64, _i32, _i32, _p, _i32, _p, _sz, _p],
     "ocrk_slab_sum_workspace_size": [_i32],
     "ocrk_slab_sum": [_p, _i32, _i32, _i32, _p, _i32, _p, _sz, _p],
+    "ocrk_slab_sum_batch_workspace_size": [_p, _i32],
+    "ocrk_slab_sum_batch": [_p, _i32, _p, _sz, _p],
     "ocrk_relu_mask": [_p, _p, _i64, _f32, _p, _i32, _p],
     "ocrk_mul_scalar": [_p, _i64, _p, _p],
     "ocrk_mean": [_p, _i32, _p, _p],
@@ -150,6 +153,15 @@
 _RESTYPE["ocrk_bn_bwd_bias_slab_rows"] = ctypes.c_size_t
 _RESTYPE["ocrk_bn_bwd_pooled_bias_slab_rows"] = ctypes.c_size_t
 _RESTYPE["ocrk_crc32c"] = ctypes.c_uint32
+
+
+class SlabJob(ctypes.Structure):
+    _fields_ = [("slab", _p), ("dst_lo", _p), ("dst_hi", _p), ("nslab", ctypes.c_int32), ("nc", ctypes.c_int32),
+                ("ld", ctypes.c_int32), ("split", ctypes.c_int32), ("accumulate", ctypes.c_int32),
+                ("reserved", ctypes.c_int32)]
+
+
+assert ctypes.sizeof(SlabJob) == 48
 
 
 class OcrkError(RuntimeError):
diff --git a/cnn_lstm_ctc_ocr_amd/csrc/conv.hip b/cnn_lstm_ctc_ocr_amd/csrc/conv.hip
--- a/cnn_lstm_ctc_ocr_amd/csrc/conv.hip
+++ b/cnn_lstm_ctc_ocr_amd/csrc/conv.hip
@@ -377,26 +377,43 @@
            (size_t)std::max<int64_t>(2, ocrk::conv_rows_bwd_w2_parts(std::max(B, 1))) * 9 * 32 * 32 * sizeof(float);
 }
 
+static int conv12_bwd_impl(const char* who, const void* dz, int B, int H, int W, const void* w_bwd,
+                           const void* relu_mask, const void* relu_bits, const void* x, int x_is_u8,
+                           const float* w1, const float* b1, float* dw2, float* dw1, float* db1, float* c1_slab,
+                           int accumulate, void* ws, size_t ws_bytes, int dtype, void* stream) {
+    OCRK_REQUIRE(ocrk_conv12_bwd_supported(B, H, W, dtype), "%s: B=%d H=%d W=%d dtype=%d not covered", who, B, H, W,
+                 dtype);
+    OCRK_REQUIRE(dz && w_bwd && x && w1 && b1 && dw2 && ws && (c1_slab || (dw1 && db1)), "%s: null pointer", who);
+    OCRK_REQUIRE(!relu_mask != !relu_bits, "%s: give exactly one of relu_mask / relu_bits", who);
+    OCRK_REQUIRE(ws_bytes >= ocrk_conv12_bwd_workspace_size(B, H, W) && (uintptr_t)ws % 16 == 0 &&
+                 (uintptr_t)c1_slab % 16 == 0, "%s: workspace too small or misaligned", who);
+    const int64_t nb = ocrk::conv_rows_bwd_w2_parts(B);
+    OCRK_REQUIRE(nb < (1ll << 31), "%s: too many rows", who);
+    hipStream_t s = ocrk::as_stream(stream);
+    float* c1part = c1_slab ? c1_slab : (float*)ws;
+    double* c1sum = (double*)((char*)ws + conv12_bwd_c1_bytes(B));
+    float* w2part = (float*)((char*)c1sum + (size_t)ocrk::SLAB_P * 10 * 32 * sizeof(double));
+    int st = ocrk::conv_rows_bwd_w2(dz, B, H, W, w_bwd, relu_mask, relu_bits, x, x_is_u8, w1, b1, c1part, w2part, dw2,
+                                    accumulate, s);
+    if (st || c1_slab) return st;
+    return ocrk::slab_sum(c1part, (int)nb, 10 * 32, c1sum, nullptr, dw1, db1, 9 * 32, accumulate, s);
+}
+
 extern "C" int ocrk_conv12_bwd(const void* dz, int B, int H, int W, const void* w_bwd, const void* relu_mask,
                                const void* relu_bits, const void* x, int x_is_u8, const float* w1, const float* b1,
                                float* dw2, float* dw1, float* db1, int accumulate, void* ws, size_t ws_bytes,
                                int dtype, void* stream) {
-    OCRK_REQUIRE(ocrk_conv12_bwd_supported(B, H, W, dtype), "ocrk_conv12_bwd: B=%d H=%d W=%d dtype=%d not covered",
-                 B, H, W, dtype);
-    OCRK_REQUIRE(dz && w_bwd && x && w1 && b1 && dw2 && dw1 && db1 && ws, "ocrk_conv12_bwd: null pointer");
-    OCRK_REQUIRE(!relu_mask != !relu_bits, "ocrk_conv12_bwd: give exactly one of relu_mask / relu_bits");
-    OCRK_REQUIRE(ws_bytes >= ocrk_conv12_bwd_workspace_size(B, H, W) && (uintptr_t)ws % 16 == 0,
-                 "ocrk_conv12_bwd: workspace too small or misaligned");
-    const int64_t nb = ocrk::conv_rows_bwd_w2_parts(B);
-    OCRK_REQUIRE(nb < (1ll << 31), "ocrk_conv12_bwd: too many rows");
-    hipStream_t s = ocrk::as_stream(stream);
-    float* c1part = (float*)ws;
-    double* c1sum = (double*)((char*)ws + conv12_bwd_c1_bytes(B));
-    float* w2part = (float*)((char*)c1sum + (size_t)ocrk::SLAB_P * 10 * 32 * sizeof(double));
-    int st = ocrk::conv_rows_bwd_w2(dz, B, H, W, w_bwd, relu_mask, relu_bits, x, x_is_u8, w1, b1, c1part, w2part, dw2,
-                                    accumulate, s);
-    if (st) return st;
-    return ocrk::slab_sum(c1part, (int)nb, 10 * 32, c1sum, nullptr, dw1, db1, 9 * 32, accumulate, s);
+    return conv12_bwd_impl("ocrk_conv12_bwd", dz, B, H, W, w_bwd, relu_mask, relu_bits, x, x_is_u8, w1, b1, dw2, dw1,
+                           db1, nullptr, accumulate, ws, ws_bytes, dtype, stream);
+}
+
+extern "C" int ocrk_conv12_bwd_parts(const void* dz, int B, int H, int W, const void* w_bwd, const void* relu_mask,
+                                     const void* relu_bits, const void* x, int x_is_u8, const float* w1,
+                                     const float* b1, float* dw2, float* c1_slab, int accumulate, void* ws,
+                                     size_t ws_bytes, int dtype, void* stream) {
+    OCRK_REQUIRE(c1_slab, "ocrk_conv12_bwd_parts: c1_slab is required");
+    return conv12_bwd_impl("ocrk_conv12_bwd_parts", dz, B, H, W, w_bwd, relu_mask, relu_bits, x, x_is_u8, w1, b1, dw2,
+                           nullptr, nullptr, c1_slab, accumulate, ws, ws_bytes, dtype, stream);
 }
 
 extern "C" int ocrk_conv3x3_fwd(const void* x, int B, int H, int W, int cin, const void* w_nk,
diff --git a/cnn_lstm_ctc_ocr_amd/csrc/tensor_ops.hip b/cnn_lstm_ctc_ocr_amd/csrc/tensor_ops.hip
--- a/cnn_lstm_ctc_ocr_amd/csrc/tensor_ops.hip
+++ b/cnn_lstm_ctc_ocr_amd/csrc/tensor_ops.hip
@@ -1,3 +1,5 @@
+#include <vector>
+
 #include "common.h"
 #include "reduce.h"
 #include "mfma_util.h"
@@ -24,13 +26,13 @@
 namespace ocrk {
 namespace {
 
-__global__ void __launch_bounds__(256)
-slab_sum_fused(const float* __restrict__ slab, int nslab, int NC, int ld, float* __restrict__ res,
-               float* __restrict__ dst_lo, float* __restrict__ dst_hi, int split, int accumulate) {
+__device__ __forceinline__ void
+slab_sum_block(const float* __restrict__ slab, int nslab, int NC, int ld, float* __restrict__ res,
+               float* __restrict__ dst_lo, float* __restrict__ dst_hi, int split, int accumulate, int blk) {
     constexpr int RG = 64, CQ = 4, U = 16;
     __shared__ double red[RG][4 * CQ + 1];
     const int cq = threadIdx.x % CQ, rg = threadIdx.x / CQ;
-    const int c0 = blockIdx.x * 4 * CQ + 4 * cq;
+    const int c0 = blk * 4 * CQ + 4 * cq;
     double s[4] = {0.0, 0.0, 0.0, 0.0};
     if (c0 < NC) {
         const float* col = slab + c0;
@@ -54,7 +56,7 @@
     for (int e = 0; e < 4; ++e) red[rg][4 * cq + e] = s[e];
     __syncthreads();
     if (threadIdx.x < 4 * CQ) {
-        const int c = blockIdx.x * 4 * CQ + threadIdx.x;
+        const int c = blk * 4 * CQ + threadIdx.x;
         if (c >= NC) return;
         double t = 0.0;
         for (int y = 0; y < RG; ++y) t += red[y][threadIdx.x];
@@ -63,6 +65,31 @@
         float* d = c < split ? (dst_lo ? dst_lo + c : nullptr) : (dst_hi ? dst_hi + (c - split) : nullptr);
         if (d) *d = accumulate ? *d + v : v;
     }
+}
+
+__global__ void __launch_bounds__(256)
+slab_sum_fused(const float* __restrict__ slab, int nslab, int NC, int ld, float* __restrict__ res,
+               float* __restrict__ dst_lo, float* __restrict__ dst_hi, int split, int accumulate) {
+    slab_sum_block(slab, nslab, NC, ld, res, dst_lo, dst_hi, split, accumulate, blockIdx.x);
+}
+
+constexpr int SLAB_BATCH = 32;
+struct SlabBatch {
+    ocrk_slab_job job[SLAB_BATCH];
+    int first[SLAB_BATCH];
+    int njobs;
+};
+static_assert(sizeof(ocrk_slab_job) == 48, "job layout (include/ocrk.h)");
+static_assert(sizeof(SlabBatch) <= 2048, "the batch table is a kernel argument");
+
+__global__ void __launch_bounds__(256)
+slab_sum_batch_kernel(const SlabBatch b) {
+    int j = 0;
+    for (int k = 1; k < b.njobs; ++k)
+        if (b.first[k] <= (int)blockIdx.x) j = k;
+    const ocrk_slab_job& q = b.job[j];
+    slab_sum_block(q.slab, q.nslab, q.nc, q.ld, nullptr, q.dst_lo, q.dst_hi, q.split, q.accumulate,
+                   (int)blockIdx.x - b.first[j]);
 }
 
 __global__ void __launch_bounds__(256)
@@ -233,6 +260,76 @@
                           ld);
 }
 
+static bool slab_job_fused(const ocrk_slab_job& j) {
+    return j.nc % 4 == 0 && j.ld % 4 == 0 && ((uintptr_t)j.slab & 15) == 0;
+}
+static size_t slab_job_ws(const ocrk_slab_job& j) {
+    return j.nc > 0 && !slab_job_fused(j) ? (ocrk_slab_sum_workspace_size(j.nc) + 15) / 16 * 16 : 0;
+}
+
+extern "C" size_t ocrk_slab_sum_batch_workspace_size(const ocrk_slab_job* jobs, int njobs) {
+    size_t n = 0;
+    for (int i = 0; jobs && i < njobs; ++i) n += slab_job_ws(jobs[i]);
+    return n;
+}
+
+extern "C" int ocrk_slab_sum_batch(const ocrk_slab_job* jobs, int njobs, void* ws, size_t ws_bytes, void* stream) {
+    OCRK_REQUIRE(njobs >= 0 && (jobs || njobs == 0), "ocrk_slab_sum_batch: njobs=%d", njobs);
+    struct Range { const float *lo, *hi; };
+    std::vector<Range> dst;
+    for (int i = 0; i < njobs; ++i) {
+        const ocrk_slab_job& j = jobs[i];
+        OCRK_REQUIRE(j.nslab >= 0 && j.nc >= 0 && j.ld >= j.nc, "ocrk_slab_sum_batch: job %d: bad sizes", i);
+        OCRK_REQUIRE(j.split >= 0 && j.split <= j.nc, "ocrk_slab_sum_batch: job %d: split=%d outside [0, nc=%d]", i,
+                     j.split, j.nc);
+        OCRK_REQUIRE(j.slab || j.nslab == 0 || j.nc == 0, "ocrk_slab_sum_batch: job %d: null slab", i);
+        if (j.dst_lo && j.split > 0) dst.push_back({j.dst_lo, j.dst_lo + j.split});
+        if (j.dst_hi && j.nc > j.split) dst.push_back({j.dst_hi, j.dst_hi + (j.nc - j.split)});
+    }
+    for (size_t a = 0; a < dst.size(); ++a)
+        for (size_t b = a + 1; b < dst.size(); ++b)
+            OCRK_REQUIRE(dst[a].hi <= dst[b].lo || dst[b].hi <= dst[a].lo,
+                         "ocrk_slab_sum_batch: two jobs write overlapping destinations (issue them in separate calls)");
+    OCRK_REQUIRE(ws_bytes >= ocrk_slab_sum_batch_workspace_size(jobs, njobs) && (ws_bytes == 0 || ws),
+                 "ocrk_slab_sum_batch: workspace too small");
+    hipStream_t s = ocrk::as_stream(stream);
+    ocrk::SlabBatch b;
+    b.njobs = 0;
+    int blocks = 0;
+    auto launch = [&]() -> int {
+        if (b.njobs == 0) return OCRK_OK;
+        for (int k = b.njobs; k < ocrk::SLAB_BATCH; ++k) { b.job[k] = ocrk_slab_job{}; b.first[k] = blocks; }
+        ocrk::slab_sum_batch_kernel<<<blocks, 256, 0, s>>>(b);
+        b.njobs = 0;
+        blocks = 0;
+        return ocrk::launch_status("ocrk_slab_sum_batch");
+    };
+    for (int i = 0; i < njobs; ++i) {
+        const ocrk_slab_job& j = jobs[i];
+        if (j.nc == 0 || !slab_job_fused(j)) continue;
+        b.job[b.njobs] = j;
+        b.first[b.njobs++] = blocks;
+        blocks += (j.nc + 15) / 16;
+        if (b.njobs == ocrk::SLAB_BATCH) {
+            int st = launch();
+            if (st) return st;
+        }
+    }
+    int st = launch();
+    if (st) return st;
+    char* w = (char*)ws;
+    for (int i = 0; i < njobs; ++i) {
+        const ocrk_slab_job& j = jobs[i];
+        const size_t nb = slab_job_ws(j);
+        if (nb == 0) continue;
+        st = ocrk::slab_sum(j.slab, j.nslab, j.nc, (double*)w, nullptr, j.dst_lo, j.dst_hi, j.split, j.accumulate, s,
+                            j.ld);
+        if (st) return st;
+        w += nb;
+    }
+    return OCRK_OK;
+}
+
 extern "C" int ocrk_relu_mask(const float* dy, const float* y, int64_t n, float scale, void* out, int out_dtype,
                               void* stream) {
     if (n == 0) return OCRK_OK;
diff --git a/cnn_lstm_ctc_ocr_amd/kernels.py b/cnn_lstm_ctc_ocr_amd/kernels.py
--- a/cnn_lstm_ctc_ocr_amd/kernels.py
+++ b/cnn_lstm_ctc_ocr_amd/kernels.py
@@ -133,7 +133,7 @@
             and IH >= 3 and IW >= 3 and bool(_lib.lib().ocrk_conv12_bwd_supported(B, IH - 2, IW - 2, BF16)))
 
 
-def conv12_bwd(dz, w_bwd, x, w1, b1, dw2, dw1, db1, relu_mask=None, relu_bits=None, accumulate=True):
+def conv12_bwd(dz, w_bwd, x, w1, b1, dw2, dw1, db1, relu_mask=None, relu_bits=None, accumulate=True, defer=None):
     _chk(dz, w_bwd, relu_mask, relu_bits, x, w1, b1, dw2, dw1, db1)
     if (relu_mask is None) == (relu_bits is None):
         raise ValueError("give exactly one of relu_mask / relu_bits")
@@ -142,6 +142,13 @@
         raise ValueError("relu_bits must be uint8 [B, H, W, 4]")
     nb = _lib.lib().ocrk_conv12_bwd_workspace_size(B, H, W)
     ws = _ws(nb, dz.device)
+    if defer is not None:
+        slab = torch.empty(B, 320, dtype=torch.float32, device=dz.device)
+        call("ocrk_conv12_bwd_parts", ptr(dz), B, H, W, ptr(w_bwd), ptr(relu_mask), ptr(relu_bits), ptr(x),
+             int(x.dtype == torch.uint8), ptr(w1), ptr(b1), ptr(dw2), ptr(slab), int(accumulate), ptr(ws), nb, BF16,
+             _stream(dz))
+        _defer_sums(defer, SumJob(slab, B, 320, 320, dw1, accumulate, dst_hi=db1, split=288))
+        return
     call("ocrk_conv12_bwd", ptr(dz), B, H, W, ptr(w_bwd), ptr(relu_mask), ptr(relu_bits), ptr(x),
          int(x.dtype == torch.uint8), ptr(w1), ptr(b1), ptr(dw2), ptr(dw1), ptr(db1), int(accumulate), ptr(ws), nb,
          BF16, _stream(dz))
@@ -194,7 +201,7 @@
             slab = torch.empty(tiles, 2 * Cin, dtype=torch.float32, device=dy.device)
             call("ocrk_conv3x3_bwd_data_bits_slab", ptr(dy), B, H, W, Cout, ptr(w_bwd), Cin, ptr(dx), ptr(relu_bits),
                  ptr(slab), dtype_code(dy.dtype), _stream(dy))
-            defer.append((lambda: slab_sum(slab, tiles, Cin, 2 * Cin, dbias, accumulate), (slab,)))
+            _defer_sums(defer, SumJob(slab, tiles, Cin, 2 * Cin, dbias, accumulate))
             return dx
         nb, ws = 0, None
         if dbias is not None:
@@ -208,7 +215,7 @@
         slab = torch.empty(tiles, 2 * Cin, dtype=torch.float32, device=dy.device)
         call("ocrk_conv3x3_bwd_data_slab", ptr(dy), B, H, W, Cout, ptr(w_bwd), Cin, ptr(dx), ptr(relu_mask),
              ptr(slab), dtype_code(dy.dtype), _stream(dy))
-        defer.append((lambda: slab_sum(slab, tiles, Cin, 2 * Cin, dbias, accumulate), (slab,)))
+        _defer_sums(defer, SumJob(slab, tiles, Cin, 2 * Cin, dbias, accumulate))
         return dx
     nb, ws = 0, None
     if dbias is not None:
@@ -322,10 +329,7 @@
              ptr(gamma), ptr(beta), kh, kw, sh, sw, int(dp_time_major), ptr(dz), ptr(dgamma), ptr(dbeta),
              ptr(dbias), int(accumulate), ptr(slab), ptr(ws), nb, dtype_code(z.dtype), _stream(z))
         if slab is not None:
-            def _late():
-                slab_sum(slab, rows, C, 2 * C, dbias, accumulate)
-                slab_sum(slab.view(-1)[C:], rows, C, 2 * C, dgamma, accumulate)
-            defer.append((_late, (slab,)))
+            _defer_sums(defer, SumJob(slab, rows, 2 * C, 2 * C, dbias, accumulate, dst_hi=dgamma, split=C))
         return dz
     if dbias is not None and defer is not None:
         rows = _lib.lib().ocrk_bn_bwd_bias_slab_rows(B, H, W, C, kh, kw, sh, sw)
@@ -333,7 +337,7 @@
         call("ocrk_bn_relu_pool_bwd_slab", ptr(z), ptr(dp), B, H, W, C, ptr(mean), ptr(invstd), ptr(gamma),
              ptr(beta), kh, kw, sh, sw, int(dp_time_major), ptr(dz), ptr(dgamma), ptr(dbeta), int(accumulate),
              ptr(slab), ptr(ws), nb, dtype_code(z.dtype), _stream(z))
-        defer.append((lambda: slab_sum(slab, rows, C, C, dbias, accumulate), (slab,)))
+        _defer_sums(defer, SumJob(slab, rows, C, C, dbias, accumulate))
         return dz
     call("ocrk_bn_relu_pool_bwd", ptr(z), ptr(dp), B, H, W, C, ptr(mean), ptr(invstd), ptr(gamma), ptr(beta),
          kh, kw, sh, sw, int(dp_time_major), ptr(dz), ptr(dgamma), ptr(dbeta), ptr(dbias), int(accumulate),
@@ -361,7 +365,7 @@
     call("ocrk_bn_relu_pool_bwd_apply", *args, ptr(dsum), ptr(count), ptr(dz),
          ptr(dbias if slab is None else None), int(accumulate), ptr(slab), ptr(ws), nb, dtype_code(z.dtype), _stream(z))
     if slab is not None:
-        defer.append((lambda: slab_sum(slab, rows, C, C, dbias, accumulate), (slab,)))
+        _defer_sums(defer, SumJob(slab, rows, C, C, dbias, accumulate))
     return dz
 
 
@@ -738,11 +742,77 @@
          _stream(slab))
 
 
+class SumJob:
+    __slots__ = ("slab", "nslab", "nc", "ld", "dst", "accumulate", "offset", "dst_hi", "split")
+
+    def __init__(self, slab, nslab, nc, ld, dst, accumulate=True, offset=0, dst_hi=None, split=None):
+        self.slab, self.nslab, self.nc, self.ld, self.dst = slab, int(nslab), int(nc), int(ld), dst
+        self.accumulate, self.offset, self.dst_hi = bool(accumulate), int(offset), dst_hi
+        self.split = self.nc if split is None else int(split)
+
+    def writes(self):
+        out = []
+        if self.dst is not None and self.split > 0:
+            out.append((self.dst.data_ptr(), self.dst.data_ptr() + 4 * self.split))
+        if self.dst_hi is not None and self.nc > self.split:
+            out.append((self.dst_hi.data_ptr(), self.dst_hi.data_ptr() + 4 * (self.nc - self.split)))
+        return out
+
+
+def slab_sum_batch(jobs):
+    jobs = list(jobs)
+    if not jobs:
+        return
+    table = (_lib.SlabJob * len(jobs))()
+    for rec, j in zip(table, jobs):
+        _chk(j.slab, j.dst, j.dst_hi)
+        for t in (j.slab, j.dst, j.dst_hi):
+            if t is not None and t.dtype != torch.float32:
+                raise TypeError("slab_sum_batch takes float32 slabs and destinations")
+        rec.slab = j.slab.data_ptr() + 4 * j.offset
+        rec.dst_lo = None if j.dst is None else j.dst.data_ptr()
+        rec.dst_hi = None if j.dst_hi is None else j.dst_hi.data_ptr()
+        rec.nslab, rec.nc, rec.ld, rec.split, rec.accumulate = j.nslab, j.nc, j.ld, j.split, int(j.accumulate)
+    nb = _lib.lib().ocrk_slab_sum_batch_workspace_size(table, len(jobs))
+    ws = _ws(nb, jobs[0].slab.device) if nb else None
+    call("ocrk_slab_sum_batch", table, len(jobs), ptr(ws), nb, _stream(jobs[0].slab))
+
+
+class LateSums:
+
+    def __init__(self):
+        self.jobs = []
+
+    def __len__(self):
+        return len(self.jobs)
+
+    def add(self, job):
+        mine = job.writes()
+        if any(a < d and c < b for q in self.jobs for (a, b) in q.writes() for (c, d) in mine):
+            self.flush()
+        self.jobs.append(job)
+
+    def flush(self):
+        jobs, self.jobs = self.jobs, []
+        slab_sum_batch(jobs)
+
+    def clear(self):
+        self.jobs = []
+
+
+def _defer_sums(defer, *jobs):
+    if isinstance(defer, LateSums):
+        for j in jobs:
+            defer.add(j)
+    else:
+        defer.append((lambda: slab_sum_batch(jobs), tuple(j.slab for j in jobs)))
+
+
 def _bias_parts(part, rows, nc, dbias, defer):
     if defer is None:
         slab_sum(part, rows, nc, nc, dbias)
     else:
-        defer.append((lambda: slab_sum(part, rows, nc, nc, dbias), (part,)))
+        _defer_sums(defer, SumJob(part, rows, nc, nc, dbias))
 
 
 def colsum(x, M, N, out, accumulate=True):
diff --git a/cnn_lstm_ctc_ocr_amd/model.py b/cnn_lstm_ctc_ocr_amd/model.py
--- a/cnn_lstm_ctc_ocr_amd/model.py
+++ b/cnn_lstm_ctc_ocr_amd/model.py
@@ -138,11 +138,12 @@
         dp = dp.contiguous()
         if dp.dtype != dt:
             dp = K.cast(dp, dt)
+        late = store.late_sums if options.get("LATE_SUMS") else None
         dz = K.bn_relu_pool_bwd(z, dp, mean, invstd, P[pe + "/batch_norm/gamma"], P[pe + "/batch_norm/beta"],
                                 POOLS[even], dp_time_major=(k == 4),
                                 dgamma=G[pe + "/batch_norm/gamma"], dbeta=G[pe + "/batch_norm/beta"],
                                 dbias=G[pe + "/bias"],
-                                sync=ctx.bn_sync,
+                                sync=ctx.bn_sync, defer=late,
                                 pooled=pooled if ctx.bn_sync is None and ctx.pooled_bn else None)
         B, H, W, C = dz.shape
         if k > 1:
@@ -155,7 +156,7 @@
                 with _conv_side(store, *_conv_late_tensors(store)):
                     _conv_late_run(store)
             K.conv12_bwd(dz, w_bwd, x, P["convnet/conv1/kernel"], P["convnet/conv1/bias"], G[pe + "/kernel"],
-                         G[po + "/kernel"], G[po + "/bias"], relu_bits=ctx.relu_bits)
+                         G[po + "/kernel"], G[po + "/bias"], relu_bits=ctx.relu_bits, defer=late)
             store.join()
             return (None, None, None, None) + (None,) * (len(ctx.needs_input_grad) - 4)
         if ctx.c1_fused and K.conv2_bwd_data_conv1_wgrad_ok(dz, x):
@@ -168,9 +169,10 @@
             store.join()
             return (None, None, None, None) + (None,) * (len(ctx.needs_input_grad) - 4)
         if k > 1 and ctx.relu_bits is not None:
-            dy_odd = K.conv3x3_bwd_data(dz, w_bwd, dbias=G[po + "/bias"], relu_bits=ctx.relu_bits)
+            dy_odd = K.conv3x3_bwd_data(dz, w_bwd, dbias=G[po + "/bias"], relu_bits=ctx.relu_bits, defer=late)
         else:
-            dy_odd = K.conv3x3_bwd_data(dz, w_bwd, relu_mask=y_odd, dbias=G[po + "/bias"] if k > 1 else None)
+            dy_odd = K.conv3x3_bwd_data(dz, w_bwd, relu_mask=y_odd, dbias=G[po + "/bias"] if k > 1 else None,
+                                        defer=late)
         dx = None
         if k == 1:
             with _conv_side(store, x, dy_odd, *_conv_late_tensors(store)):
@@ -310,7 +312,8 @@
         if dout.dtype != dt:
             dout = K.cast(dout, dt)
         _wxT, wx, _whT, wh, _bias = store.lstm_images(layer, dt)
-        dG = K.lstm_bwd(wh, seq_len, dout, cprev, acts, T, B, H, dbias=store.flat_bias_pair_grad(layer))
+        dG = K.lstm_bwd(wh, seq_len, dout, cprev, acts, T, B, H, dbias=store.flat_bias_pair_grad(layer),
+                        defer=store.late_sums if options.get("LATE_SUMS") else None)
         R = T * B
         dx = None
         pre = f"rnn/bdrnn{layer}"
@@ -371,7 +374,8 @@
         if dout.dtype != dt:
             dout = K.cast(dout, dt)
         _wxT, wx, _whgT, _whcT, whg, whc, _bias = store.gru_images(layer, dt)
-        dG = K.gru_bwd(whg, whc, seq_len, dout, hprev, acts, T, B, H, dbias=store.gru_bias_cat_grad(layer))
+        dG = K.gru_bwd(whg, whc, seq_len, dout, hprev, acts, T, B, H, dbias=store.gru_bias_cat_grad(layer),
+                       defer=store.late_sums if options.get("LATE_SUMS") else None)
         pre = f"rnn/bdrnn{layer}"
         R = T * B
         side = side_work(store, x, hprev, rh, dG)
diff --git a/cnn_lstm_ctc_ocr_amd/options.py b/cnn_lstm_ctc_ocr_amd/options.py
--- a/cnn_lstm_ctc_ocr_amd/options.py
+++ b/cnn_lstm_ctc_ocr_amd/options.py
@@ -6,6 +6,7 @@
     "F32_TRAIN_EXACT": 0,
     "SIDE_STREAM": 1,
     "CONV_SIDE": 1,
+    "LATE_SUMS": 1,
     "CONV12_FUSED": 1,
     "RELU_BITS": 1,
     "POOLED_BN": 1,
diff --git a/cnn_lstm_ctc_ocr_amd/params.py b/cnn_lstm_ctc_ocr_amd/params.py
--- a/cnn_lstm_ctc_ocr_amd/params.py
+++ b/cnn_lstm_ctc_ocr_amd/params.py
@@ -115,6 +115,7 @@
         self._images = {}
         self.pending = []
         self.conv_late = []
+        self.late_sums = K.LateSums()
         self.bn_group = None
         self.f32_conv_exact = False
         self.load_state_dict(values if values is not None else reference_init(self.cfg, seed))
@@ -143,10 +144,12 @@
             self.load_state_dict({k.replace("__", "/"): z[k] for k in z.files})
 
     def zero_grad(self):
+        self.late_sums.clear()
         self.join()
         self.flat_grad.zero_()
 
     def join(self):
+        self.late_sums.flush()
         while self.conv_late:
             fn, _tensors = self.conv_late.pop(0)
             fn()
diff --git a/cnn_lstm_ctc_ocr_amd/train.py b/cnn_lstm_ctc_ocr_amd/train.py
--- a/cnn_lstm_ctc_ocr_amd/train.py
+++ b/cnn_lstm_ctc_ocr_amd/train.py
@@ -46,6 +46,7 @@
         if not self.active() or self.work is not None:
             return
         g = self.store.flat_grad
+        self.store.late_sums.flush()
         if g.is_cuda:
             if self._stream is None:
                 self._stream = torch.cuda.Stream(g.device)
@@ -173,6 +174,9 @@
         prev_group, store.bn_group = store.bn_group, self._bn_group()
         try:
             return self._forward_backward(image, width, label)
+        except BaseException:
+            store.late_sums.clear()
+            raise
         finally:
             store.bn_group = prev_group
 
@@ -181,6 +185,7 @@
         if host_labels(label) and not (isinstance(width, torch.Tensor) and width.is_cuda):
             check_feasible_host(label, width)
         if self._grads_zeroed and not (store.device.type == "cuda" and torch.cuda.is_current_stream_capturing()):
+            store.late_sums.clear()
             store.join()
         else:
             store.zero_grad()
diff --git a/include/ocrk.h b/include/ocrk.h
--- a/include/ocrk.h
+++ b/include/ocrk.h
@@ -103,6 +103,10 @@
 int ocrk_conv12_bwd(const void* dz, int B, int H, int W, const void* w_bwd, const void* relu_mask,
                     const void* relu_bits, const void* x, int x_is_u8, const float* w1, const float* b1, float* dw2,
                     float* dw1, float* db1, int accumulate, void* ws, size_t ws_bytes, int dtype, void* stream);
+int ocrk_conv12_bwd_parts(const void* dz, int B, int H, int W, const void* w_bwd, const void* relu_mask,
+                          const void* relu_bits, const void* x, int x_is_u8, const float* w1, const float* b1,
+                          float* dw2, float* c1_slab, int accumulate, void* ws, size_t ws_bytes, int dtype,
+                          void* stream);
 
 size_t ocrk_conv_stats_tiles(int64_t M);
 int ocrk_conv3x3_fwd_rowstats_supported(int B, int H, int W, int cin, int cout);
@@ -251,6 +255,14 @@
 size_t ocrk_slab_sum_workspace_size(int nc);
 int ocrk_slab_sum(const float* slab, int nslab, int nc, int ld, float* out, int accumulate, void* ws,
                   size_t ws_bytes, void* stream);
+typedef struct ocrk_slab_job {
+    const float* slab;
+    float* dst_lo;
+    float* dst_hi;
+    int32_t nslab, nc, ld, split, accumulate, reserved;
+} ocrk_slab_job;
+size_t ocrk_slab_sum_batch_workspace_size(const ocrk_slab_job* jobs, int njobs);
+int ocrk_slab_sum_batch(const ocrk_slab_job* jobs, int njobs, void* ws, size_t ws_bytes, void* stream);
 int ocrk_relu_mask(const float* dy, const float* y, int64_t n, float scale, void* out, int out_dtype,
                    void* stream);
 int ocrk_mul_scalar(float* x, int64_t n, const float* s, void* stream);
```

Result: no change. 54670, median of 6 (+0.7%).
